# aantoine890/navierstokes

Hardware: AMD Instinct MI355X
Metric: fp64 CSR SpMV GFLOP/s & % HBM roofline @ nnz; 1/2/4/8 GPU (higher is better)
Workload: dtype f64

## Files before the change

include/mi355_spmv.h:

```cpp
#ifndef MI355_SPMV_H
#define MI355_SPMV_H

#ifdef __cplusplus
extern "C" {
#endif

#define MI355_SPMV_VERSION 501

enum {
    MI_OK = 0,
    MI_ERR_ARG = 1,
    MI_ERR_NODEVICE = 2,
    MI_ERR_HIP = 3,
    MI_ERR_ALLOC = 4,
    MI_ERR_UNSUPPORTED = 5,
    MI_ERR_STATE = 6
};

#define MI_MAX_POWERS 16

typedef struct mi_csr_s* mi_csr_t;
typedef struct mi_bcsr4_s* mi_bcsr4_t;
typedef struct mi_part_s* mi_part_t;
typedef void* mi_stream_t;

enum {
    MI_KERNEL_AUTO = 0,
    MI_KERNEL_STREAM = 1,
    MI_KERNEL_RING = 2,
    MI_KERNEL_ROWPAR = 3,
    MI_KERNEL_BCSR4 = 4,
    MI_KERNEL_MRING = 6,
    MI_KERNEL_SSTREAM = 7,
    MI_KERNEL_TILE = 5
};

int mi_version(void);
const char* mi_strerror(int status);
const char* mi_last_error(void);
int mi_device_count(int* count);
int mi_set_device(int device);
int mi_device_synchronize(void);
int mi_flush_cache(void);
int mi_flush_cache_async(mi_stream_t s);

int mi_csr_create(int n, int ncols, const int* ptrow, const int* indcol, const double* coef, mi_csr_t* out);
int mi_csr_create_mapped(int n, int ncols, const int* ptrow, const int* indcol, const double* coef,
                         const int* rowmap, mi_csr_t* out);
int mi_csr_destroy(mi_csr_t A);
int mi_csr_update_values(mi_csr_t A, const double* coef);
int mi_csr_update_values_dev(mi_csr_t A, const double* d_coef, mi_stream_t s);
int mi_csr_dims(mi_csr_t A, int* n, int* ncols, long long* nnz);
int mi_csr_reorder_info(mi_csr_t A, int* reordered, int* block, double* spread_before, double* spread_after,
                        double* us_natural, double* us_reordered);
int mi_csr_perm(mi_csr_t A, int* reordered, int* perm );
int mi_vec_to_internal_dev(mi_csr_t A, const double* d_x, double* d_x_int, mi_stream_t s);
int mi_vec_from_internal_dev(mi_csr_t A, const double* d_x_int, double* d_x, mi_stream_t s);
int mi_spmv_internal_dev(mi_csr_t A, const double* d_x_int, double* d_y_int, mi_stream_t s);
int mi_spmk_internal_dev(mi_csr_t A, int k, const double* d_x_int, double* const* d_y_int_out, mi_stream_t s);
int mi_reorder_probe(int n, const int* ptrow, const int* indcol, int* block, int* perm, double* spread_before,
                     double* spread_after);
int mi_csr_set_kernel(mi_csr_t A, int kernel_id);
int mi_csr_ring_info(mi_csr_t A, int* config_id, int* runs, int* runs_not_ringable, double* nnz_fraction_ringable);
int mi_csr_ring_shape_info(mi_csr_t A, int* blocks, int* lean, int* depth, double* us_aligned, double* us_unaligned);
int mi_csr_tune_info(mi_csr_t A, double* us_ring, double* us_stream);
int mi_csr_tune_detail(mi_csr_t A, double us[5], int* ring_nt, int* stream_nt);
int mi_ring_plan_probe(int n, const int* ptrow, const int* indcol, int config_id, int* nblk, int* runs,
                       int* runs_not_ringable, double* nnz_fraction_ringable, int* max_slot);
int mi_csr_tile_info(mi_csr_t A, int* built, int* nblk, double* unique_per_nnz, double us[2], int* nt);
int mi_tile_plan_probe(int n, const int* ptrow, const int* indcol, int threads, int* nblk, long long* distinct_total,
                       int* max_distinct, long long* nnz_listed);
int mi_csr_placement_info(mi_csr_t A, int* n_values, int* n_total, double* us, int cap);
int mi_vec_alloc_placed(mi_csr_t A, int nvec, int draws, double** d_vecs, double* us, int cap, int* n_us);
int mi_vec_free_placed(double* d_vec);
int mi_csr_sstream_info(mi_csr_t A, int* built, int* rounds, long long* steps, double* padding, double us[4], int* form);
int mi_sstream_plan_probe(int n, int ncols, const int* ptrow, const int* indcol, int* eligible, int* rounds, long long* steps, double* padding);
int mi_sstream_plan_probe_ex(int n, int ncols, const int* ptrow, const int* indcol, int shift, int ghost_lo, int ghost_hi, int* eligible, int* rounds,
                             long long* steps, double* padding, int* ghost_workgroups, int* rounds_min_max);
int mi_sstream_mw_plan_probe(int n, int ncols, const int* ptrow, const int* indcol, int shift, int* eligible, int* rounds, long long* steps, double* padding);
int mi_csr_mring_info(mi_csr_t A, int* built, int* runs, int* runs_not_served, double* nnz_fraction_served, double us[2], int* nt);
int mi_mring_plan_probe(int n, const int* ptrow, const int* indcol, int* nblk, int* runs, int* runs_not_served,
                        double* nnz_fraction_served, long long* window_restarts);
int mi_mring_plan_deal_probe(int n, const int* ptrow, const int* indcol, int* table_len, int* run_blocks, int cap);
int mi_ring_plan_lean(int n, const int* ptrow, const int* indcol, int config_id, int* lean);
int mi_csr_block4_structure(int n, const int* ptrow, const int* indcol, int* is_blocked, long long* nblocks);
int mi_csr_set_nontemporal(mi_csr_t A, int ring_nt, int stream_nt);
int mi_stream_read_probe(long long bytes, int launches, double* us_per_launch);
int mi_csr_get_kernel(mi_csr_t A, int* kernel_id);
const char* mi_csr_kernel_name(mi_csr_t A);

int mi_spmv(mi_csr_t A, const double* x, double* y);
int mi_spmv_dev(mi_csr_t A, const double* d_x, double* d_y, mi_stream_t s);

int mi_spmk(mi_csr_t A, int k, const double* x, double* const* y_out);
int mi_spmk_dev(mi_csr_t A, int k, const double* d_x, double* const* d_y_out, mi_stream_t s);

int mi_csr_spmk_info(mi_csr_t A, int k, int* eligible, int* one_launch, double* us_k_launches, double* us_one_launch);

int mi_spmk_plan_probe(int n, const int* ptrow, const int* indcol, int* eligible, int* runs, int* max_deps);

int mi_dot(int n, const double* x, const double* y, double* out);
int mi_dot_dev(int n, const double* d_x, const double* d_y, double* d_out, mi_stream_t s);
int mi_axpy(int n, double a, const double* x, double* y);
int mi_axpy_dev(int n, double a, const double* d_x, double* d_y, mi_stream_t s);
int mi_orthogonalize(int n, const double* b, const double* x1, double* x3, double alpha, double* beta_out);
int mi_orthogonalize_dev(int n, const double* d_b, const double* d_x1, double* d_x3, double alpha,
                         double* d_beta_out, mi_stream_t s);
int mi_spmv_dot_dev(mi_csr_t A, const double* d_x, double* d_y, const double* d_b, double* d_beta_out, mi_stream_t s);
int mi_csr_dot_epilogue_info(mi_csr_t A, int* in_epilogue);
int mi_csr_dot_epilogue_layout(mi_csr_t A, int* threads, int* wgs, int* nblk, int* run_first_block, int* block_row0,
                               int* block_rows, int cap_runs, int cap_blocks);
int mi_spmv_orthogonalize_dev(mi_csr_t A, const double* d_x, double* d_x1, const double* d_b, double* d_x3, double alpha,
                              double* d_beta_out, mi_stream_t s);
int mi_orthonormalize_against_basis(int n, int m, const double* const* basis, double* y, double* dots_out );
int mi_orthonormalize_against_basis_dev(int n, int m, const double* const* d_basis, double* d_y, double* d_dots ,
                                        mi_stream_t s);
int mi_mdot(int n, int m, const double* const* basis, const double* y, double* dots );
int mi_mdot_dev(int n, int m, const double* const* d_basis , const double* d_y,
                double* d_dots , mi_stream_t s);
int mi_maxpy(int n, int m, const double* coef , int negate, const double* const* basis, double* y);
int mi_maxpy_dev(int n, int m, const double* d_coef , int negate, const double* const* d_basis, double* d_y,
                 double* d_norm_out, mi_stream_t s);
int mi_cgs_dev(int n, int m, const double* const* d_basis, double* d_y, int passes, double* d_h ,
               double* d_norm , mi_stream_t s);
int mi_norm2(int n, const double* x, double* out);
int mi_norm2_dev(int n, const double* d_x, double* d_out, mi_stream_t s);
int mi_rel_error(int n, const double* ref, const double* test, double* out);
int mi_rel_error_dev(int n, const double* d_ref, const double* d_test, double* d_out, mi_stream_t s);
int mi_gather_dev(int m, const int* d_idx, const double* d_src, double* d_dst, mi_stream_t s);

int mi_bcsr4_create(int nbrows, int nbcols, const int* ptrow, const int* indcol, const double* coef,
                    mi_bcsr4_t* out);
int mi_bcsr4_destroy(mi_bcsr4_t A);
enum { MI_BLOCK_ROWMAJOR = 0, MI_BLOCK_COLMAJOR = 1 };
int mi_bcsr4_create_layout(int nbrows, int nbcols, const int* ptrow, const int* indcol, const double* coef, int layout, mi_bcsr4_t* out);
int mi_bcsr4_update_values_layout(mi_bcsr4_t A, const double* coef, int layout);
int mi_bcsr4_update_values_layout_dev(mi_bcsr4_t A, const double* d_coef, int layout, mi_stream_t s);
int mi_bcsr4_tile_info(mi_bcsr4_t A, int* built, int* in_use, double* us_plain, double* us_tile);
int mi_bcsr4_sell_info(mi_bcsr4_t A, int* built, int* form_in_use, long long* steps, double* padding, double us[4]);
int mi_bcsr4_sell_plan_probe(int nbrows, const int* ptrow, const int* indcol, int nwaves_max, int* nslices, long long* nsteps, int* nwaves,
                             int* sptr, int* wrng, unsigned* col);
int mi_bcsr4_update_values(mi_bcsr4_t A, const double* coef);
int mi_bcsr4_update_values_dev(mi_bcsr4_t A, const double* d_coef, mi_stream_t s);
int mi_bcsr4_spmv(mi_bcsr4_t A, const double* x, double* y);
int mi_bcsr4_spmv_dev(mi_bcsr4_t A, const double* d_x, double* d_y, mi_stream_t s);
int mi_bcsr4_spmk(mi_bcsr4_t A, int k, const double* x, double* const* y_out);
int mi_bcsr4_spmk_dev(mi_bcsr4_t A, int k, const double* d_x, double* const* d_y_out, mi_stream_t s);

enum { MI_ARITH_CHAIN = 0, MI_ARITH_BLOCKACC = 1 };
int mi_bcsr4_spmm(mi_bcsr4_t A, int s, const double* X, long long ldx, double* Y, long long ldy, int arith);
int mi_bcsr4_spmm_dev(mi_bcsr4_t A, int s, const double* d_X, long long ldx, double* d_Y, long long ldy, int arith,
                      mi_stream_t st);
int mi_bcsr4_spmm_info(mi_bcsr4_t A, int s, int* tile_built, int* form_in_use, int* longest_list, double us[5]);
int mi_bcsr4_spmm_plan_probe(int nbrows, const int* ptrow, const int* indcol, int per, int ucap, int* refused, int* ntiles, int* umax,
                             double* mean_list, int* wg_ptr, long long wg_ptr_cap, unsigned* nodes, long long nodes_cap,
                             unsigned short* slots, long long slots_cap, int* rows, long long rows_cap);
int mi_spmm_dev(mi_csr_t A, int s, const double* d_X, long long ldx, double* d_Y, long long ldy, mi_stream_t st);
int mi_krylov_basis_dev(mi_csr_t A, int s, const double* d_v0, double* d_V, long long ldv, int orth, double* d_coef,
                        mi_stream_t st);
int mi_krylov_basis_cgs_dev(mi_csr_t A, int s, const double* d_v0, double* d_V, long long ldv, int passes, double* d_coef,
                            mi_stream_t st);

typedef struct mi_bilu4_s* mi_bilu4_t;
int mi_bilu4_create(int nbrows, const int* ptrow, const int* indcol, const double* coef, int layout , int fill,
                    mi_bilu4_t* out);
int mi_bilu4_create_host(int nbrows, const int* ptrow, const int* indcol, const double* coef, int layout, int fill, mi_bilu4_t* out);
int mi_bilu4_destroy(mi_bilu4_t F);
int mi_bilu4_refactor(mi_bilu4_t F, const double* coef, int layout);
int mi_bilu4_solve_dev(mi_bilu4_t F, const double* d_b, double* d_x, mi_stream_t s);
int mi_bilu4_solve(mi_bilu4_t F, const double* b, double* x);
int mi_bilu4_info(mi_bilu4_t F, int* nbrows, long long* nblocks, int* fwd_levels, int* bwd_levels, int* launches, int* form,
                  double us[2], double* factor_seconds, long long* factor_bytes);
int mi_bilu4_factor_host(mi_bilu4_t F, int* ptr, int* col, int* diag, double* val, long long cap_blocks);
int mi_bilu4_plan_probe(int nbrows, const int* ptrow, const int* indcol, int fill, long long* nblocks, int* fwd_levels,
                        int* bwd_levels, int* fwd_launches, int* bwd_launches, int* fwd_sizes, int* bwd_sizes, int cap_levels);

int mi_bilu4dev_plan_probe(int nbrows, const int* ptrow, const int* indcol, int fill, long long* update_pairs, int* launches,
                           long long* plan_bytes);
int mi_bilu4dev_prepare(mi_bilu4_t F);
int mi_bilu4dev_refactor(mi_bilu4_t F, const double* d_coef, int layout, mi_stream_t s);
int mi_bilu4dev_status(mi_bilu4_t F, int* bad_row);
int mi_bilu4dev_fetch(mi_bilu4_t F);
int mi_bilu4dev_info(mi_bilu4_t F, int* prepared, int* launches, long long* plan_bytes);

enum { MI_BILU_FORM_LEVELS = 0, MI_BILU_FORM_ONE = 1, MI_BILU_FORM_AUTO = -1 };
int mi_bilu4one_plan_probe(int nbrows, const int* ptrow, const int* indcol, int fill, int workgroups, int* eligible, int nchunks[2],
                           int max_deps[2], long long* plan_bytes, int* const chunk_pos[2], int* const chunk_lev[2],
                           int* const dep_ptr[2], int* const dep[2]);
int mi_bilu4one_prepare(mi_bilu4_t F);
int (mi_bilu4_set_solve_form)(mi_bilu4_t F, int form);
int mi_bilu4one_status(mi_bilu4_t F);
int mi_bilu4one_info(mi_bilu4_t F, int* prepared, int* eligible, int* workgroups, int nchunks[2], int max_deps[2], long long* plan_bytes);

int mi_bilu4sw_prepare(mi_bilu4_t F);
int mi_bilu4sw_solve_dev(mi_bilu4_t F, const double* d_b, double* d_x, int sweeps_fwd, int sweeps_bwd, mi_stream_t s);
int mi_bilu4sw_solve(mi_bilu4_t F, const double* b, double* x, int sweeps_fwd, int sweeps_bwd);
int mi_bilu4sw_info(mi_bilu4_t F, int* prepared, int* max_fwd, int* max_bwd, int* launches_last, long long* work_bytes);

int mi_bilu4sp_prepare(mi_bilu4_t F);
int mi_bilu4sp_solve_dev(mi_bilu4_t F, const double* d_b, double* d_x, int sweeps_fwd, int sweeps_bwd, mi_stream_t s);
int mi_bilu4sp_solve(mi_bilu4_t F, const double* b, double* x, int sweeps_fwd, int sweeps_bwd);
int mi_bilu4sp_status(mi_bilu4_t F, int* bad_block_row, long long* overflowed);
int mi_bilu4sp_fetch(mi_bilu4_t F, float* val, long long cap_blocks);
int mi_bilu4sp_info(mi_bilu4_t F, int* prepared, int* convert_launches, int* launches_last, long long* copy_bytes);

int mi_part_create(int nranks, int rank, const long long* row_starts, const int* ptrow,
                   const int* indcol_global, const double* coef, mi_part_t* out);
int mi_part_destroy(mi_part_t P);
int mi_part_sizes(mi_part_t P, int* n_local, int* n_halo, int* n_interior_rows, int* n_boundary_rows);
int mi_part_recv_counts(mi_part_t P, int* counts );
int mi_part_recv_ids(mi_part_t P, int peer, long long* ids );
int mi_part_set_send_ids(mi_part_t P, int peer, int count, const long long* ids );
int mi_part_send_counts(mi_part_t P, int* counts );
int mi_part_local_csr(mi_part_t P, int which, int* nrows, const int** ptrow, const int** indcol_local,
                      const double** coef, const int** rowmap);
int mi_part_combined_info(mi_part_t P, int* n_left);
int mi_part_sends_contiguous(mi_part_t P, int* contiguous);
int mi_part_send_index(mi_part_t P, int* total, const int** local_idx );
int mi_part_finalize(mi_part_t P);
int mi_part_set_kernel(mi_part_t P, int kernel_id);
int mi_part_update_values(mi_part_t P, const double* coef);
int mi_part_pack_dev(mi_part_t P, const double* d_x_ext, double* d_sendbuf, mi_stream_t s);
int mi_part_spmv_interior_dev(mi_part_t P, const double* d_x_ext, double* d_y_local, mi_stream_t s);
int mi_part_spmv_boundary_dev(mi_part_t P, const double* d_x_ext, double* d_y_local, mi_stream_t s);

#define MI_COMM_ID_BYTES 128
int mi_comm_available(void);
int mi_comm_unique_id(void* id128);
int mi_part_comm_init(mi_part_t P, const void* id128);
int mi_part_comm_info(mi_part_t P, int* comm_ranks, int* comm_rank);
int mi_part_spmv_dev(mi_part_t P, double* d_x_ext, double* d_y_local, mi_stream_t s);
int mi_part_status(mi_part_t P);
int mi_part_send_union(mi_part_t P, int* count, const int** local_idx );
int mi_part_allgather_setup(mi_part_t P, const int* counts , const long long* ids );
int mi_part_set_allgather(mi_part_t P, int on);
int mi_part_allgather_info(mi_part_t P, int* ready, int* in_use, int* slice );
#define MI_IPC_HANDLE_BYTES 64
int mi_part_push_export(mi_part_t P, void* handle64, long long* layout );
int mi_part_push_connect(mi_part_t P, const void* handles , const long long* layouts );
int mi_part_spmv_push_dev(mi_part_t P, double* d_x_ext, double* d_y_local, mi_stream_t s);
int mi_part_push_info(mi_part_t P, int* ready, int* fused, int* neighbours);
const char* mi_part_kernel_name(mi_part_t P, int which);
int mi_part_push_unfuse(mi_part_t P);
int mi_part_push_disable(mi_part_t P);
int mi_comm_selftest(int count, double* max_abs_err);

typedef struct mi_dist_s* mi_dist_t;
typedef struct mi_dist_vec_s* mi_dist_vec_t;
int mi_dist_create(int ndev, int n, const int* ptrow, const int* indcol, const double* coef, mi_dist_t* out);
int mi_dist_destroy(mi_dist_t D);
int mi_dist_info(mi_dist_t D, int* nranks, int* distinct_devices, int* exchange, int* fused, long long* halo_total, long long* halo_max);
const char* mi_dist_exchange_name(mi_dist_t D);
const char* mi_dist_exchange_note(mi_dist_t D);
int mi_dist_rank_info(mi_dist_t D, int rank, int* device, long long* row_start, int* n_local, int* n_halo, long long* nnz_local,
                      mi_stream_t* stream );
int mi_dist_update_values(mi_dist_t D, const double* coef);
int mi_dist_spmv(mi_dist_t D, const double* x, double* y);
int mi_dist_spmk(mi_dist_t D, int k, const double* x, double* const* y_out);
int mi_dist_dot(mi_dist_t D, const double* x, const double* y, double* out);
int mi_dist_orthogonalize(mi_dist_t D, const double* b, const double* x1, double* x3, double alpha, double* beta_out);
int mi_dist_vec_create(mi_dist_t D, mi_dist_vec_t* out);
int mi_dist_vec_destroy(mi_dist_vec_t v);
int mi_dist_vec_set(mi_dist_vec_t v, const double* host );
int mi_dist_vec_get(mi_dist_vec_t v, double* host );
int mi_dist_vec_ptr(mi_dist_vec_t v, int rank, double** d_ptr);
int mi_dist_spmv_dev(mi_dist_t D, mi_dist_vec_t x, mi_dist_vec_t y);
int mi_dist_spmk_dev(mi_dist_t D, int k, mi_dist_vec_t x, const mi_dist_vec_t* y_out );
int mi_dist_synchronize(mi_dist_t D);
int mi_dist_dot_dev(mi_dist_t D, mi_dist_vec_t a, mi_dist_vec_t b, double* out);
int mi_dist_orthogonalize_dev(mi_dist_t D, mi_dist_vec_t b, mi_dist_vec_t x1, mi_dist_vec_t x3, double alpha, double* beta_out);

#ifdef __cplusplus
}
#endif
#endif
```

navierstokes_amd/csrc/capi_csr.hip:

```cpp
#include "capi_internal.hpp"
#include "reorder.hpp"
#include "mring_plan.hpp"
#include "tile_plan.hpp"

int get_table(mi_csr_t A, int nnzb, BlockTable** out)
{
    auto it = A->tables.find(nnzb);
    if (it == A->tables.end()) {
        std::vector<int> rows, ptrs;
        int row_align = A->nnz < 20000000 ? 64 : 1;
        if (const char* e = getenv("MI355_STREAM_ROW_ALIGN")) row_align = std::max(1, atoi(e));
        build_row_blocks(A->n, A->h_ptrow.data(), nnzb, 4 * kWG, rows, ptrs, row_align, 7);
        BlockTable T;
        T.nnzb = nnzb;
        T.nblk = (int)rows.size() - 1;
        std::vector<int2> h(rows.size());
        for (size_t i = 0; i < rows.size(); i++) h[i] = make_int2(rows[i], ptrs[i]);
        HIP_TRY(T.d_blk.upload(h));
        it = A->tables.emplace(nnzb, std::move(T)).first;
    }
    *out = &it->second;
    return MI_OK;
}

static inline bool beyond_infinity_cache(double bytes_per_nnz, long long nnz, int n) { return bytes_per_nnz * (double)nnz + 16.0 * (double)n > 0.75 * 256e6; }

constexpr double kSsMaxPadding = 0.12;
static double ss_max_padding()
{
    if (const char* e = getenv("MI355_SSTREAM_MAX_PADDING")) return std::max(0.0, atof(e));
    return kSsMaxPadding;
}

static int build_sstream(mi_csr_t A, const int* ptrow, const int* indcol, int ghost_lo = 0, int ghost_hi = 0)
{
    if (A->ss.dev.val) return MI_OK;
    SsPlanHost P;
    SsMwPlanHost M;
    const int shift = (A->y_offset & 1) && !A->d_rowmap ? 1 : 0;
    build_sstream_plan(A->n, A->ncols, ptrow, indcol, ss_max_padding(), P, true, shift, ghost_lo, ghost_hi);
    SstreamCopy T;
    hipError_t e;
    if (!P.eligible) {
        if (ghost_lo < ghost_hi || env_is("MI355_SSTREAM_MW", "0")) return MI_OK;
        build_sstream_mw_plan(A->n, A->ncols, ptrow, indcol, ss_max_padding(), M, shift);
        if (!M.eligible) return MI_OK;
        e = ss_mw_upload(M, T.dev);
        T.mw = e == hipSuccess;
    } else e = ss_upload(P, T.dev, ghost_lo < ghost_hi);
    const SsPlanHost& Q = P.eligible ? P : M;
    if (e != hipSuccess) {
        if (e == hipErrorOutOfMemory) { (void)hipGetLastError(); return MI_OK; }
        return fail(MI_ERR_HIP, std::string("sliced copy: ") + hipGetErrorString(e));
    }
    T.nwg = Q.nwg;
    T.rounds = Q.rounds;
    T.shift = Q.shift;
    T.steps = Q.steps;
    T.padding = (double)Q.pad_places / (double)A->nnz;
    T.max_slice_nnz = Q.max_slice_nnz;
    if (ghost_lo < ghost_hi) {
        T.h_wg_halo = P.wg_halo;
        T.h_wg = P.wg;
        T.fusable = P.fusable;
    }
    sstream_fill_values(T.rounds, A->n, T.shift, A->d_ptrow, A->d_coef, nullptr, T.dev.slice_step, T.dev.slice_len, T.dev.val, T.max_slice_nnz, nullptr, T.mw ? 1 : 0);
    if ((e = hipGetLastError()) != hipSuccess) {
        T = {};
        return fail(MI_ERR_HIP, std::string("sliced copy fill: ") + hipGetErrorString(e));
    }
    T.nt = beyond_infinity_cache(10.0, A->nnz, A->n);
    T.deep = T.nt;
    if (const char* fe = getenv("MI355_SSTREAM_FORM")) {
        const int f = atoi(fe);
        T.nt = (f & 1) == 0;
        T.deep = f >= 2;
    }
    A->ss.copy() = std::move(T);
    return MI_OK;
}

int launch_sstream(mi_csr_t A, const double* d_x, double* d_y, const int* rowmap, hipStream_t s, const RingComm* comm)
{
    SstreamTable& T = A->ss;
    SsView S{T.dev.val, T.dev.slot, T.dev.wg, T.dev.win, T.nwg, A->n + T.shift, A->ncols, rowmap, T.shift};
    double* yy = rowmap ? d_y : d_y - T.shift;
    if (T.mw) {
        if (comm) return fail(MI_ERR_STATE, "the cut-ring sliced stream has no fused multi-GPU form");
        SsMwView V{S, T.dev.winK};
        if (T.deep) {
            if (T.nt) hipLaunchKernelGGL((spmv_sstream_mw<12, true>), dim3((unsigned)T.nwg), dim3(256), 0, s, V, d_x, yy);
            else hipLaunchKernelGGL((spmv_sstream_mw<12, false>), dim3((unsigned)T.nwg), dim3(256), 0, s, V, d_x, yy);
        } else {
            if (T.nt) hipLaunchKernelGGL((spmv_sstream_mw<8, true>), dim3((unsigned)T.nwg), dim3(256), 0, s, V, d_x, yy);
            else hipLaunchKernelGGL((spmv_sstream_mw<8, false>), dim3((unsigned)T.nwg), dim3(256), 0, s, V, d_x, yy);
        }
        HIP_TRY(hipGetLastError());
        return MI_OK;
    }
    if (comm) {
        const unsigned grid = (unsigned)(T.nwg + comm->push_wgs);
        if (T.deep) {
            if (T.nt) hipLaunchKernelGGL((spmv_sstream_fused<12, true>), dim3(grid), dim3(256), 0, s, S, d_x, yy, *comm);
            else hipLaunchKernelGGL((spmv_sstream_fused<12, false>), dim3(grid), dim3(256), 0, s, S, d_x, yy, *comm);
        } else {
            if (T.nt) hipLaunchKernelGGL((spmv_sstream_fused<8, true>), dim3(grid), dim3(256), 0, s, S, d_x, yy, *comm);
            else hipLaunchKernelGGL((spmv_sstream_fused<8, false>), dim3(grid), dim3(256), 0, s, S, d_x, yy, *comm);
        }
    } else if (T.deep) {
        if (T.nt) hipLaunchKernelGGL((spmv_sstream<12, true>), dim3((unsigned)T.nwg), dim3(256), 0, s, S, d_x, yy);
        else hipLaunchKernelGGL((spmv_sstream<12, false>), dim3((unsigned)T.nwg), dim3(256), 0, s, S, d_x, yy);
    } else {
        if (T.nt) hipLaunchKernelGGL((spmv_sstream<8, true>), dim3((unsigned)T.nwg), dim3(256), 0, s, S, d_x, yy);
        else hipLaunchKernelGGL((spmv_sstream<8, false>), dim3((unsigned)T.nwg), dim3(256), 0, s, S, d_x, yy);
    }
    HIP_TRY(hipGetLastError());
    return MI_OK;
}

static bool ring_wants_skew(int n, const int* ptrow)
{
    long long bad = 0;
    for (int i = 0; i < n; i++) {
        const int len = ptrow[i + 1] - ptrow[i];
        bad += len > 0 && (len % 16 == 0 || len == 8);
    }
    return 2 * bad > n;
}

constexpr long long kLargeNnz = 20000000;
static size_t placed_vector_len(int n, int ncols) { return (size_t)std::max(n, ncols) + 64; }
static int large_row_align(long long nnz) { return nnz >= kLargeNnz ? 1 : 0; }

static int build_mring(mi_csr_t A, const int* indcol, int row_align = 0)
{
    if (A->mring.d_plan || A->n == 0 || A->nnz == 0) return MI_OK;
    std::vector<int> back;
    if (!indcol) {
        if (!A->d_indcol) return fail(MI_ERR_STATE, "mring plan: the handle no longer holds its column indices");
        back.resize((size_t)A->nnz);
        HIP_TRY(hipMemcpy(back.data(), A->d_indcol, sizeof(int) * (size_t)A->nnz, hipMemcpyDeviceToHost));
        indcol = back.data();
    }
    MringPlanHost P;
    build_mring_plan(A->n, A->h_ptrow.data(), indcol, P, row_align);
    MringTable M;
    HIP_TRY(M.d_plan.alloc(P.plan.size()));
    HIP_TRY(M.d_first.upload(P.first));
    HIP_TRY(M.d_ok.alloc(P.run_ok.size()));
    HIP_TRY(M.d_rng.alloc(P.run_rng.size()));
    HIP_TRY(M.d_slots.alloc(P.slots.size()));
    HIP_TRY(M.d_plan.fill(P.plan));
    HIP_TRY(M.d_ok.fill(P.run_ok));
    HIP_TRY(M.d_rng.fill(P.run_rng));
    HIP_TRY(M.d_slots.fill(P.slots));
    M.nblk = P.nblk;
    M.wgs = P.wgs;
    M.nruns = P.nruns;
    M.bpw = P.bpw;
    M.bad_runs = P.bad_runs;
    M.restarts = P.restarts;
    M.ok_fraction = 1.0 - (double)P.bad_nnz / (double)A->nnz;
    M.depth = P.bpw >= 40 ? 4 : 2;
    M.skew = ring_wants_skew(A->n, A->h_ptrow.data());
    M.nt = beyond_infinity_cache(10.0, A->nnz, A->n);
    A->mring = std::move(M);
    return MI_OK;
}

static int build_tile(mi_csr_t A, const int* indcol)
{
    if (A->tile.d_desc || A->n == 0 || A->nnz == 0) return MI_OK;
    std::vector<int> back;
    if (!indcol) {
        if (!A->d_indcol) return fail(MI_ERR_STATE, "tile plan: the handle no longer holds its column indices");
        back.resize((size_t)A->nnz);
        HIP_TRY(hipMemcpy(back.data(), A->d_indcol, sizeof(int) * (size_t)A->nnz, hipMemcpyDeviceToHost));
        indcol = back.data();
    }
    TilePlanHost P;
    build_tile_plan(A->n, A->h_ptrow.data(), indcol, P, kTileNnzb, 0, A->nnz < 20000000 ? 64 : 1);
    TileTable T;
    HIP_TRY(T.d_desc.alloc(P.desc.size()));
    HIP_TRY(T.d_ulist.alloc(P.ulist.size()));
    HIP_TRY(T.d_slots.alloc(P.slots.size()));
    HIP_TRY(T.d_desc.fill(P.desc));
    HIP_TRY(T.d_ulist.fill(P.ulist));
    HIP_TRY(T.d_slots.fill(P.slots));
    T.nblk = P.nblk;
    T.unique_per_nnz = (double)(P.ulist.size() - kTileThreads) / (double)A->nnz;
    long long mult8 = 0;
    for (int i = 0; i < A->n; i++) {
        const int len = A->h_ptrow[i + 1] - A->h_ptrow[i];
        mult8 += len > 0 && len % 8 == 0;
    }
    T.skew = 10 * mult8 > A->n;
    T.nt = beyond_infinity_cache(10.0, A->nnz, A->n);
    A->tile = std::move(T);
    return MI_OK;
}

static int fill_ring_table(RingTable& R, const RingPlanHost& best, int n, const int* ptrow, const int* indcol, long long nnz, bool ghosts,
                           const int* row_min = nullptr, const int* row_max = nullptr, bool square = false)
{
    R.cfg = best.cfg;
    if (best.cfg.id == 4 && best.bpw >= 40) R.cfg.depth = 4;
    if (const char* e = getenv("MI355_RING_DEPTH")) {
        const int d = atoi(e);
        if (best.cfg.id == 4 && d >= 2 && d <= 4) R.cfg.depth = d;
    }
    R.nblk = best.nblk;
    R.wgs = best.wgs;
    R.bpw = best.bpw;
    R.bad_runs = best.bad_runs;
    R.ok_fraction = nnz ? 1.0 - (double)best.bad_nnz / (double)nnz : 0.0;
    R.lean = best.lean && best.cfg.id == 4 && !env_is("MI355_RING_LEAN", "0");
    if (best.nblk <= 0) return MI_OK;
    HIP_TRY(R.d_plan.upload(best.plan));
    HIP_TRY(R.d_ok.upload(best.run_ok));
    R.all_in_loop = true;
    for (int g = 0; g < best.wgs; g++) R.all_in_loop = R.all_in_loop && best.run_ok[g] == 1;
    R.h_dep_ptr.clear();
    R.h_dep_run.clear();
    if (square && row_min && R.all_in_loop && R.lean && best.cfg.id == 4 && !ghosts) build_run_deps(best, n, R.h_dep_ptr, R.h_dep_run);
    for (int g = 0; g < best.wgs; g++)
        R.uniform = R.uniform && best.run_rng[2 * g] == std::min(best.nblk, g * best.bpw) &&
                    best.run_rng[2 * g + 1] == std::min(best.nblk, (g + 1) * best.bpw);
    HIP_TRY(R.d_rng.upload(best.run_rng));
    if (ghosts) {
        R.h_run_halo = best.run_halo;
        HIP_TRY(R.d_run_halo.upload(best.run_halo));
    }
    {
        std::vector<unsigned short> slots;
        build_ring_slots(best, indcol, slots);
        HIP_TRY(R.d_slots.upload(slots));
    }
    R.skew = ring_wants_skew(n, ptrow);
    if (const char* e2 = getenv("MI355_RING_SKEW")) R.skew = atoi(e2) != 0;
    return MI_OK;
}

static int time_on(LaunchTimer& tm, mi_csr_t A, const double* x, double* y, int warm, int timed, double* us)
{
    return tm.time(warm, timed, [&] { return launch_spmv(A, x, y, nullptr); }, us);
}

static int placement_draws(mi_csr_t A, ScratchPair* given, bool keep_pair)
{
    const long long nnz = A->nnz;
    const char* pe = getenv("MI355_PLACEMENT_DRAWS");
    int draws = pe ? std::max(0, std::min(16, atoi(pe))) : 4;
    const bool early_stop = pe == nullptr;
    if (!pe) {
        size_t mem_free = 0, mem_total = 0;
        if (hipMemGetInfo(&mem_free, &mem_total) == hipSuccess && nnz > 0)
            draws = (int)std::min<size_t>((size_t)draws, mem_free / 8 / (sizeof(double) * (size_t)nnz));
        else (void)hipGetLastError();
    }
    const bool blocked_choice = A->auto_kernel == MI_KERNEL_BCSR4 && A->blocked && A->blocked->d_coef && !(A->blocked->sell_form >= 0 && A->blocked->sell.val);
    const bool streams_coef = A->auto_kernel == MI_KERNEL_RING || A->auto_kernel == MI_KERNEL_MRING || A->auto_kernel == MI_KERNEL_STREAM || A->auto_kernel == MI_KERNEL_TILE || blocked_choice;
    if (!(draws > 0 && streams_coef && nnz >= kLargeNnz)) return MI_OK;
    LaunchTimer tm;
    ScratchPair own;
    ScratchPair& pair = given ? *given : own;
    if (!given) {
        const size_t len = std::max(placed_vector_len(A->n, A->ncols), (size_t)(A->n_out > 0 ? A->n_out : 1));
        if (int rc = own.alloc(len, len)) return rc;
    }
    double *const tx = pair.x, *const ty = pair.y;
    if (int rc = tm.init()) return rc;
    auto time_now = [&](double* us) { return time_on(tm, A, tx, ty, 3, 8, us); };
    auto redraw = [&](auto& slot, size_t len, size_t pad, int ndraws) {
        using Arr = std::remove_reference_t<decltype(slot)>;
        double best = 0.0;
        if (!slot || len == 0 || time_now(&best) != MI_OK) return;
        const double first = best;
        A->place_us.push_back(best);
        std::vector<Arr> losers;
        for (int d = 0; d < ndraws; d++) {
            Arr fresh;
            if (fresh.alloc(len + pad) != hipSuccess) { (void)hipGetLastError(); break; }
            if ((pad && hipMemset(fresh + len, 0, sizeof(*fresh.get()) * pad) != hipSuccess) ||
                hipMemcpy(fresh, slot, sizeof(*fresh.get()) * len, hipMemcpyDeviceToDevice) != hipSuccess) { (void)hipGetLastError(); break; }
            std::swap(slot, fresh);
            double t = 0.0;
            const int rct = time_now(&t);
            A->place_us.push_back(rct == MI_OK ? t : -1.0);
            if (rct == MI_OK && t < 0.96 * best) best = t;
            else std::swap(slot, fresh);
            losers.push_back(std::move(fresh));
            if (early_stop && d == 0 && rct == MI_OK && std::fabs(t - first) <= 0.02 * first) break;
        }
        for (Arr& l : losers) l = {};
    };
    if (blocked_choice) redraw(A->blocked->d_coef, 16 * (size_t)A->blocked->nblocks, 16, draws);
    else redraw(A->d_coef, (size_t)nnz, (size_t)kRingPadNnz, draws);
    A->place_draws_coef = (int)A->place_us.size();
    if (A->auto_kernel == MI_KERNEL_RING) redraw(A->ring.d_slots, (size_t)A->ring.nblk * A->ring.cfg.nnzb, 0, (draws + 1) / 2);
    else if (A->auto_kernel == MI_KERNEL_MRING) redraw(A->mring.d_slots, (size_t)A->mring.nblk * kMringNnzb, 0, (draws + 1) / 2);
    if (keep_pair && !A->kept_x) A->kept_x = std::move(pair.x), A->kept_y = std::move(pair.y);
    return MI_OK;
}

constexpr long long kMeasureNnz = 200000;

struct CsrInput {
    int n, ncols;
    const int* ptrow;
    const int* indcol;
    const double* coef;
    const int* rowmap;
    int ghost_lo, ghost_hi;
    long long nnz = 0;
    bool offset_only = false;
    std::vector<int> row_min, row_max;
    bool ghosts() const { return ghost_lo < ghost_hi; }
};

static int check_input(CsrInput& in)
{
    const int n = in.n;
    const int* ptrow = in.ptrow;
    CHECK_ARG(n >= 0 && in.ncols >= 0, "negative dimension");
    CHECK_ARG(ptrow, "ptrow is null");
    CHECK_ARG(ptrow[0] == 0, "ptrow[0] must be 0");
    for (int i = 0; i < n; i++) CHECK_ARG(ptrow[i] <= ptrow[i + 1], "ptrow must be non-decreasing");
    in.nnz = ptrow[n];
    CHECK_ARG(in.nnz == 0 || (in.indcol && in.coef), "indcol/coef is null");
    CHECK_ARG(in.nnz <= 0x7fffffffLL - 2 * kRingPadNnz && n <= 0x7fffffff - 2 * kRingPadRows, "matrix too large for 32-bit offsets: partition it (mi_part_*)");
    in.row_min.resize((size_t)n);
    in.row_max.resize((size_t)n);
    for (int i = 0; i < n; i++) {
        int lo = 0x7fffffff, hi = -1;
        for (int k = ptrow[i]; k < ptrow[i + 1]; k++) {
            const int c = in.indcol[k];
            CHECK_ARG(c >= 0 && c < in.ncols, "column index outside [0, ncols)");
            lo = c < lo ? c : lo;
            hi = c > hi ? c : hi;
        }
        in.row_min[i] = lo;
        in.row_max[i] = hi;
    }
    in.offset_only = in.rowmap != nullptr && n > 0;
    for (int i = 1; in.offset_only && i < n; i++) in.offset_only = in.rowmap[i] == in.rowmap[0] + i;
    return MI_OK;
}

static int upload(mi_csr_t A, const CsrInput& in)
{
    const int n = in.n;
    const long long nnz = in.nnz;
    const size_t pad = 8, padv = kRingPadNnz, padr = kRingPadRows;
    HIP_TRY(hipGetDevice(&A->device));
    HIP_TRY(A->d_ptrow.alloc((size_t)n + 1 + padr));
    HIP_TRY(A->d_indcol.alloc((size_t)nnz + pad));
    HIP_TRY(A->d_coef.alloc((size_t)nnz + padv));
    HIP_TRY(hipMemset(A->d_ptrow + n + 1, 0, sizeof(int) * padr));
    HIP_TRY(hipMemset(A->d_indcol + nnz, 0, sizeof(int) * pad));
    HIP_TRY(hipMemset(A->d_coef + nnz, 0, sizeof(double) * padv));
    HIP_TRY(A->d_ptrow.fill(in.ptrow, (size_t)n + 1));
    HIP_TRY(A->d_indcol.fill(in.indcol, (size_t)nnz));
    HIP_TRY(A->d_coef.fill(in.coef, (size_t)nnz));
    A->mapped = in.rowmap != nullptr;
    if (in.offset_only) A->y_offset = in.rowmap[0];
    if (in.rowmap && n > 0 && !in.offset_only) {
        HIP_TRY(A->d_rowmap.alloc((size_t)n + padr));
        HIP_TRY(hipMemset(A->d_rowmap + n, 0, sizeof(int) * padr));
        HIP_TRY(A->d_rowmap.fill(in.rowmap, (size_t)n));
    }
    return MI_OK;
}

static int plan_ring(mi_csr_t A, const CsrInput& in)
{
    const int n = in.n;
    const long long nnz = in.nnz;
    if (n == 0 || nnz == 0) return MI_OK;
    int forced = 0;
    if (const char* e = getenv("MI355_RING_CONFIG")) forced = atoi(e);
    RingPlanHost best;
    bool have = false;
    for (int t = 0; t < kNumRingConfigs && !have; t++) {
        const int id = forced >= 1 && forced <= kNumRingConfigs ? forced : kRingConfigOrder[t];
        RingPlanHost P;
        build_ring_plan(kRingConfigs[id - 1], n, in.ptrow, in.row_min.data(), in.row_max.data(), P, in.ghost_lo, in.ghost_hi, large_row_align(nnz));
        const double okf = 1.0 - (double)P.bad_nnz / (double)nnz;
        if (forced || okf >= 0.90) {
            best = std::move(P);
            have = true;
        } else if (t == 0) {
            best = std::move(P);
        }
        if (forced) break;
    }
    RingTable R;
    if (int rc = fill_ring_table(R, best, n, in.ptrow, in.indcol, nnz, in.ghosts(), in.row_min.data(), in.row_max.data(), n == in.ncols)) return rc;
    A->ring = std::move(R);
    A->auto_kernel = (have && A->ring.ok_fraction >= 0.90) ? MI_KERNEL_RING : MI_KERNEL_STREAM;
    return MI_OK;
}

static bool plan_wanted(const char* sw, const char* name, bool by_size, bool* asked)
{
    *asked = env_is(sw, "1") || env_is("MI355_SPMV_KERNEL", name);
    return !env_is(sw, "0") && (*asked || by_size);
}

static int plan_optional(mi_csr_t A, const CsrInput& in)
{
    if (in.n == 0 || in.nnz == 0) return MI_OK;
    const bool measured = in.nnz >= kMeasureNnz;
    bool asked;
    int rc;
    if (plan_wanted("MI355_TILE", "tile", measured && A->auto_kernel != MI_KERNEL_RING, &asked)) {
        if ((rc = build_tile(A, in.indcol))) return rc;
        if (!asked && A->tile.unique_per_nnz > 0.6) A->tile = {};
    }
    if (plan_wanted("MI355_MRING", "mring", measured && A->auto_kernel != MI_KERNEL_RING, &asked)) {
        if ((rc = build_mring(A, in.indcol, large_row_align(in.nnz)))) return rc;
        if (!asked && A->mring.ok_fraction < 0.90) A->mring = {};
    }
    if (plan_wanted("MI355_SSTREAM", "sstream", measured, &asked)) {
        if ((rc = build_sstream(A, in.ptrow, in.indcol, in.ghost_lo, in.ghost_hi))) return rc;
        A->ss.asked = asked;
    }
    return MI_OK;
}

static int attach_blocked(mi_csr_t A, const CsrInput& in)
{
    const int n = in.n;
    const int* rowmap = in.rowmap;
    bool node_map = rowmap != nullptr && !in.offset_only && n % 4 == 0;
    for (int b = 0; node_map && b < n / 4; b++)
        node_map = rowmap[4 * b] % 4 == 0 && rowmap[4 * b + 1] == rowmap[4 * b] + 1 && rowmap[4 * b + 2] == rowmap[4 * b] + 2 &&
                   rowmap[4 * b + 3] == rowmap[4 * b] + 3;
    if (!(!rowmap || in.offset_only || node_map) || n < 4 || in.nnz < 16 || in.ncols % 4 != 0 || env_is("MI355_AUTO_BCSR", "0")) return MI_OK;
    std::vector<int> bptr, bcol;
    std::vector<double> bval;
    if (!csr_to_bcsr4_exact(n, in.ptrow, in.indcol, in.coef, bptr, bcol, bval)) return MI_OK;
    mi_bcsr4_t B = nullptr;
    if (int rc = mi_bcsr4_create(n / 4, in.ncols / 4, bptr.data(), bcol.data(), bval.data(), &B)) return rc;
    A->blocked.reset(B);
    if (node_map) {
        std::vector<int> bmap((size_t)n / 4);
        for (int b = 0; b < n / 4; b++) bmap[b] = rowmap[4 * b] / 4;
        HIP_TRY(B->d_browmap.upload(bmap));
    }
    return MI_OK;
}

static void load_defaults(mi_csr_t A, const CsrInput& in)
{
    A->ring.nt = A->ring.d_slots && beyond_infinity_cache(10.0, in.nnz, in.n);
    if (const char* e = getenv("MI355_RING_NT")) A->ring.nt = A->ring.d_slots && atoi(e) != 0;
    A->stream_nt = beyond_infinity_cache(12.0, in.nnz, in.n);
    if (const char* e = getenv("MI355_STREAM_NT")) A->stream_nt = atoi(e) != 0;
    if (const char* e = getenv("MI355_TILE_NT")) A->tile.nt = atoi(e) != 0;
    if (const char* e = getenv("MI355_MRING_NT")) A->mring.nt = atoi(e) != 0;
    if (A->blocked) A->auto_kernel = MI_KERNEL_BCSR4;
    A->n_out = in.n;
    if (in.rowmap)
        for (int i = 0; i < in.n; i++) A->n_out = in.rowmap[i] + 1 > A->n_out ? in.rowmap[i] + 1 : A->n_out;
}

static bool apply_forced_kernel(mi_csr_t A)
{
    const char* e = getenv("MI355_SPMV_KERNEL");
    if (!e) return false;
    if (!strcmp(e, "stream")) A->auto_kernel = MI_KERNEL_STREAM;
    else if (!strcmp(e, "ring") && A->ring.d_plan) A->auto_kernel = MI_KERNEL_RING;
    else if (!strcmp(e, "rowpar")) A->auto_kernel = MI_KERNEL_ROWPAR;
    else if (!strcmp(e, "bcsr4") && A->blocked) A->auto_kernel = MI_KERNEL_BCSR4;
    else if (!strcmp(e, "tile") && A->tile.d_desc) A->auto_kernel = MI_KERNEL_TILE;
    else if (!strcmp(e, "mring") && A->mring.d_plan) A->auto_kernel = MI_KERNEL_MRING;
    else if (!strcmp(e, "sstream") && A->ss.dev.val) A->auto_kernel = MI_KERNEL_SSTREAM;
    else return false;
    return true;
}

static bool& nt_flag(mi_csr_t A, int k)
{
    switch (k) {
    case MI_KERNEL_RING: return A->ring.nt;
    case MI_KERNEL_TILE: return A->tile.nt;
    case MI_KERNEL_MRING: return A->mring.nt;
    default: return A->stream_nt;
    }
}

static double tuned_us(mi_csr_t A, int k)
{
    if (k == MI_KERNEL_BCSR4 && A->tune_us[k][0] > 0) return A->tune_us[k][0];
    if (k != MI_KERNEL_RING && k != MI_KERNEL_TILE && k != MI_KERNEL_MRING) k = MI_KERNEL_STREAM;
    return A->tune_us[k][nt_flag(A, k)];
}

static const struct {
    int kernel;
    const char* nt_env;
} kTuneKernels[4] = {{MI_KERNEL_RING, "MI355_RING_NT"}, {MI_KERNEL_STREAM, "MI355_STREAM_NT"}, {MI_KERNEL_TILE, "MI355_TILE_NT"}, {MI_KERNEL_MRING, "MI355_MRING_NT"}};

static void tune(mi_csr_t A, LaunchTimer& tm, const ScratchPair& sp)
{
    const int timed = A->nnz < 40000000 ? 12 : 6;
    auto measure = [&](int warm, int count, double& slot, bool& failed) {
        double t = 0.0;
        if (time_on(tm, A, sp.x, sp.y, warm, count, &t) == MI_OK) slot = min_measured(slot, t);
        else failed = true;
    };
    const bool ring_ok = A->auto_kernel == MI_KERNEL_RING;
    auto in_race = [&](int k) {
        return k == MI_KERNEL_RING ? ring_ok : k == MI_KERNEL_TILE ? A->tile.d_desc != nullptr : k == MI_KERNEL_MRING ? A->mring.d_plan != nullptr : true;
    };
    bool nt0[4], failed[4][2] = {};
    for (int i = 0; i < 4; i++) nt0[i] = nt_flag(A, kTuneKernels[i].kernel);
    const double* ring_us = A->tune_us[MI_KERNEL_RING];
    for (int round = 0; round < 2; round++)
        for (int i = 0; i < 4; i++)
            for (int nt = 0; nt < 2; nt++) {
                const int k = kTuneKernels[i].kernel;
                double& us = A->tune_us[k][nt];
                if (!in_race(k) || failed[i][nt] || (getenv(kTuneKernels[i].nt_env) && nt != nt0[i])) continue;
                if (k == MI_KERNEL_RING && nt && !A->ring.d_slots) continue;
                if (k == MI_KERNEL_STREAM && round == 1 && ring_ok &&
                    us > 1.25 * std::min(ring_us[0] > 0 ? ring_us[0] : ring_us[1], ring_us[1] > 0 ? ring_us[1] : ring_us[0]))
                    continue;
                nt_flag(A, k) = nt;
                A->kernel = k;
                measure(3, timed, us, failed[i][nt]);
            }
    for (int i = 0; i < 4; i++) {
        const int k = kTuneKernels[i].kernel;
        for (int nt = 0; nt < 2; nt++)
            if (failed[i][nt]) A->tune_us[k][nt] = 0.0;
        nt_flag(A, k) = in_race(k) ? better(A->tune_us[k][1], A->tune_us[k][0]) : nt0[i];
    }
    for (int i = 0; i < 4; i++)
        if (better(tuned_us(A, kTuneKernels[i].kernel), tuned_us(A, A->auto_kernel))) A->auto_kernel = kTuneKernels[i].kernel;
    if (A->blocked) {
        const double holder = tuned_us(A, A->auto_kernel);
        bool bfailed = false;
        A->kernel = MI_KERNEL_BCSR4;
        measure(3, 6, A->tune_us[MI_KERNEL_BCSR4][0], bfailed);
        if (better(A->tune_us[MI_KERNEL_BCSR4][0], holder)) A->auto_kernel = MI_KERNEL_BCSR4;
    }
    if (A->ss.dev.val && !getenv("MI355_SSTREAM_FORM")) {
        const double holder = tuned_us(A, A->auto_kernel);
        double* us = A->ss.tune_us;
        bool sfailed[4] = {};
        A->kernel = MI_KERNEL_SSTREAM;
        for (int round = 0; round < 2; round++)
            for (int f = 0; f < 4; f++) {
                if (sfailed[f]) continue;
                A->ss.nt = (f & 1) == 0;
                A->ss.deep = f >= 2;
                measure(3, timed, us[f], sfailed[f]);
            }
        int bf = -1;
        for (int f = 0; f < 4; f++) {
            if (sfailed[f]) us[f] = 0.0;
            if (us[f] > 0 && (bf < 0 || us[f] < us[bf])) bf = f;
        }
        if (bf >= 0) {
            A->ss.nt = (bf & 1) == 0;
            A->ss.deep = bf >= 2;
            if (better(us[bf], holder)) A->auto_kernel = MI_KERNEL_SSTREAM;
        }
        if (A->auto_kernel != MI_KERNEL_SSTREAM && !A->ss.asked && !(A->ghost_lo < A->ghost_hi)) A->ss.copy() = {};
    }
    A->kernel = MI_KERNEL_AUTO;
}

static void compare_ring_shapes(mi_csr_t A, const CsrInput& in, LaunchTimer& tm, const ScratchPair& sp)
{
    const long long nnz = in.nnz;
    if (!env_is("MI355_RING_SHAPE_COMPARE", "1") || getenv("MI355_RING_ROW_ALIGN") || nnz < kLargeNnz) return;
    auto time_now = [&](double* us) { return time_on(tm, A, sp.x, sp.y, 3, 8, us); };
    double us64 = 0.0, us1 = 0.0;
    if (A->auto_kernel == MI_KERNEL_RING && A->ring.cfg.id == 4) {
        RingPlanHost alt;
        build_ring_plan(kRingConfigs[3], in.n, in.ptrow, in.row_min.data(), in.row_max.data(), alt, in.ghost_lo, in.ghost_hi, 64);
        RingTable aligned;
        if (1.0 - (double)alt.bad_nnz / (double)nnz >= 0.90 &&
            fill_ring_table(aligned, alt, in.n, in.ptrow, in.indcol, nnz, in.ghosts(), in.row_min.data(), in.row_max.data(), in.n == in.ncols) == MI_OK) {
            aligned.nt = A->ring.nt;
            A->kernel = MI_KERNEL_RING;
            int rct = time_now(&us1);
            RingTable unaligned = std::move(A->ring);
            A->ring = std::move(aligned);
            if (rct == MI_OK) rct = time_now(&us64);
            A->kernel = MI_KERNEL_AUTO;
            A->tune_us_ring_aligned = us64;
            A->tune_us_ring_unaligned = us1;
            if (rct != MI_OK || !(us64 < 0.98 * us1)) A->ring = std::move(unaligned);
            else unaligned = {};
        }
    } else if (A->auto_kernel == MI_KERNEL_MRING) {
        MringTable unaligned = std::move(A->mring);
        if (build_mring(A, in.indcol, 64) == MI_OK && A->mring.d_plan && A->mring.ok_fraction >= 0.90) {
            A->mring.nt = unaligned.nt;
            A->kernel = MI_KERNEL_MRING;
            int rct = time_now(&us64);
            MringTable aligned = std::move(A->mring);
            A->mring = std::move(unaligned);
            if (rct == MI_OK) rct = time_now(&us1);
            A->kernel = MI_KERNEL_AUTO;
            A->tune_us_ring_aligned = us64;
            A->tune_us_ring_unaligned = us1;
            if (rct == MI_OK && us64 < 0.98 * us1) A->mring = std::move(aligned);
            else aligned = {};
        } else {
            A->mring = std::move(unaligned);
        }
    }
}

static int measure_at_create(mi_csr_t A, const CsrInput& in, bool defer_placement)
{
    const size_t scratch_len = placed_vector_len(in.n, in.ncols);
    LaunchTimer tm;
    ScratchPair sp;
    int rc = sp.alloc(std::max(scratch_len, (size_t)(in.ncols > 0 ? in.ncols : 1)), std::max(scratch_len, (size_t)(A->n_out > 0 ? A->n_out : 1)));
    if (rc || (rc = tm.init())) return rc;
    tune(A, tm, sp);
    compare_ring_shapes(A, in, tm, sp);
    if (!defer_placement) (void)placement_draws(A, &sp, !in.rowmap && in.n == in.ncols && in.n == A->n_out && !in.ghosts());
    return MI_OK;
}

int csr_create_impl(int n, int ncols, const int* ptrow, const int* indcol, const double* coef,
                    const int* rowmap, mi_csr_t* out, int ghost_lo, int ghost_hi, bool defer_placement)
{
    CHECK_ARG(out, "out is null");
    *out = nullptr;
    CsrInput in{n, ncols, ptrow, indcol, coef, rowmap, ghost_lo, ghost_hi};
    int rc = check_input(in);
    if (rc || (rc = need_device())) return rc;
    std::unique_ptr<mi_csr_s> owner(new (std::nothrow) mi_csr_s());
    mi_csr_t A = owner.get();
    if (!A) return fail(MI_ERR_ALLOC, "host allocation failed");
    A->n = n;
    A->ncols = ncols;
    A->nnz = in.nnz;
    A->ghost_lo = ghost_lo;
    A->ghost_hi = ghost_hi;
    A->h_ptrow.assign(ptrow, ptrow + n + 1);
    if ((rc = upload(A, in)) || (rc = plan_ring(A, in)) || (rc = plan_optional(A, in)) || (rc = attach_blocked(A, in))) return rc;
    load_defaults(A, in);
    const bool forced_kernel = apply_forced_kernel(A);
    if (!forced_kernel && in.nnz < kMeasureNnz && A->auto_kernel == MI_KERNEL_RING && !in.ghosts()) A->auto_kernel = MI_KERNEL_STREAM;
    if (!forced_kernel && !env_is("MI355_SPMV_AUTOTUNE", "0") && in.nnz >= kMeasureNnz && (rc = measure_at_create(A, in, defer_placement))) return rc;
    HIP_TRY(hipStreamSynchronize(nullptr));
    *out = owner.release();
    return MI_OK;
}

static int time_handle(mi_csr_t A, int warm, int timed, double* us)
{
    LaunchTimer tm;
    ScratchPair sp;
    int rc = sp.alloc((size_t)(A->ncols > 0 ? A->ncols : 1), (size_t)(A->n_out > 0 ? A->n_out : 1));
    if (rc || (rc = tm.init())) return rc;
    return time_on(tm, A, sp.x, sp.y, warm, timed, us);
}

static int maybe_reorder(mi_csr_t A, const int* ptrow, const int* indcol, const double* coef)
{
    const bool force = env_is("MI355_REORDER", "1");
    if (env_is("MI355_REORDER", "0")) return MI_OK;
    const int n = A->n;
    if (A->mapped || n != A->ncols || n < 8 || A->nnz == 0) return MI_OK;
    if (!force && (n < 100000 || resolve_kernel(A) == MI_KERNEL_RING || resolve_kernel(A) == MI_KERNEL_SSTREAM)) return MI_OK;
    const int block = csr_has_block4_pattern(n, ptrow, indcol) ? 4 : 1;
    const double nn = (double)n / block;
    const double spread = mean_column_distance(n, ptrow, indcol, block);
    A->spread_before = spread;
    if (!force && spread < 2.0 * std::pow(nn, 2.0 / 3.0)) return MI_OK;
    Reorder R;
    rcm_reorder(n, ptrow, indcol, block, R);
    A->reorder_block = block;
    A->spread_after = R.spread_after;
    if (!force && R.spread_after > 0.5 * spread) return MI_OK;
    std::vector<int> p2, c2, src_start;
    std::vector<double> v2;
    permute_csr(n, ptrow, indcol, coef, R, p2, c2, v2, src_start);
    mi_csr_t inner = nullptr;
    int rc = csr_create_impl(n, n, p2.data(), c2.data(), v2.data(), R.iperm.data(), &inner);
    if (rc) return rc;
    A->inner.reset(inner);
    HIP_TRY(A->d_iperm.alloc((size_t)n));
    HIP_TRY(A->d_src_start.alloc((size_t)n));
    HIP_TRY(A->d_xp.alloc((size_t)n));
    HIP_TRY(A->d_iperm.fill(R.iperm));
    HIP_TRY(A->d_src_start.fill(src_start));
    bool keep = true;
    if (!force && !env_is("MI355_SPMV_AUTOTUNE", "0")) {
        const int timed = A->nnz < 40000000 ? 12 : 6;
        (void)A->inner.own.release();
        rc = time_handle(A, 3, timed, &A->us_natural);
        A->inner.reset(inner);
        if (rc) return rc;
        if ((rc = time_handle(A, 3, timed, &A->us_reordered))) return rc;
        keep = A->us_reordered < 0.97 * A->us_natural;
    }
    if (!keep) {
        A->inner.reset(), A->d_iperm = {}, A->d_src_start = {}, A->d_xp = {};
        return MI_OK;
    }
    A->h_iperm = R.iperm;
    A->xp_claimed = false;
    A->d_ptrow = {}, A->d_indcol = {}, A->d_coef = {};
    A->drop_tables();
    A->ring = {}, A->tile = {}, A->mring = {}, A->ss = {}, A->blocked.reset();
    return MI_OK;
}

extern "C" int mi_csr_create(int n, int ncols, const int* ptrow, const int* indcol, const double* coef, mi_csr_t* out)
{
    int rc = csr_create_impl(n, ncols, ptrow, indcol, coef, nullptr, out, 0, 0, true);
    if (rc) return rc;
    if ((rc = maybe_reorder(*out, ptrow, indcol, coef)) || (!(*out)->inner && (rc = placement_draws(*out, nullptr, n == ncols))) ||
        (hipStreamSynchronize(nullptr) != hipSuccess && (rc = fail(MI_ERR_HIP, "mi_csr_create: synchronize")))) {
        mi_csr_destroy(*out);
        *out = nullptr;
    }
    return rc;
}

extern "C" int mi_reorder_probe(int n, const int* ptrow, const int* indcol, int* block, int* perm, double* spread_before,
                                double* spread_after)
{
    CHECK_ARG(n >= 0 && ptrow && (ptrow[n] == 0 || indcol), "bad argument");
    for (int i = 0; i < n; i++) {
        CHECK_ARG(ptrow[i] <= ptrow[i + 1], "ptrow must be non-decreasing");
        for (int k = ptrow[i]; k < ptrow[i + 1]; k++) CHECK_ARG(indcol[k] >= 0 && indcol[k] < n, "column index outside [0, n)");
    }
    const int b = csr_has_block4_pattern(n, ptrow, indcol) ? 4 : 1;
    Reorder R;
    rcm_reorder(n, ptrow, indcol, b, R);
    if (block) *block = b;
    if (perm)
        for (int i = 0; i < n; i++) perm[i] = R.perm[i];
    if (spread_before) *spread_before = R.spread_before;
    if (spread_after) *spread_after = R.spread_after;
    return MI_OK;
}

extern "C" int mi_csr_reorder_info(mi_csr_t A, int* reordered, int* block, double* spread_before, double* spread_after,
                                   double* us_natural, double* us_reordered)
{
    CHECK_ARG(A, "null handle");
    if (reordered) *reordered = A->inner ? 1 : 0;
    if (block) *block = A->reorder_block;
    if (spread_before) *spread_before = A->spread_before;
    if (spread_after) *spread_after = A->spread_after;
    if (us_natural) *us_natural = A->us_natural;
    if (us_reordered) *us_reordered = A->us_reordered;
    return MI_OK;
}

extern "C" int mi_csr_perm(mi_csr_t A, int* reordered, int* perm)
{
    CHECK_ARG(A, "null handle");
    if (reordered) *reordered = A->inner ? 1 : 0;
    if (perm) {
        if (A->inner) {
            CHECK_ARG((int)A->h_iperm.size() == A->n, "permutation not kept on this handle");
            for (int r = 0; r < A->n; r++) perm[A->h_iperm[r]] = r;
        } else {
            for (int i = 0; i < A->n; i++) perm[i] = i;
        }
    }
    return MI_OK;
}

extern "C" int mi_vec_to_internal_dev(mi_csr_t A, const double* d_x, double* d_x_int, mi_stream_t s)
{
    CHECK_ARG(A, "null handle");
    if (A->n == 0) return MI_OK;
    CHECK_ARG(d_x && d_x_int && d_x != d_x_int, "null vector, or in place");
    if (A->inner) return gather_perm(A, d_x, d_x_int, (hipStream_t)s);
    HIP_TRY(hipMemcpyAsync(d_x_int, d_x, sizeof(double) * (size_t)A->n, hipMemcpyDeviceToDevice, (hipStream_t)s));
    return MI_OK;
}

extern "C" int mi_vec_from_internal_dev(mi_csr_t A, const double* d_x_int, double* d_x, mi_stream_t s)
{
    CHECK_ARG(A, "null handle");
    if (A->n == 0) return MI_OK;
    CHECK_ARG(d_x && d_x_int && d_x != d_x_int, "null vector, or in place");
    if (A->inner) return scatter_perm(A, d_x_int, d_x, (hipStream_t)s);
    HIP_TRY(hipMemcpyAsync(d_x, d_x_int, sizeof(double) * (size_t)A->n, hipMemcpyDeviceToDevice, (hipStream_t)s));
    return MI_OK;
}

extern "C" int mi_spmv_internal_dev(mi_csr_t A, const double* d_x_int, double* d_y_int, mi_stream_t s)
{
    CHECK_ARG(A, "null handle");
    CHECK_ARG(A->n == A->ncols && !A->mapped, "the internal numbering is defined for square, unmapped matrices");
    CHECK_ARG(A->n == 0 || (d_x_int && d_y_int), "null vector");
    if (A->inner) return launch_spmv(A->inner, d_x_int, d_y_int, (hipStream_t)s, false);
    return launch_spmv(A, d_x_int, d_y_int, (hipStream_t)s);
}

extern "C" int mi_spmk_internal_dev(mi_csr_t A, int k, const double* d_x_int, double* const* d_y_int_out, mi_stream_t s)
{
    CHECK_ARG(A, "null handle");
    if (k < 1 || k > MI_MAX_POWERS) return fail(MI_ERR_UNSUPPORTED, "k must be in 1..MI_MAX_POWERS");
    CHECK_ARG(d_y_int_out, "null output array");
    CHECK_ARG(A->n == A->ncols && !A->mapped, "the internal numbering is defined for square, unmapped matrices");
    if (A->n == 0) return MI_OK;
    CHECK_ARG(d_x_int, "null vector");
    for (int p = 0; p < k; p++) CHECK_ARG(d_y_int_out[p], "null output vector");
    return spmk_unmapped(A->inner ? A->inner : A, k, d_x_int, d_y_int_out, (hipStream_t)s);
}

extern "C" int mi_csr_create_mapped(int n, int ncols, const int* ptrow, const int* indcol, const double* coef,
                                    const int* rowmap, mi_csr_t* out)
{
    return csr_create_impl(n, ncols, ptrow, indcol, coef, rowmap, out);
}

extern "C" int mi_csr_destroy(mi_csr_t A)
{
    if (!A) return MI_OK;
    delete A;
    return MI_OK;
}

static int refresh_blocked_values(mi_csr_t A, hipStream_t s, bool sliced_done = false)
{
    if (A->ss.dev.val && !sliced_done) {
        SstreamTable& T = A->ss;
        sstream_fill_values(T.rounds, A->n, T.shift, A->d_ptrow, A->d_coef, nullptr, T.dev.slice_step, T.dev.slice_len, T.dev.val, T.max_slice_nnz, s, T.mw ? 1 : 0);
        HIP_TRY(hipGetLastError());
    }
    if (!A->blocked || A->blocked->nbrows == 0) return MI_OK;
    return bcsr4_refresh_from_csr(A->blocked, A->d_ptrow, A->d_coef, nullptr, s);
}

__global__ __launch_bounds__(256) void permute_values_kernel(int n, const int* __restrict__ new_ptrow, const int* __restrict__ src_start,
                                                             const double* __restrict__ src, double* __restrict__ dst)
{
    __shared__ int s_p[65], s_a[64];
    const int tid = threadIdx.x;
    for (int r0 = blockIdx.x * 64; r0 < n; r0 += gridDim.x * 64) {
        const int nr = min(64, n - r0);
        if (tid <= nr) s_p[tid] = new_ptrow[r0 + tid];
        if (tid < nr) s_a[tid] = src_start[r0 + tid];
        __syncthreads();
        const int b0 = s_p[0], seg = s_p[nr] - b0;
        for (int k = tid; k < seg; k += 256) {
            const int p = b0 + k;
            int lo = 0, hi = nr;
            while (hi - lo > 1) {
                const int mid = (lo + hi) >> 1;
                if (s_p[mid] <= p) lo = mid;
                else hi = mid;
            }
            dst[p] = src[s_a[lo] + (p - s_p[lo])];
        }
        __syncthreads();
    }
}

extern "C" int mi_csr_update_values_dev(mi_csr_t A, const double* d_coef, mi_stream_t s_)
{
    CHECK_ARG(A, "null handle");
    if (A->nnz == 0) return MI_OK;
    CHECK_ARG(d_coef, "null coef");
    hipStream_t s = (hipStream_t)s_;
    if (A->inner) {
        mi_csr_t I = A->inner;
        hipLaunchKernelGGL(permute_values_kernel, dim3((unsigned)std::max(1, std::min((A->n + 63) / 64, 4096))), dim3(256), 0, s, A->n, I->d_ptrow, A->d_src_start, d_coef, I->d_coef);
        HIP_TRY(hipGetLastError());
        return refresh_blocked_values(I, s);
    }
    if (A->ss.dev.val && d_coef != A->d_coef) {
        SstreamTable& T = A->ss;
        sstream_fill_values(T.rounds, A->n, T.shift, A->d_ptrow, d_coef, A->d_coef, T.dev.slice_step, T.dev.slice_len, T.dev.val, T.max_slice_nnz, s, T.mw ? 1 : 0);
        HIP_TRY(hipGetLastError());
        return refresh_blocked_values(A, s, true);
    }
    if (A->blocked && A->blocked->nbrows > 0 && d_coef != A->d_coef)
        return bcsr4_refresh_from_csr(A->blocked, A->d_ptrow, d_coef, A->d_coef, s);
    if (d_coef != A->d_coef) HIP_TRY(hipMemcpyAsync(A->d_coef, d_coef, sizeof(double) * (size_t)A->nnz, hipMemcpyDeviceToDevice, s));
    return refresh_blocked_values(A, s);
}

extern "C" int mi_csr_update_values(mi_csr_t A, const double* coef)
{
    CHECK_ARG(A, "null handle");
    if (A->nnz == 0) return MI_OK;
    CHECK_ARG(coef, "null coef");
    if (A->inner) {
        if (!A->d_vtmp) HIP_TRY(A->d_vtmp.alloc((size_t)A->nnz));
        HIP_TRY(hipMemcpy(A->d_vtmp, coef, sizeof(double) * (size_t)A->nnz, hipMemcpyHostToDevice));
        int rc = mi_csr_update_values_dev(A, A->d_vtmp, nullptr);
        if (rc) return rc;
        HIP_TRY(hipStreamSynchronize(nullptr));
        return MI_OK;
    }
    HIP_TRY(hipMemcpy(A->d_coef, coef, sizeof(double) * (size_t)A->nnz, hipMemcpyHostToDevice));
    int rc = refresh_blocked_values(A, nullptr);
    if (rc) return rc;
    HIP_TRY(hipStreamSynchronize(nullptr));
    return MI_OK;
}

extern "C" int mi_csr_dims(mi_csr_t A, int* n, int* ncols, long long* nnz)
{
    CHECK_ARG(A, "null handle");
    if (n) *n = A->n;
    if (ncols) *ncols = A->ncols;
    if (nnz) *nnz = A->nnz;
    return MI_OK;
}

int resolve_kernel(const mi_csr_s* A)
{
    int k = A->kernel != MI_KERNEL_AUTO ? A->kernel : A->auto_kernel;
    if (k == MI_KERNEL_RING && !A->ring.d_plan) k = MI_KERNEL_STREAM;
    if (k == MI_KERNEL_BCSR4 && !A->blocked) k = MI_KERNEL_STREAM;
    if (k == MI_KERNEL_TILE && !A->tile.d_desc) k = MI_KERNEL_STREAM;
    if (k == MI_KERNEL_MRING && !A->mring.d_plan) k = MI_KERNEL_STREAM;
    if (k == MI_KERNEL_SSTREAM && !A->ss.dev.val) k = A->ring.d_plan && A->ring.ok_fraction >= 0.90 ? MI_KERNEL_RING : MI_KERNEL_STREAM;
    return k;
}

extern "C" int mi_csr_tune_info(mi_csr_t A, double* us_ring, double* us_stream)
{
    CHECK_ARG(A, "null handle");
    if (A->inner) A = A->inner;
    if (us_ring) *us_ring = A->tune_us[MI_KERNEL_RING][A->ring.nt];
    if (us_stream) *us_stream = A->tune_us[MI_KERNEL_STREAM][A->stream_nt];
    return MI_OK;
}

extern "C" int mi_csr_tune_detail(mi_csr_t A, double us[5], int* ring_nt, int* stream_nt)
{
    CHECK_ARG(A, "null handle");
    if (A->inner) A = A->inner;
    if (us) {
        us[0] = A->tune_us[MI_KERNEL_RING][0];
        us[1] = A->tune_us[MI_KERNEL_RING][1];
        us[2] = A->tune_us[MI_KERNEL_STREAM][0];
        us[3] = A->tune_us[MI_KERNEL_STREAM][1];
        us[4] = A->tune_us[MI_KERNEL_BCSR4][0];
    }
    if (ring_nt) *ring_nt = A->ring.nt ? 1 : 0;
    if (stream_nt) *stream_nt = A->stream_nt ? 1 : 0;
    return MI_OK;
}
extern "C" int mi_ring_plan_probe(int n, const int* ptrow, const int* indcol, int config_id, int* nblk, int* runs,
                                  int* runs_not_ringable, double* nnz_fraction_ringable, int* max_slot)
{
    CHECK_ARG(n >= 0 && ptrow && config_id >= 1 && config_id <= kNumRingConfigs, "bad argument");
    const long long nnz = ptrow[n];
    CHECK_ARG(nnz == 0 || indcol, "indcol is null");
    std::vector<int> row_min((size_t)n), row_max((size_t)n);
    for (int i = 0; i < n; i++) {
        int lo = 0x7fffffff, hi = -1;
        for (int k = ptrow[i]; k < ptrow[i + 1]; k++) {
            lo = std::min(lo, indcol[k]);
            hi = std::max(hi, indcol[k]);
        }
        row_min[i] = lo;
        row_max[i] = hi;
    }
    RingPlanHost P;
    build_ring_plan(kRingConfigs[config_id - 1], n, ptrow, row_min.data(), row_max.data(), P);
    std::vector<unsigned short> slots;
    if (P.nblk > 0) build_ring_slots(P, indcol, slots);
    const RingConfig& c = P.cfg;
    const int T = c.threads, per = c.nnzb / T;
    int next_row = 0, mslot = -1;
    long long next_nz = 0;
    std::vector<int> content((size_t)c.ring, -1);
    int cur_run = -1;
    std::vector<int> run_of((size_t)P.nblk, -1);
    long long wmax = 0, wsum = 0;
    for (int g = 0; g < P.wgs; g++) {
        const int b0 = P.run_rng[2 * g], b1 = P.run_rng[2 * g + 1];
        if (b0 < 0 || b1 < b0 || b1 > P.nblk || b1 - b0 > kRingMaxB) return fail(MI_ERR_STATE, "run range out of bounds or longer than the kernel's plan");
        long long w = 0;
        for (int b = b0; b < b1; b++) {
            if (run_of[b] >= 0) return fail(MI_ERR_STATE, "a block belongs to two runs");
            run_of[b] = g;
            w += !P.run_ok[g] || P.plan[(size_t)8 * b + 7] == 2 ? kRingPlainWeight : 1;
        }
        wmax = std::max(wmax, w);
        wsum += w;
    }
    for (int b = 0; b < P.nblk; b++)
        if (run_of[b] < 0) return fail(MI_ERR_STATE, "a block belongs to no run");
    if (P.wgs > 0 && wmax > 2 * (wsum / P.wgs) + 4 * kRingPlainWeight) return fail(MI_ERR_STATE, "one run carries more than twice the mean weight");
    for (int b = 0; b < P.nblk; b++) {
        const int* Q = &P.plan[(size_t)8 * b];
        if (Q[0] != next_row || Q[1] != next_nz) return fail(MI_ERR_STATE, "plan does not cover rows / nonzeros in order");
        const int brows = Q[7] == 2 ? Q[4] : Q[2];
        next_row += brows;
        next_nz += Q[3];
        if (Q[3] != ptrow[Q[0] + brows] - ptrow[Q[0]]) return fail(MI_ERR_STATE, "block nonzero count disagrees with ptrow");
        const int run = run_of[b];
        if (P.lean && P.run_ok[run] && brows > T) return fail(MI_ERR_STATE, "a LEAN plan holds a block of more than T rows");
        if (!P.run_ok[run] || Q[3] == 0) {
            if (Q[7] == 2 || (Q[7] && Q[3] == 0)) return fail(MI_ERR_STATE, "flags of a block outside the ring loop");
            continue;
        }
        if (Q[7] == 2) {
            if (Q[2] != 0 || Q[5] != 0) return fail(MI_ERR_STATE, "a PLAIN block is visible to the ring loop");
            if (P.run_ok[run] != 3) return fail(MI_ERR_STATE, "a run with a PLAIN block does not tell the kernel to look behind its loop");
            continue;
        }
        if (Q[7] != 1 || Q[3] > c.nnzb || Q[2] > 2 * T) return fail(MI_ERR_STATE, "a served run holds a block the kernel cannot take");
        int cmin = 0x7fffffff, cmax = -1;
        for (long long k = Q[1]; k < (long long)Q[1] + Q[3]; k++) {
            cmin = std::min(cmin, indcol[k]);
            cmax = std::max(cmax, indcol[k]);
        }
        if (cmax - cmin + 1 > c.ring) return fail(MI_ERR_STATE, "block window wider than the ring");
        if (cmin - Q[6] < 0 || cmax - Q[6] >= 2 * c.ring) return fail(MI_ERR_STATE, "ring base out of range for the block's columns");
        if (Q[4] + Q[5] < cmax + 1) return fail(MI_ERR_STATE, "window does not reach the block's last column");
        if (P.lean && Q[5] > T && b != P.run_rng[2 * run]) return fail(MI_ERR_STATE, "a LEAN plan brings more than T new columns into a block inside a run");
        if (run != cur_run) {
            std::fill(content.begin(), content.end(), -1);
            cur_run = run;
        }
        for (int col = Q[4]; col < Q[4] + Q[5]; col++) {
            int sl = col - Q[6];
            if (sl >= c.ring) sl -= c.ring;
            if (sl < 0 || sl >= c.ring) return fail(MI_ERR_STATE, "a new column falls outside the ring");
            content[sl] = col;
        }
        for (int k = 0; k < Q[3]; k++)
            if (content[(indcol[Q[1] + k] - Q[6]) >= c.ring ? indcol[Q[1] + k] - Q[6] - c.ring : indcol[Q[1] + k] - Q[6]] != indcol[Q[1] + k])
                return fail(MI_ERR_STATE, "a nonzero's column is not in the window when its block runs");
        for (int k = 0; k < Q[3]; k++) {
            const int slot = slots[(size_t)b * c.nnzb + (size_t)ring_slot_pos(T, per, k)];
            int want = indcol[Q[1] + k] - Q[6];
            if (want >= c.ring) want -= c.ring;
            if (slot != want || slot < 0 || slot >= c.ring) return fail(MI_ERR_STATE, "16-bit slot disagrees with the column");
            mslot = std::max(mslot, slot);
        }
    }
    if (next_row != n || next_nz != nnz) return fail(MI_ERR_STATE, "plan does not cover the matrix");
    if (nblk) *nblk = P.nblk;
    if (runs) *runs = P.wgs;
    if (runs_not_ringable) *runs_not_ringable = P.bad_runs;
    if (nnz_fraction_ringable) *nnz_fraction_ringable = nnz ? 1.0 - (double)P.bad_nnz / (double)nnz : 0.0;
    if (max_slot) *max_slot = mslot;
    return MI_OK;
}

extern "C" int mi_spmk_plan_probe(int n, const int* ptrow, const int* indcol, int* eligible, int* runs, int* max_deps)
{
    CHECK_ARG(n >= 0 && ptrow && ptrow[0] == 0 && eligible, "bad argument");
    CHECK_ARG(ptrow[n] == 0 || indcol, "indcol is null");
    *eligible = 0;
    if (runs) *runs = 0;
    if (max_deps) *max_deps = 0;
    if (n == 0 || ptrow[n] == 0) return MI_OK;
    std::vector<int> row_min((size_t)n), row_max((size_t)n);
    for (int i = 0; i < n; i++) {
        int lo = 0x7fffffff, hi = -1;
        for (int k = ptrow[i]; k < ptrow[i + 1]; k++) {
            CHECK_ARG(indcol[k] >= 0 && indcol[k] < n, "column index outside [0, n)");
            lo = std::min(lo, indcol[k]);
            hi = std::max(hi, indcol[k]);
        }
        row_min[i] = lo;
        row_max[i] = hi;
    }
    RingPlanHost P;
    build_ring_plan(kRingConfigs[3], n, ptrow, row_min.data(), row_max.data(), P);
    bool all_in_loop = P.lean && P.nblk > 0;
    for (int g = 0; g < P.wgs; g++) all_in_loop = all_in_loop && P.run_ok[g] == 1;
    if (!all_in_loop) return MI_OK;
    std::vector<int> dp, dr;
    build_run_deps(P, n, dp, dr);
    const int W = P.wgs, T = P.cfg.threads;
    std::vector<int> owner((size_t)n, -1);
    for (int g = 0; g < W; g++)
        for (int b = P.run_rng[2 * g]; b < P.run_rng[2 * g + 1]; b++)
            for (int r = P.plan[(size_t)8 * b]; r < P.plan[(size_t)8 * b] + P.plan[(size_t)8 * b + 2]; r++) owner[r] = g;
    for (int i = 0; i < n; i++)
        if (owner[i] < 0) return fail(MI_ERR_STATE, "a row belongs to no run");
    int md = 0;
    std::vector<char> on_list((size_t)W);
    for (int g = 0; g < W; g++) {
        md = std::max(md, dp[g + 1] - dp[g]);
        std::fill(on_list.begin(), on_list.end(), 0);
        for (int j = dp[g]; j < dp[g + 1]; j++) on_list[dr[j]] = 1;
        const int b0 = P.run_rng[2 * g], b1 = P.run_rng[2 * g + 1];
        if (b0 >= b1) continue;
        for (int b = b0; b < b1; b++) {
            const int* Q = &P.plan[(size_t)8 * b];
            for (int k = Q[1]; k < Q[1] + Q[3]; k++)
                if (!on_list[owner[indcol[k]]]) return fail(MI_ERR_STATE, "a run names a column of a run that is not on its list");
            const int load_hi = std::min(n - 1, Q[4] + std::max(Q[5], T) - 1);
            for (int col = Q[4]; col <= load_hi; col++)
                if (!on_list[owner[col]]) return fail(MI_ERR_STATE, "a run loads a column of a run that is not on its list");
        }
    }
    *eligible = md <= 64 ? 1 : 0;
    if (runs) *runs = W;
    if (max_deps) *max_deps = md;
    return MI_OK;
}

extern "C" int mi_csr_sstream_info(mi_csr_t A, int* built, int* rounds, long long* steps, double* padding, double us[4], int* form)
{
    CHECK_ARG(A, "null handle");
    if (A->inner) A = A->inner;
    if (built) *built = A->ss.dev.val != nullptr;
    if (rounds) *rounds = A->ss.rounds;
    if (steps) *steps = A->ss.steps;
    if (padding) *padding = A->ss.padding;
    if (us)
        for (int f = 0; f < 4; f++) us[f] = A->ss.tune_us[f];
    if (form) *form = A->ss.dev.val ? (A->ss.deep ? 2 : 0) + (A->ss.nt ? 0 : 1) : -1;
    return MI_OK;
}

extern "C" int mi_sstream_plan_probe(int n, int ncols, const int* ptrow, const int* indcol, int* eligible, int* rounds, long long* steps, double* padding)
{
    return mi_sstream_plan_probe_ex(n, ncols, ptrow, indcol, 0, 0, 0, eligible, rounds, steps, padding, nullptr, nullptr);
}

extern "C" int mi_sstream_plan_probe_ex(int n, int ncols, const int* ptrow, const int* indcol, int shift, int ghost_lo, int ghost_hi, int* eligible, int* rounds,
                                        long long* steps, double* padding, int* ghost_workgroups, int* rounds_min_max)
{
    CHECK_ARG(n >= 0 && ncols >= 0 && ptrow && ptrow[0] == 0 && eligible, "bad argument");
    CHECK_ARG(shift == 0 || shift == 1, "shift must be 0 or 1");
    CHECK_ARG(ghost_lo >= 0 && ghost_hi <= ncols, "ghost range outside the columns");
    CHECK_ARG(ptrow[n] == 0 || indcol, "indcol is null");
    for (int i = 0; i < n; i++) CHECK_ARG(ptrow[i] <= ptrow[i + 1], "ptrow must be non-decreasing");
    for (int k = 0; k < ptrow[n]; k++) CHECK_ARG(indcol[k] >= 0 && indcol[k] < ncols, "column index outside [0, ncols)");
    SsPlanHost P;
    build_sstream_plan(n, ncols, ptrow, indcol, ss_max_padding(), P, true, shift, ghost_lo, ghost_hi);
    *eligible = P.eligible ? 1 : 0;
    if (rounds) *rounds = P.rounds;
    if (steps) *steps = P.steps;
    if (padding) *padding = ptrow[n] > 0 ? (double)P.pad_places / (double)ptrow[n] : 0.0;
    if (ghost_workgroups) *ghost_workgroups = 0;
    if (rounds_min_max) rounds_min_max[0] = rounds_min_max[1] = 0;
    if (!P.eligible) {
        g_err = std::string("not eligible: ") + P.why;
        return MI_OK;
    }
    if (const char* bad = check_sstream_plan(P, n, ptrow, indcol, ghost_lo, ghost_hi)) return fail(MI_ERR_STATE, std::string("sliced-stream plan: ") + bad);
    int gw = 0, rmin = 0x7fffffff, rmax = 0, rmax_ghost = 0, pmin = 0x7fffffff, pmax = 0;
    for (int g = 0; g < P.nwg; g++) {
        const int c = P.rptr[g + 1] - P.rptr[g];
        gw += P.wg_halo[g];
        rmin = std::min(rmin, c);
        rmax = std::max(rmax, c);
        if (P.wg_halo[g]) rmax_ghost = std::max(rmax_ghost, c);
        else { pmin = std::min(pmin, c); pmax = std::max(pmax, c); }
    }
    if (pmax > 0 && pmax - pmin > 1) return fail(MI_ERR_STATE, "sliced-stream plan: the workgroups' shares differ by more than a round");
    if (gw && gw < P.nwg && rmax > 1 && rmax_ghost >= rmax && P.rounds >= 2 * P.nwg) return fail(MI_ERR_STATE, "sliced-stream plan: a ghost-reading workgroup carries the longest share");
    if (ghost_lo < ghost_hi && !P.fusable) g_err = "eligible, but a ghost-reading workgroup's columns do not fit its first fill: the fused step keeps the ring kernel";
    if (ghost_workgroups) *ghost_workgroups = gw;
    if (rounds_min_max) { rounds_min_max[0] = rmin; rounds_min_max[1] = rmax; }
    return MI_OK;
}

extern "C" int mi_sstream_mw_plan_probe(int n, int ncols, const int* ptrow, const int* indcol, int shift, int* eligible, int* rounds, long long* steps, double* padding)
{
    CHECK_ARG(n >= 0 && ncols >= 0 && ptrow && ptrow[0] == 0 && eligible, "bad argument");
    CHECK_ARG(shift == 0 || shift == 1, "shift must be 0 or 1");
    CHECK_ARG(ptrow[n] == 0 || indcol, "indcol is null");
    for (int i = 0; i < n; i++) CHECK_ARG(ptrow[i] <= ptrow[i + 1], "ptrow must be non-decreasing");
    for (int k = 0; k < ptrow[n]; k++) CHECK_ARG(indcol[k] >= 0 && indcol[k] < ncols, "column index outside [0, ncols)");
    SsMwPlanHost P;
    build_sstream_mw_plan(n, ncols, ptrow, indcol, ss_max_padding(), P, shift);
    *eligible = P.eligible ? 1 : 0;
    if (rounds) *rounds = P.rounds;
    if (steps) *steps = P.steps;
    if (padding) *padding = ptrow[n] > 0 ? (double)P.pad_places / (double)ptrow[n] : 0.0;
    if (!P.eligible) {
        g_err = std::string("not eligible: ") + P.why;
        return MI_OK;
    }
    if (const char* bad = check_sstream_mw_plan(P, n, ptrow, indcol)) return fail(MI_ERR_STATE, std::string("cut-ring sliced-stream plan: ") + bad);
    return MI_OK;
}

extern "C" int mi_csr_block4_structure(int n, const int* ptrow, const int* indcol, int* is_blocked, long long* nblocks)
{
    CHECK_ARG(n >= 0 && ptrow && is_blocked, "bad argument");
    CHECK_ARG(ptrow[n] == 0 || indcol, "indcol is null");
    std::vector<double> dummy((size_t)ptrow[n], 0.0);
    std::vector<int> bptr, bcol;
    std::vector<double> bval;
    const bool ok = csr_to_bcsr4_exact(n, ptrow, indcol, dummy.data(), bptr, bcol, bval);
    *is_blocked = ok ? 1 : 0;
    if (nblocks) *nblocks = ok ? (long long)bcol.size() : 0;
    return MI_OK;
}

extern "C" int mi_csr_set_nontemporal(mi_csr_t A, int ring_nt, int stream_nt)
{
    CHECK_ARG(A, "null handle");
    if (A->inner) A = A->inner;
    if (ring_nt >= 0) A->ring.nt = ring_nt != 0 && A->ring.d_slots;
    if (stream_nt >= 0) A->stream_nt = stream_nt != 0;
    return MI_OK;
}

extern "C" int mi_csr_ring_info(mi_csr_t A, int* config_id, int* runs, int* runs_not_ringable, double* nnz_fraction_ringable)
{
    CHECK_ARG(A, "null handle");
    if (A->inner) A = A->inner;
    if (config_id) *config_id = A->ring.cfg.id;
    if (runs) *runs = A->ring.wgs;
    if (runs_not_ringable) *runs_not_ringable = A->ring.bad_runs;
    if (nnz_fraction_ringable) *nnz_fraction_ringable = A->ring.ok_fraction;
    return MI_OK;
}

extern "C" int mi_csr_tile_info(mi_csr_t A, int* built, int* nblk, double* unique_per_nnz, double us[2], int* nt)
{
    CHECK_ARG(A, "null handle");
    if (A->inner) A = A->inner;
    if (built) *built = A->tile.d_desc != nullptr;
    if (nblk) *nblk = A->tile.nblk;
    if (unique_per_nnz) *unique_per_nnz = A->tile.unique_per_nnz;
    if (us) {
        us[0] = A->tune_us[MI_KERNEL_TILE][0];
        us[1] = A->tune_us[MI_KERNEL_TILE][1];
    }
    if (nt) *nt = A->tile.nt;
    return MI_OK;
}

extern "C" int mi_csr_placement_info(mi_csr_t A, int* n_values, int* n_total, double* us, int cap)
{
    CHECK_ARG(A && cap >= 0 && (cap == 0 || us), "bad argument");
    if (A->inner) A = A->inner;
    if (n_values) *n_values = A->place_draws_coef;
    if (n_total) *n_total = (int)A->place_us.size();
    for (int i = 0; i < cap && i < (int)A->place_us.size(); i++) us[i] = A->place_us[i];
    return MI_OK;
}

extern "C" int mi_vec_alloc_placed(mi_csr_t A, int nvec, int draws, double** d_vecs, double* us, int cap, int* n_us)
{
    CHECK_ARG(A && nvec >= 1 && d_vecs && cap >= 0 && (cap == 0 || us), "bad argument");
    int rc = need_device();
    if (rc) return rc;
    if (n_us) *n_us = 0;
    const size_t bytes = sizeof(double) * placed_vector_len(A->n, A->ncols);
    const int npairs = (nvec + 1) / 2;
    if (draws > 64) draws = 64;
    const bool timed = draws > npairs && A->nnz >= kLargeNnz && A->n == A->ncols;
    const int cand = timed ? draws : npairs;
    std::vector<double*> xs((size_t)cand, nullptr), ys((size_t)cand, nullptr);
    auto release = [&]() {
        for (double* q : xs) if (q) (void)hipFree(q);
        for (double* q : ys) if (q) (void)hipFree(q);
    };
    for (int c = 0; c < cand; c++) {
        hipError_t e = hipSuccess;
        if (c == 0 && A->kept_x && A->kept_y) {
            xs[0] = A->kept_x.own.release();
            ys[0] = A->kept_y.own.release();
        } else {
            e = hipMalloc(&xs[c], bytes);
            if (e == hipSuccess) e = hipMalloc(&ys[c], bytes);
        }
        if (e == hipSuccess) e = hipMemset(xs[c], 0, bytes);
        if (e == hipSuccess) e = hipMemset(ys[c], 0, bytes);
        if (e != hipSuccess) {
            release();
            return fail(e == hipErrorOutOfMemory ? MI_ERR_ALLOC : MI_ERR_HIP, std::string("mi_vec_alloc_placed: ") + hipGetErrorString(e));
        }
    }
    std::vector<int> order((size_t)cand);
    for (int c = 0; c < cand; c++) order[c] = c;
    if (timed) {
        std::vector<double> t((size_t)cand, 0.0);
        int rct;
        {
            LaunchTimer tm;
            rct = tm.init();
            for (int c = 0; c < cand && !rct; c++) rct = tm.time(4, 10, [&] { return mi_spmv_dev(A, xs[c], ys[c], nullptr); }, &t[c]);
        }
        if (rct) {
            release();
            return fail(MI_ERR_HIP, "mi_vec_alloc_placed: timing a candidate pair failed");
        }
        std::stable_sort(order.begin(), order.end(), [&](int a, int b) { return t[a] < t[b]; });
        for (int c = 0; c < cand && c < cap; c++) us[c] = t[c];
        if (n_us) *n_us = std::min(cand, cap);
        for (int c = 0; c < cand; c++) (void)hipMemset(ys[c], 0, bytes);
        (void)hipDeviceSynchronize();
    }
    for (int v = 0; v < nvec; v++) {
        double*& slot = (v & 1) ? ys[order[v >> 1]] : xs[order[v >> 1]];
        d_vecs[v] = slot;
        slot = nullptr;
    }
    release();
    return MI_OK;
}

extern "C" int mi_vec_free_placed(double* d_vec)
{
    if (d_vec) HIP_TRY(hipFree(d_vec));
    return MI_OK;
}

extern "C" int mi_csr_mring_info(mi_csr_t A, int* built, int* runs, int* runs_not_served, double* nnz_fraction_served, double us[2], int* nt)
{
    CHECK_ARG(A, "null handle");
    if (A->inner) A = A->inner;
    if (built) *built = A->mring.d_plan != nullptr;
    if (runs) *runs = A->mring.nruns;
    if (runs_not_served) *runs_not_served = A->mring.bad_runs;
    if (nnz_fraction_served) *nnz_fraction_served = A->mring.ok_fraction;
    if (us) {
        us[0] = A->tune_us[MI_KERNEL_MRING][0];
        us[1] = A->tune_us[MI_KERNEL_MRING][1];
    }
    if (nt) *nt = A->mring.nt;
    return MI_OK;
}

extern "C" int mi_mring_plan_probe(int n, const int* ptrow, const int* indcol, int* nblk, int* runs, int* runs_not_served,
                                   double* nnz_fraction_served, long long* window_restarts)
{
    CHECK_ARG(n >= 0 && ptrow && ptrow[0] == 0, "bad matrix");
    CHECK_ARG(ptrow[n] == 0 || indcol, "indcol is null");
    MringPlanHost P;
    build_mring_plan(n, ptrow, indcol, P);
    if (const char* bad = check_mring_plan(P, n, ptrow, indcol)) return fail(MI_ERR_STATE, std::string("mring plan: ") + bad);
    if (nblk) *nblk = P.nblk;
    if (runs) *runs = P.nruns;
    if (runs_not_served) *runs_not_served = P.bad_runs;
    if (nnz_fraction_served) *nnz_fraction_served = ptrow[n] ? 1.0 - (double)P.bad_nnz / (double)ptrow[n] : 0.0;
    if (window_restarts) *window_restarts = P.restarts;
    return MI_OK;
}

extern "C" int mi_mring_plan_deal_probe(int n, const int* ptrow, const int* indcol, int* table_len, int* run_blocks, int cap)
{
    CHECK_ARG(n >= 0 && ptrow && ptrow[0] == 0 && table_len && cap >= 0 && (cap == 0 || run_blocks), "bad argument");
    CHECK_ARG(ptrow[n] == 0 || indcol, "indcol is null");
    MringPlanHost P;
    build_mring_plan(n, ptrow, indcol, P);
    *table_len = P.wgs;
    for (int g = 0; g < P.wgs && g < cap; g++) run_blocks[g] = P.run_rng[2 * g + 1] - P.run_rng[2 * g];
    return MI_OK;
}

extern "C" int mi_tile_plan_probe(int n, const int* ptrow, const int* indcol, int threads, int* nblk, long long* distinct_total,
                                  int* max_distinct, long long* nnz_listed)
{
    CHECK_ARG(n >= 0 && ptrow && ptrow[0] == 0, "bad matrix");
    CHECK_ARG(ptrow[n] == 0 || indcol, "indcol is null");
    TilePlanHost P;
    build_tile_plan(n, ptrow, indcol, P, kTileNnzb, threads);
    if (const char* bad = check_tile_plan(P, n, ptrow, indcol)) return fail(MI_ERR_STATE, std::string("tile plan: ") + bad);
    if (nblk) *nblk = P.nblk;
    if (distinct_total) *distinct_total = P.nblk > 0 ? (long long)P.ulist.size() - kTileThreads : 0;
    if (max_distinct) *max_distinct = P.max_unique;
    if (nnz_listed) *nnz_listed = P.listed;
    return MI_OK;
}

extern "C" int mi_ring_plan_lean(int n, const int* ptrow, const int* indcol, int config_id, int* lean)
{
    CHECK_ARG(n >= 0 && ptrow && lean && config_id >= 1 && config_id <= kNumRingConfigs, "bad argument");
    std::vector<int> row_min((size_t)n), row_max((size_t)n);
    for (int i = 0; i < n; i++) {
        int lo = 0x7fffffff, hi = -1;
        for (int k = ptrow[i]; k < ptrow[i + 1]; k++) {
            lo = std::min(lo, indcol[k]);
            hi = std::max(hi, indcol[k]);
        }
        row_min[i] = lo;
        row_max[i] = hi;
    }
    RingPlanHost P;
    build_ring_plan(kRingConfigs[config_id - 1], n, ptrow, row_min.data(), row_max.data(), P);
    *lean = P.lean && P.cfg.id == 4 && P.bad_runs == 0;
    return MI_OK;
}

extern "C" int mi_csr_ring_shape_info(mi_csr_t A, int* blocks, int* lean, int* depth, double* us_aligned, double* us_unaligned)
{
    CHECK_ARG(A, "null handle");
    if (A->inner) A = A->inner;
    if (blocks) *blocks = A->ring.nblk;
    if (lean) *lean = A->ring.lean;
    if (depth) *depth = A->ring.cfg.depth;
    if (us_aligned) *us_aligned = A->tune_us_ring_aligned;
    if (us_unaligned) *us_unaligned = A->tune_us_ring_unaligned;
    return MI_OK;
}

extern "C" int mi_csr_set_kernel(mi_csr_t A, int kernel_id)
{
    CHECK_ARG(A, "null handle");
    if (A->inner) A = A->inner;
    CHECK_ARG(kernel_id >= MI_KERNEL_AUTO && kernel_id <= MI_KERNEL_SSTREAM, "unknown kernel id");
    if (kernel_id == MI_KERNEL_SSTREAM && !A->ss.dev.val && A->nnz > 0 && A->d_indcol && !env_is("MI355_SSTREAM", "0")) {
        int rc = need_device();
        if (rc) return rc;
        std::vector<int> back((size_t)A->nnz);
        HIP_TRY(hipMemcpy(back.data(), A->d_indcol, sizeof(int) * (size_t)A->nnz, hipMemcpyDeviceToHost));
        if ((rc = build_sstream(A, A->h_ptrow.data(), back.data(), A->ghost_lo, A->ghost_hi))) return rc;
        A->ss.asked = true;
    }
    if (kernel_id == MI_KERNEL_SSTREAM && !A->ss.dev.val)
        return fail(MI_ERR_UNSUPPORTED, "MI_KERNEL_SSTREAM: the handle holds no sliced copy (the matrix pads too much or its rows do "
                                        "not fit the sliding LDS window: mi_sstream_plan_probe says which)");
    if (kernel_id == MI_KERNEL_BCSR4 && !A->blocked)
        return fail(MI_ERR_UNSUPPORTED, "MI_KERNEL_BCSR4: this matrix has no exact 4x4 block structure (or is row-mapped)");
    if (kernel_id == MI_KERNEL_TILE) {
        int rc = need_device();
        if (rc) return rc;
        if ((rc = build_tile(A, nullptr))) return rc;
    }
    if (kernel_id == MI_KERNEL_MRING) {
        int rc = need_device();
        if (rc) return rc;
        if ((rc = build_mring(A, nullptr, large_row_align(A->nnz)))) return rc;
    }
    A->kernel = kernel_id;
    HIP_TRY(hipStreamSynchronize(nullptr));
    return MI_OK;
}

extern "C" int mi_csr_get_kernel(mi_csr_t A, int* kernel_id)
{
    CHECK_ARG(A && kernel_id, "null argument");
    if (A->inner) A = A->inner;
    *kernel_id = resolve_kernel(A);
    return MI_OK;
}

extern "C" const char* mi_csr_kernel_name(mi_csr_t A)
{
    if (!A) return "";
    if (A->inner) A = A->inner;
    switch (resolve_kernel(A)) {
    case MI_KERNEL_STREAM: return A->stream_nt ? "spmv_csr_stream<1024, true>" : "spmv_csr_stream<1024, false>";
    case MI_KERNEL_RING: {
        static thread_local char nm[128];
        const RingConfig& c = A->ring.cfg;
        snprintf(nm, sizeof nm, "spmv_csr_ring<%d, %d, %d, %d, %d, %s, %s, %s, false, %s, false>", c.threads, c.nnzb, c.ring, c.depth, kRingMaxB,
                 A->d_rowmap ? "true" : "false", A->ring.nt ? "true" : "false", A->ring.skew ? "true" : "false",
                 A->ring.lean && c.threads == 256 && c.depth != 3 ? "true" : "false");
        return nm;
    }
    case MI_KERNEL_ROWPAR: return "spmv_csr_rowpar";
    case MI_KERNEL_BCSR4: {
        const mi_bcsr4_s* B = A->blocked;
        static const char* const sell_names[4] = {"spmv_bcsr4_sell<8, true, 0, 2, 4>", "spmv_bcsr4_sell<8, false, 0, 2, 4>", "spmv_bcsr4_sell<4, true, 0, 2, 8>", "spmv_bcsr4_sell<12, true, 0, 2, 4>"};
        if (B && B->sell_form >= 0 && B->sell.val) return sell_names[B->sell_form & 3];
        return B && B->use_tile && B->tl.ptr ? "spmv_bcsr4_tile<2>" : "spmv_bcsr4<2>";
    }
    case MI_KERNEL_MRING: {
        static thread_local char nm[96];
        snprintf(nm, sizeof nm, "spmv_csr_mring<%d, %d, %d, %d, %s, %s, %s>", kMringThreads, kMringNnzb, A->mring.depth, kMringMaxB,
                 A->d_rowmap ? "true" : "false", A->mring.nt ? "true" : "false", A->mring.skew ? "true" : "false");
        return nm;
    }
    case MI_KERNEL_SSTREAM: {
        static thread_local char nm[64];
        if (A->ss.mw) snprintf(nm, sizeof nm, "spmv_sstream_mw<%d, %s>", A->ss.deep ? 12 : 8, A->ss.nt ? "true" : "false");
        else snprintf(nm, sizeof nm, "spmv_sstream<%d, %s, 0>", A->ss.deep ? 12 : 8, A->ss.nt ? "true" : "false");
        return nm;
    }
    case MI_KERNEL_TILE: {
        static thread_local char nm[64];
        snprintf(nm, sizeof nm, "spmv_csr_tile<%d, %s, %s>", kTileNnzb, A->tile.nt ? "true" : "false", A->tile.skew ? "true" : "false");
        return nm;
    }
    default: return "";
    }
}
extern "C" int mi_spmv_dev(mi_csr_t A, const double* d_x, double* d_y, mi_stream_t s)
{
    CHECK_ARG(A, "null handle");
    CHECK_ARG(A->n == 0 || (d_x && d_y), "null vector");
    return launch_spmv(A, d_x, d_y, (hipStream_t)s);
}

extern "C" int mi_spmv(mi_csr_t A, const double* x, double* y)
{
    CHECK_ARG(A, "null handle");
    CHECK_ARG(A->n == 0 || (x && y), "null vector");
    if (A->mapped) return fail(MI_ERR_UNSUPPORTED, "mapped matrices are device-only (use mi_spmv_dev)");
    if (A->n == 0) return MI_OK;
    if (!A->d_x) HIP_TRY(A->d_x.alloc((size_t)(A->ncols > 0 ? A->ncols : 1)));
    if (!A->d_y) HIP_TRY(A->d_y.alloc((size_t)A->n));
    HIP_TRY(hipMemcpy(A->d_x, x, sizeof(double) * (size_t)A->ncols, hipMemcpyHostToDevice));
    int rc = launch_spmv(A, A->d_x, A->d_y, nullptr);
    if (rc) return rc;
    HIP_TRY(hipMemcpy(y, A->d_y, sizeof(double) * (size_t)A->n, hipMemcpyDeviceToHost));
    return MI_OK;
}

extern "C" int mi_spmk_dev(mi_csr_t A, int k, const double* d_x, double* const* d_y_out, mi_stream_t s)
{
    CHECK_ARG(A, "null handle");
    if (k < 1 || k > MI_MAX_POWERS) return fail(MI_ERR_UNSUPPORTED, "k must be in 1..MI_MAX_POWERS");
    CHECK_ARG(A->n == A->ncols, "matrix powers need a square matrix");
    CHECK_ARG(!A->mapped, "matrix powers need an unmapped matrix");
    CHECK_ARG(d_y_out, "null output array");
    if (A->n == 0) return MI_OK;
    for (int p = 0; p < k; p++) CHECK_ARG(d_y_out[p], "null output vector");
    if (A->inner) {
        int rc = A->d_pp.grow(k, (size_t)A->n);
        if (rc) return rc;
        double* xp = nullptr;
        if ((rc = reorder_scratch(A, (hipStream_t)s, &xp))) return rc;
        if ((rc = gather_perm(A, d_x, xp, (hipStream_t)s))) return rc;
        if ((rc = spmk_unmapped(A->inner, k, xp, A->d_pp.ptr.data(), (hipStream_t)s))) return rc;
        for (int p = 0; p < k; p++)
            if ((rc = scatter_perm(A, A->d_pp.ptr[p], d_y_out[p], (hipStream_t)s))) return rc;
        return MI_OK;
    }
    return spmk_unmapped(A, k, d_x, d_y_out, (hipStream_t)s);
}

extern "C" int mi_spmk(mi_csr_t A, int k, const double* x, double* const* y_out)
{
    CHECK_ARG(A, "null handle");
    if (k < 1 || k > MI_MAX_POWERS) return fail(MI_ERR_UNSUPPORTED, "k must be in 1..MI_MAX_POWERS");
    CHECK_ARG(A->n == A->ncols, "matrix powers need a square matrix");
    CHECK_ARG(A->n == 0 || (x && y_out), "null vector");
    if (A->n == 0) return MI_OK;
    if (!A->d_x) HIP_TRY(A->d_x.alloc((size_t)A->ncols));
    if (int rc = A->d_pow.grow(k, (size_t)A->n)) return rc;
    HIP_TRY(hipMemcpy(A->d_x, x, sizeof(double) * (size_t)A->ncols, hipMemcpyHostToDevice));
    int rc = mi_spmk_dev(A, k, A->d_x, A->d_pow.ptr.data(), nullptr);
    if (rc) return rc;
    for (int p = 0; p < k; p++) {
        CHECK_ARG(y_out[p], "null output vector");
        HIP_TRY(hipMemcpy(y_out[p], A->d_pow.ptr[p], sizeof(double) * (size_t)A->n, hipMemcpyDeviceToHost));
    }
    return MI_OK;
}
```

navierstokes_amd/csrc/capi_internal.hpp:

```cpp
#pragma once
#include "mi355_spmv.h"

#include <hip/hip_runtime.h>

#include <cstdio>
#include <cstdlib>
#include <cmath>
#include <chrono>
#include <cstring>
#include <map>
#include <memory>
#include <mutex>
#include <new>
#include <string>
#include <vector>

#include "dev_array.hpp"
#include "partition.hpp"
#include "push_exchange.hpp"
#include "ring_plan.hpp"
#include "spmv_kernels.hpp"
#include "spmv_ring.hpp"
#include "spmv_sstream_mw.hpp"

using namespace mi355;

extern thread_local std::string g_err;

static inline int fail(int code, const std::string& msg)
{
    g_err = msg;
    return code;
}

static inline int hip_fail(hipError_t e, const char* what)
{
    const int code = (e == hipErrorNoDevice || e == hipErrorInvalidDevice || e == hipErrorInsufficientDriver) ? MI_ERR_NODEVICE
                                                                                                               : (e == hipErrorOutOfMemory ? MI_ERR_ALLOC : MI_ERR_HIP);
    return fail(code, std::string(what) + ": " + hipGetErrorString(e));
}

#define HIP_TRY_AS(what, expr)                            \
    do {                                                  \
        hipError_t e_ = (expr);                           \
        if (e_ != hipSuccess) return hip_fail(e_, what);  \
    } while (0)
#define HIP_TRY(expr) HIP_TRY_AS(#expr, expr)

#define CHECK_ARG(cond, msg)                        \
    do {                                            \
        if (!(cond)) return fail(MI_ERR_ARG, msg);  \
    } while (0)


template <class T> static inline int dev_alloc(DevArray<T>& a, size_t n, size_t at_least = 0) { HIP_TRY_AS("hipMalloc", a.alloc(std::max(n, at_least))); return MI_OK; }
template <class T> static inline int dev_zeros(DevArray<T>& a, size_t n, size_t at_least = 0) { HIP_TRY_AS("hipMalloc + hipMemset", a.zeros(std::max(n, at_least))); return MI_OK; }
template <class T> static inline int dev_upload(DevArray<T>& a, const std::vector<T>& h, size_t at_least = 0) { HIP_TRY_AS("hipMalloc + hipMemcpy", a.upload(h, at_least)); return MI_OK; }
static inline int dev_alloc(MappedWord& w) { HIP_TRY_AS("hipHostMalloc (mapped)", w.alloc()); return MI_OK; }
static inline int dev_create(OwnedStream& s, unsigned flags = hipStreamDefault) { HIP_TRY_AS("hipStreamCreate", s.create(flags)); return MI_OK; }
static inline int dev_create(OwnedEvent& e, unsigned flags = hipEventDefault) { HIP_TRY_AS("hipEventCreate", e.create(flags)); return MI_OK; }

int need_device();

static inline bool env_is(const char* name, const char* value)
{
    const char* e = getenv(name);
    return e && !strcmp(e, value);
}

struct LaunchTimer {
    hipStream_t s;
    OwnedEvent e1, e0;
    explicit LaunchTimer(hipStream_t st = nullptr) : s(st) {}
    int init()
    {
        int rc;
        (rc = dev_create(e0)) || (rc = dev_create(e1));
        return rc;
    }
    template <class F>
    int time(int warm, int timed, F&& launch, double* us)
    {
        int rc;
        for (int w = 0; w < warm; w++)
            if ((rc = launch())) return rc;
        HIP_TRY(hipEventRecord(e0, s));
        for (int w = 0; w < timed; w++)
            if ((rc = launch())) return rc;
        HIP_TRY(hipEventRecord(e1, s));
        HIP_TRY(hipEventSynchronize(e1));
        float ms = 0.f;
        HIP_TRY(hipEventElapsedTime(&ms, e0, e1));
        *us = ms * 1e3 / timed;
        return MI_OK;
    }
};

struct ScratchPair {
    DevArray<double> x, y;
    ~ScratchPair() { x = {}, y = {}; }
    int alloc(size_t nx, size_t ny)
    {
        HIP_TRY(x.alloc(nx));
        HIP_TRY(y.alloc(ny));
        HIP_TRY(hipMemset(x, 0, sizeof(double) * nx));
        return MI_OK;
    }
};

static inline double min_measured(double a, double b) { return a > 0 ? std::min(a, b) : b; }
static inline bool better(double a, double b) { return a > 0 && (b <= 0 || a < b); }

static inline bool stream_is_capturing(hipStream_t s)
{
    hipStreamCaptureStatus st = hipStreamCaptureStatusNone;
    if (hipStreamIsCapturing(s, &st) != hipSuccess) {
        (void)hipGetLastError();
        return false;
    }
    return st != hipStreamCaptureStatusNone;
}

struct BlockTable {
    int nnzb = 0;
    int nblk = 0;
    DevArray<int2> d_blk;
};

struct RingTable {
    RingConfig cfg{};
    int nblk = 0, wgs = 0, bpw = 0, bad_runs = 0;
    double ok_fraction = 0.0;
    DevArray<int> d_plan;
    DevArray<int> d_ok;
    DevArray<int> d_rng;
    DevArray<int> d_run_halo;
    std::vector<int> h_run_halo;
    bool uniform = true;
    bool lean = false;
    bool all_in_loop = false;
    std::vector<int> h_dep_ptr, h_dep_run;
    DevArray<unsigned short> d_slots;
    bool nt = false;
    bool skew = false;
};

struct MringTable {
    int nblk = 0, wgs = 0, nruns = 0, bpw = 0, bad_runs = 0, depth = 2;
    double ok_fraction = 0.0;
    long long restarts = 0;
    DevArray<int> d_plan;
    DevArray<int> d_first;
    DevArray<int> d_ok;
    DevArray<int> d_rng;
    DevArray<unsigned short> d_slots;
    bool nt = false, skew = false;
};

struct TileTable {
    int nblk = 0;
    DevArray<int> d_desc;
    DevArray<unsigned> d_ulist;
    DevArray<unsigned short> d_slots;
    double unique_per_nnz = 0.0;
    bool nt = false;
    bool skew = false;
};

struct SstreamCopy {
    bool mw = false;
    SsDevice dev;
    int nwg = 0, rounds = 0;
    int shift = 0;
    long long steps = 0;
    double padding = 0.0;
    int max_slice_nnz = 0;
    bool nt = true;
    bool deep = true;
    bool fusable = false;
    bool asked = false;
    std::vector<int> h_wg_halo;
    std::vector<SsWg> h_wg;
};
struct SstreamTable : SstreamCopy {
    double tune_us[4] = {0, 0, 0, 0};
    SstreamCopy& copy() { return *this; }
};

template <class H, class Destroy = std::default_delete<H>>
struct OwnedHandle {
    std::unique_ptr<H, Destroy> own;
    operator H*() const { return own.get(); }
    H* operator->() const { return own.get(); }
    void reset(H* p = nullptr) { own.reset(p); }
};

struct DevPowers {
    std::vector<DevArray<double>> own;
    std::vector<double*> ptr;
    int grow(int k, size_t n)
    {
        while ((int)own.size() < k) {
            DevArray<double> a;
            HIP_TRY(a.alloc(n));
            ptr.push_back(a);
            own.push_back(std::move(a));
        }
        return MI_OK;
    }
    void release()
    {
        for (auto& a : own) a = {};
        own.clear(), ptr.clear();
    }
};

struct SpmkTables {
    DevArray<unsigned> flags;
    DevArray<int> dep_ptr, dep_run;
    MappedWord giveups;
};

struct SpmmTilePlan {
    int rows = 0, umax = 0, ntiles = 0;
    double mean_list = 0.0;
    DevArray<int> d_ptr;
    DevArray<unsigned> d_nodes;
    DevArray<unsigned short> d_slots;
    DevArray<int> d_rows;
};

struct Bcsr4TileLists {
    DevArray<int> ptr;
    DevArray<unsigned> nodes;
    DevArray<unsigned short> slots;
};

struct Bcsr4Sliced {
    DevArray<double> val;
    DevArray<unsigned> col;
    DevArray<int> sptr;
    DevArray<int> wrng;
    DevArray<int> wrng2;
};

struct mi_bcsr4_s {
    int device = 0;
    int nbrows = 0, nbcols = 0;
    long long nblocks = 0;
    DevArray<int> d_ptrow, d_indcol;
    DevArray<double> d_coef;
    DevArray<int> d_browmap;
    Bcsr4TileLists tl;
    bool use_tile = false;
    double tune_us_plain = 0.0, tune_us_tile = 0.0;
    Bcsr4Sliced sell;
    int sell_nslices = 0, sell_nwaves = 0, sell_nwaves2 = 0;
    long long sell_nsteps = 0;
    int max_slice_vals = 0;
    int sell_form = -1;
    double tune_us_sell[4] = {0, 0, 0, 0};
    SpmmTilePlan st, st64;
    int st_state = 0;
    int spmm_choice[9] = {0, 0, 0, 0, 0, 0, 0, 0, 0};
    double spmm_us[9][5] = {};
    DevArray<double> d_x, d_y;
    DevPowers d_pow;
    ~mi_bcsr4_s() { d_ptrow = {}, d_indcol = {}, d_coef = {}, d_browmap = {}, tl = {}, sell = {}, st = {}, st64 = {}, d_x = {}, d_y = {}, d_pow.release(); }
};


struct mi_csr_s {
    int device = 0;
    int n = 0, ncols = 0;
    long long nnz = 0;
    DevArray<int> d_ptrow, d_indcol;
    DevArray<double> d_coef;
    DevArray<int> d_rowmap;
    bool mapped = false;
    int y_offset = 0;
    int ghost_lo = 0, ghost_hi = 0;
    std::vector<int> h_ptrow;
    std::map<int, BlockTable> tables;
    RingTable ring;
    TileTable tile;
    SstreamTable ss;
    MringTable mring;
    int kernel = MI_KERNEL_AUTO;
    int auto_kernel = MI_KERNEL_STREAM;
    std::vector<double> place_us;
    int place_draws_coef = 0;
    DevArray<double> kept_x, kept_y;
    double tune_us[MI_KERNEL_SSTREAM + 1][2] = {};
    double tune_us_ring_aligned = 0.0, tune_us_ring_unaligned = 0.0;
    bool stream_nt = false;
    OwnedHandle<mi_bcsr4_s> blocked;
    int n_out = 0;
    OwnedHandle<mi_csr_s> inner;
    DevArray<int> d_iperm;
    std::vector<int> h_iperm;
    DevArray<int> d_src_start;
    DevArray<double> d_xp;
    hipStream_t xp_stream = nullptr;
    bool xp_claimed = false;
    std::map<hipStream_t, DevArray<double>> xp_more;
    DevPowers d_pp;
    DevArray<double> d_vtmp;
    double spread_before = 0.0, spread_after = 0.0, us_natural = 0.0, us_reordered = 0.0;
    int reorder_block = 0;
    DevArray<double> d_x, d_y;
    DevPowers d_pow;
    SpmkTables kstep;
    unsigned kstep_epoch = 0;
    int kstep_setup = 0;
    int kstep_choice[9] = {0, 0, 0, 0, 0, 0, 0, 0, 0};
    double kstep_us[9][2] = {};
    void drop_tables()
    {
        for (auto& kv : tables) kv.second = {};
        tables.clear();
    }
    ~mi_csr_s()
    {
        d_ptrow = {}, d_indcol = {}, d_coef = {}, d_rowmap = {}, d_x = {}, d_y = {}, kept_x = {}, kept_y = {}, d_pow.release();
        drop_tables();
        ring = {}, tile = {}, mring = {}, ss = {}, blocked.reset(), inner.reset(), d_iperm = {}, d_src_start = {}, d_xp = {};
        for (auto& kv : xp_more) kv.second = {};
        d_vtmp = {}, d_pp.release(), kstep = {};
    }
};

struct RcclCommDestroy { void operator()(void* comm) const; };
struct IpcMappingClose { void operator()(void* base) const; };
struct WinRegistryErase { void operator()(std::string* key) const; };
using RcclComm = std::unique_ptr<void, RcclCommDestroy>;
using IpcMappings = std::vector<std::unique_ptr<void, IpcMappingClose>>;
using WinRegistryEntry = std::unique_ptr<std::string, WinRegistryErase>;

struct PartRccl {
    RcclComm comm;
    OwnedStream comm_stream;
    OwnedEvent ev_pack, ev_comm;
    DevArray<double> d_sendbuf;
    unsigned step_no = 0;
    bool flag_handoff = false;
};

struct PartAllGather {
    DevArray<int> d_ag_idx;
    DevArray<int> d_ag_src;
    DevArray<double> d_ag_send;
    DevArray<double> d_ag_recv;
    int ag_slice = 0;
    bool ready() const { return d_ag_idx != nullptr; }
};

struct PushWindow {
    IpcMappings ipc_opened;
    WinRegistryEntry win_entry;
    DevArray<char> win;
    unsigned* win_flags = nullptr;
    double* win_data = nullptr;
    bool peer_on_my_device = false;
};
struct PushTables {
    DevArray<PushLink> d_links;
    DevArray<int2> d_push_work;
    DevArray<int> d_link_chunks;
    DevArray<unsigned> d_tickets;
    DevArray<int> d_nb;
    int n_links = 0, n_push_work = 0, n_nb = 0;
};
struct PartPush : PushWindow, PushTables {
    unsigned push_step = 0;
    bool push_ready = false;
    PushTables& tables() { return *this; }
};

struct PartOneLaunch {
    DevArray<int> d_run_link;
    DevArray<double> d_stage;
    DevArray<unsigned> d_ready;
    DevArray<int2> d_ext_units;
    DevArray<unsigned> d_ext_order;
    OwnedHandle<mi_csr_s> piece_all;
    const int* d_run_halo = nullptr;
    int npush_runs = 0;
    bool fused = false;
    bool ghost_readers = true;
    bool fused_ext = false;
    bool ext_csr = false;
    int ext_wgs = 0;
    int n_ext_units = 0;
    int n_ext_plain = 0;
    bool ext_split = false;
    int ext_debug = 0;
};

struct mi_part_s {
    PartPlan plan;
    OwnedHandle<mi_csr_s> piece[2];
    DevArray<int> d_send_idx;
    bool finalized = false;
    int kernel = MI_KERNEL_AUTO;
    PartRccl rccl;
    std::vector<int> ag_union;
    PartAllGather ag;
    bool ag_use = false;
    DevArray<unsigned> d_flags;
    MappedWord timeouts;
    PartPush push;
    PartOneLaunch one;
    ~mi_part_s() { piece[0].reset(), piece[1].reset(), d_send_idx = {}, rccl = {}, ag = {}, d_flags = {}, timeouts = {}, push = {}, one = {}; }
};

static inline size_t win_data_offset(int nranks) { return ((size_t)nranks * kWinFlagStride * sizeof(unsigned) + 255) / 256 * 256; }

extern std::mutex g_mu;
int get_ws(hipStream_t s, double** out);

struct Scratch {
    std::vector<DevArray<double>> bufs;
    ~Scratch()
    {
        for (auto& a : bufs) a = {};
    }
    int up(const double* h, size_t n, double** d)
    {
        *d = nullptr;
        DevArray<double> a;
        int rc = dev_alloc(a, n, 1);
        if (rc) return rc;
        *d = a;
        bufs.push_back(std::move(a));
        if (h && n) HIP_TRY(hipMemcpy(*d, h, sizeof(double) * n, hipMemcpyHostToDevice));
        return MI_OK;
    }
};

int csr_create_impl(int n, int ncols, const int* ptrow, const int* indcol, const double* coef, const int* rowmap, mi_csr_t* out,
                    int ghost_lo = 0, int ghost_hi = 0, bool defer_placement = false);
int resolve_kernel(const mi_csr_s* A);
int get_table(mi_csr_t A, int nnzb, BlockTable** out);
int launch_spmv(mi_csr_t A, const double* d_x, double* d_y, hipStream_t s, bool use_map = true, const RingComm* comm = nullptr,
                const RingDot* dot = nullptr);
bool ring_dot_eligible(const mi_csr_s* A);
int reorder_scratch(mi_csr_t A, hipStream_t s, double** buf);
void launch_ring_cfg(const mi_csr_s* A, const CsrView& V, const double* d_x, double* d_y, hipStream_t s, const RingComm* comm, const RingDot* dot);
int spmk_unmapped(mi_csr_t H, int k, const double* d_x, double* const* d_y, hipStream_t s);
int gather_perm(mi_csr_t A, const double* d_x, double* d_xp, hipStream_t s);
int ortho_update_from_parts(int n, int nparts, const double* parts, double alpha, const double* d_b, const double* d_x1, double* d_x3, double* d_beta_out,
                            hipStream_t s);
int scatter_perm(mi_csr_t A, const double* d_src, double* d_dst, hipStream_t s);
constexpr size_t kLdsBytesPerCU = 160 * 1024;
static inline size_t spmm_tile_lds(const SpmmTilePlan* T, int s) { return T ? (size_t)T->umax * (4 * s + 2) * sizeof(double) : (size_t)-1; }
hipError_t spmm_tile_launch(const mi_bcsr4_s* A, const SpmmTilePlan* Pl, const Bcsr4View& V, int s, int arith, const double* X, long long ldx,
                            double* Y, long long ldy, hipStream_t st);
hipError_t spmm_otile_launch(const mi_bcsr4_s* A, const SpmmTilePlan* Pl, const Bcsr4View& V, int s, int arith, bool nt, const double* X, long long ldx,
                             double* Y, long long ldy, hipStream_t st);
int part_push_window(mi_part_s* P);
void part_push_layout(const mi_part_s* P, long long* layout );
int part_push_connect_bases(mi_part_s* P, void* const* bases , const long long* layouts,
                            IpcMappings opened = {}, bool peer_on_my_device = false);
int part_ext_launch(mi_part_s* P, const double* d_x_ext, double* d_y_local, unsigned step, unsigned spin_max, hipStream_t s, unsigned long long* trace, int* grid_out);
int launch_sstream(mi_csr_t A, const double* d_x, double* d_y, const int* rowmap, hipStream_t s, const RingComm* comm = nullptr);
static inline bool sstream_y_ok(const mi_csr_s* A, const double* yy, const int* map) { return map || A->ss.mw || (((uintptr_t)(yy - A->ss.shift)) & 15) == 0; }
int bcsr4_values_changed(mi_bcsr4_s* A, hipStream_t s);
void bcsr4_drop_sliced(mi_bcsr4_s* A);
int bcsr4_refresh_from_csr(mi_bcsr4_s* A, const int* d_csr_ptrow, const double* d_src, double* d_csr_out, hipStream_t s);
int launch_bcsr4(mi_bcsr4_t A, const double* d_x, double* d_y, mi_stream_t s, bool use_map);
```

navierstokes_amd/csrc/spmv_sstream.hpp:

```cpp
#pragma once
#include <hip/hip_runtime.h>

#include <algorithm>
#include <thread>
#include <vector>

#include "dev_array.hpp"
#include "spmv_ring.hpp"

namespace mi355 {

typedef double ss_v2d __attribute__((ext_vector_type(2)));
constexpr int kSsRing = 8192;
constexpr int kSsSliceRows = 128;
constexpr int kSsRound = 512;
constexpr int kSsNewMax = 1024;
constexpr int kSsPark = 20;
#ifndef MI355_SS_TAIL
#define MI355_SS_TAIL 2
#endif
constexpr int kSsTail = MI355_SS_TAIL;
constexpr unsigned kSsPad = 0x8000u;
constexpr unsigned kSsFirst = 0x4000u;
constexpr int kSsPadSteps = 64;
constexpr int kSsMaxWgs = 256;
constexpr int kSsFill = 24;
constexpr int kSsGhostSlack = 3;

struct SsWg {
    int r_begin, r_end;
    int w0_lo, w0_n;
    int w1_lo, w1_n;
    int t[5];
    int halo;
    int link;
    int pad[3];
};
static_assert(sizeof(SsWg) == 64, "one record = one 64-byte scalar load");

struct SsView {
    const ss_v2d* val;
    const unsigned* slot;
    const SsWg* wg;
    const int2* win;
    int nwg, n, ncols;
    const int* rowmap;
    int shift;
    unsigned long long* trace = nullptr;
};

struct SsPlanHost {
    bool eligible = false;
    const char* why = "";
    int nwg = 0, rounds = 0, shift = 0;
    long long steps = 0, pad_places = 0;
    int max_slice_nnz = 0;
    std::vector<int> wptr, rptr, slice_step, slice_len;
    std::vector<int2> win;
    std::vector<SsWg> wg;
    std::vector<int> wg_halo;
    bool fusable = false;
    std::vector<unsigned> slot;
};

inline void build_sstream_plan(int n, int ncols, const int* ptrow, const int* indcol, double max_padding, SsPlanHost& P, bool want_slots = true, int shift = 0,
                               int ghost_lo = 0, int ghost_hi = 0)
{
    P = SsPlanHost();
    const long long nnz = n > 0 ? ptrow[n] : 0;
    if (n <= 0 || nnz <= 0) { P.why = "empty matrix"; return; }
    if (shift != 0 && shift != 1) { P.why = "bad shift"; return; }
    P.shift = shift;
    const int nv = n + shift;
    auto PT = [&](int v) { const int i = v - shift; return ptrow[i < 0 ? 0 : (i > n ? n : i)]; };
    const int rounds = (nv + kSsRound - 1) / kSsRound;
    int nwg = std::min(kSsMaxWgs, rounds);
    if (nwg >= 8) nwg = nwg / 8 * 8;
    P.nwg = nwg;
    P.rounds = rounds;
    const bool ghosts = ghost_lo < ghost_hi;
    std::vector<int> cmin((size_t)rounds, 0x7fffffff), cmax((size_t)rounds, -1);
    for (int r = 0; r < rounds; r++) {
        int lo = 0x7fffffff, hi = -1;
        for (int k = PT(r * kSsRound); k < PT(std::min(nv, (r + 1) * kSsRound)); k++) {
            lo = std::min(lo, indcol[k]);
            hi = std::max(hi, indcol[k]);
        }
        cmin[r] = lo;
        cmax[r] = hi;
    }
    auto deal = [&](const std::vector<int>& less) {
        std::vector<int> cnt((size_t)nwg, rounds / nwg);
        const int extra = rounds % nwg;
        const int per = nwg % 8 == 0 ? nwg / 8 : nwg, chunks = nwg / per;
        for (int xcd = 0; xcd < chunks; xcd++) {
            const int e = (int)((long long)extra * (xcd + 1) / chunks - (long long)extra * xcd / chunks);
            for (int j = 0; j < e; j++) cnt[(size_t)xcd * per + j]++;
        }
        int pool = 0;
        for (int g = 0; g < nwg; g++) {
            const int take = std::min(less[g], cnt[g] - 1);
            if (take > 0) { cnt[g] -= take; pool += take; }
        }
        while (pool > 0) {
            int best = -1;
            for (int g = 0; g < nwg; g++)
                if (!less[g] && (best < 0 || cnt[g] < cnt[best] || (cnt[g] == cnt[best] && g % per < best % per))) best = g;
            if (best < 0) {
                for (int g = 0; g < nwg && pool > 0; g++) { cnt[g]++; pool--; }
                break;
            }
            cnt[best]++;
            pool--;
        }
        P.rptr.assign((size_t)nwg + 1, 0);
        for (int g = 0; g < nwg; g++) P.rptr[g + 1] = P.rptr[g] + cnt[g];
    };
    std::vector<char> too_wide((size_t)nwg, 0);
    auto windows = [&]() -> bool {
        P.win.assign((size_t)rounds, make_int2(0, 0));
        P.wg_halo.assign((size_t)nwg, 0);
        std::fill(too_wide.begin(), too_wide.end(), 0);
        for (int g = 0; g < nwg; g++) {
            int allmin = 0x7fffffff;
            for (int r = P.rptr[g]; r < P.rptr[g + 1]; r++) allmin = std::min(allmin, cmin[r]);
            int whi = 0, wlo = 0;
            for (int r = P.rptr[g]; r < P.rptr[g + 1]; r++) {
                const int nhi = std::max(whi, cmax[r] + 1);
                if (r == P.rptr[g]) {
                    const int lo = std::max(std::max(0, nhi - kSsRing), std::min(allmin, nhi));
                    P.win[r] = make_int2(lo, nhi - lo);
                    wlo = lo;
                } else {
                    P.win[r] = make_int2(whi, nhi - whi);
                    if (nhi - whi > kSsNewMax) { P.why = "a round brings more new columns than the window takes in at once"; return false; }
                }
                whi = nhi;
                if (cmin[r] != 0x7fffffff && cmin[r] < whi - kSsRing) { P.why = "a round's rows reach further apart than the LDS ring holds"; return false; }
            }
            if (ghosts && whi > wlo && (wlo < ghost_lo || whi > ghost_hi)) {
                P.wg_halo[g] = 1;
                if (whi - wlo > kSsRing) too_wide[g] = 1;
                else {
                    P.win[P.rptr[g]] = make_int2(wlo, whi - wlo);
                    for (int r = P.rptr[g] + 1; r < P.rptr[g + 1]; r++) P.win[r] = make_int2(whi, 0);
                }
            }
        }
        return true;
    };
    std::vector<int> less((size_t)nwg, 0);
    deal(less);
    if (!windows()) return;
    if (ghosts)
        for (int it = 0; it < 64; it++) {
            std::vector<int> want = less;
            bool changed = false;
            for (int g = 0; g < nwg; g++) {
                if (!P.wg_halo[g]) continue;
                const int need = too_wide[g] ? std::max(less[g] + 1, kSsGhostSlack) : std::max(less[g], kSsGhostSlack);
                if (need != less[g]) { want[g] = need; changed = true; }
            }
            if (!changed) break;
            less = want;
            deal(less);
            if (!windows()) return;
        }
    P.fusable = ghosts;
    for (int g = 0; g < nwg; g++)
        if (P.wg_halo[g] && too_wide[g]) P.fusable = false;
    P.wptr.assign((size_t)nwg * 4 + 1, 0);
    P.slice_step.assign((size_t)rounds * 4, 0);
    P.slice_len.assign((size_t)rounds * 4, 0);
    long long t = 0, places = 0;
    for (int g = 0; g < nwg; g++)
        for (int wv = 0; wv < 4; wv++) {
            P.wptr[(size_t)g * 4 + wv] = (int)t;
            for (int r = P.rptr[g]; r < P.rptr[g + 1]; r++) {
                const int row0 = r * kSsRound + wv * kSsSliceRows;
                int L = 1;
                for (int v = row0; v < std::min(nv, row0 + kSsSliceRows); v++) L = std::max(L, PT(v + 1) - PT(v));
                if (row0 < nv) P.max_slice_nnz = std::max(P.max_slice_nnz, PT(std::min(nv, row0 + kSsSliceRows)) - PT(row0));
                P.slice_step[(size_t)r * 4 + wv] = (int)t;
                P.slice_len[(size_t)r * 4 + wv] = L;
                t += L;
                places += (long long)L * kSsSliceRows;
            }
        }
    P.wptr[(size_t)nwg * 4] = (int)t;
    P.steps = t;
    P.pad_places = places - nnz;
    if (t + kSsPadSteps >= 0x7fffffffLL / 64) { P.why = "too many steps for 32-bit offsets"; return; }
    if ((double)P.pad_places > max_padding * (double)nnz) { P.why = "row lengths vary too much inside the 128-row slices (padding)"; return; }
    P.wg.assign((size_t)nwg, SsWg());
    for (int g = 0; g < nwg; g++) {
        SsWg& W = P.wg[g];
        W.r_begin = P.rptr[g];
        W.r_end = P.rptr[g + 1];
        if (W.r_begin < W.r_end) {
            const int2 w0 = P.win[W.r_begin], w1 = P.win[std::min(W.r_begin + 1, W.r_end - 1)];
            W.w0_lo = w0.x;
            W.w0_n = w0.y;
            W.w1_lo = w1.x;
            W.w1_n = w1.y;
        }
        for (int k = 0; k < 5; k++) W.t[k] = P.wptr[(size_t)g * 4 + k];
        W.halo = P.wg_halo[g];
        W.link = -1;
    }
    P.eligible = true;
    if (!want_slots) return;
    P.slot.assign((size_t)(t + kSsPadSteps) * 64, kSsPad | (kSsPad << 16) | kSsFirst);
    auto fill = [&](int r0, int r1) {
        for (int r = r0; r < r1; r++)
            for (int wv = 0; wv < 4; wv++) {
                const int row0 = r * kSsRound + wv * kSsSliceRows;
                const size_t base = (size_t)P.slice_step[(size_t)r * 4 + wv] * 64;
                const int L = P.slice_len[(size_t)r * 4 + wv];
                for (int j = 0; j < L; j++)
                    for (int l = 0; l < 64; l++) {
                        unsigned s = 0;
                        for (int h = 0; h < 2; h++) {
                            const int v = row0 + 2 * l + h;
                            unsigned sh = kSsPad;
                            if (v < nv && j < PT(v + 1) - PT(v)) sh = (unsigned)(indcol[PT(v) + j] & (kSsRing - 1));
                            s |= sh << (16 * h);
                        }
                        if (j == 0) s |= kSsFirst;
                        P.slot[base + (size_t)j * 64 + l] = s;
                    }
            }
    };
    unsigned nt = std::thread::hardware_concurrency();
    nt = nt > 16 ? 16 : (nt < 1 ? 1 : nt);
    if (rounds < 64 || nt == 1) fill(0, rounds);
    else {
        std::vector<std::thread> th;
        for (unsigned k = 0; k < nt; k++) th.emplace_back(fill, (int)((long long)rounds * k / nt), (int)((long long)rounds * (k + 1) / nt));
        for (std::thread& x : th) x.join();
    }
}

inline const char* check_sstream_plan(const SsPlanHost& P, int n, const int* ptrow, const int* indcol, int ghost_lo = 0, int ghost_hi = 0)
{
    if (!P.eligible) return nullptr;
    const int shift = P.shift, nv = n + shift;
    auto PT = [&](int v) { const int i = v - shift; return ptrow[i < 0 ? 0 : (i > n ? n : i)]; };
    if (P.rptr[0] != 0 || P.rptr[P.nwg] != P.rounds) return "the workgroups' rounds do not cover the matrix";
    for (int g = 0; g < P.nwg; g++) {
        int wlo = 0, whi = 0;
        const SsWg& W = P.wg[g];
        if (W.r_begin != P.rptr[g] || W.r_end != P.rptr[g + 1] || W.r_end < W.r_begin) return "a workgroup record disagrees with the round table";
        for (int k = 0; k < 5; k++)
            if (W.t[k] != P.wptr[(size_t)g * 4 + k]) return "a workgroup record disagrees with the stream table";
        if (W.r_begin < W.r_end) {
            const int2 w0 = P.win[W.r_begin], w1 = P.win[std::min(W.r_begin + 1, W.r_end - 1)];
            if (W.w0_lo != w0.x || W.w0_n != w0.y || W.w1_lo != w1.x || W.w1_n != w1.y) return "a workgroup record disagrees with the window table";
        }
        bool names_ghost = false;
        for (int r = P.rptr[g]; r < P.rptr[g + 1]; r++) {
            const int2 w = P.win[r];
            if (r == P.rptr[g]) { wlo = w.x; whi = w.x + w.y; }
            else {
                if (w.x != whi) return "a round's new columns do not continue the window";
                whi += w.y;
                if (w.y > kSsNewMax) return "too many new columns";
            }
            wlo = std::max(wlo, whi - kSsRing);
            for (int wv = 0; wv < 4; wv++) {
                const int row0 = r * kSsRound + wv * kSsSliceRows;
                const size_t base = (size_t)P.slice_step[(size_t)r * 4 + wv] * 64;
                int L = 1;
                for (int v = row0; v < std::min(nv, row0 + kSsSliceRows); v++) L = std::max(L, PT(v + 1) - PT(v));
                if (L != P.slice_len[(size_t)r * 4 + wv]) return "slice length disagrees with the rows";
                for (int j = 0; j < L; j++)
                    for (int l = 0; l < 64; l++) {
                        const unsigned s = P.slot[base + (size_t)j * 64 + l];
                        if (l == 0 && ((s & kSsFirst) != 0) != (j == 0)) return "slice-begin flag misplaced";
                        for (int h = 0; h < 2; h++) {
                            const int v = row0 + 2 * l + h;
                            const unsigned sh = (s >> (16 * h)) & 0xffffu;
                            const bool real = v < nv && j < PT(v + 1) - PT(v);
                            if (!real) {
                                if (!(sh & kSsPad)) return "a padding place is not flagged";
                                continue;
                            }
                            const int c = indcol[PT(v) + j];
                            if (sh & kSsPad) return "a nonzero is flagged as padding";
                            if ((sh & (kSsRing - 1)) != (unsigned)(c & (kSsRing - 1))) return "slot is not the column's ring slot";
                            if (c < wlo || c >= whi) return "a column lies outside the window when its round runs";
                            names_ghost = names_ghost || (ghost_lo < ghost_hi && (c < ghost_lo || c >= ghost_hi));
                        }
                    }
            }
        }
        if (names_ghost && !P.wg_halo[g]) return "a workgroup names a ghost column and is not marked";
        if (P.fusable && P.wg_halo[g])
            for (int r = P.rptr[g] + 1; r < P.rptr[g + 1]; r++)
                if (P.win[r].y != 0) return "a ghost-reading workgroup takes columns in after its first fill";
        if (W.halo != P.wg_halo[g]) return "a workgroup record's ghost mark disagrees with the plan's";
    }
    return nullptr;
}

template <int CAP>
__global__ __launch_bounds__(256) void sstream_fill_kernel(int nslices, int n, int shift, const int* __restrict__ ptrow, const double* __restrict__ src,
                                                           double* __restrict__ csr_out, const int* __restrict__ slice_step, const int* __restrict__ slice_len,
                                                           ss_v2d* __restrict__ val, int pair64)
{
    __shared__ double buf[CAP > 0 ? CAP : 1];
    __shared__ int rp[kSsSliceRows + 1];
    const int tid = threadIdx.x;
    for (int sidx = blockIdx.x; sidx < nslices; sidx += gridDim.x) {
        const int row0 = kSsSliceRows * sidx - shift;
        if (tid <= kSsSliceRows) rp[tid] = ptrow[max(0, min(row0 + tid, n))];
        __syncthreads();
        const int base = rp[0], seg = rp[kSsSliceRows] - base;
        const bool staged = CAP > 0 && seg <= CAP;
        if (staged) {
            for (int k = tid; k < seg; k += 256) {
                const double v = src[base + k];
                buf[k] = v;
                if (csr_out) csr_out[base + k] = v;
            }
            __syncthreads();
        } else if (csr_out) {
            for (int k = tid; k < seg; k += 256) csr_out[base + k] = src[base + k];
        }
        const int t0 = slice_step[sidx], L = slice_len[sidx];
        for (int q = tid; q < L * 64; q += 256) {
            const int j = q >> 6, lane = q & 63;
            const int ra = pair64 ? lane : 2 * lane, rb = pair64 ? lane + 64 : 2 * lane + 1;
            const int a0 = rp[ra], a1 = rp[ra + 1], b0 = rp[rb], b1 = rp[rb + 1];
            ss_v2d v = {0.0, 0.0};
            if (j < a1 - a0) v.x = staged ? buf[a0 - base + j] : src[a0 + j];
            if (j < b1 - b0) v.y = staged ? buf[b0 - base + j] : src[b0 + j];
            val[(size_t)(t0 + j) * 64 + lane] = v;
        }
        __syncthreads();
    }
}

inline void sstream_fill_values(int rounds, int n, int shift, const int* d_ptrow, const double* d_src, double* d_csr_out, const int* d_slice_step,
                                const int* d_slice_len, ss_v2d* d_val, int max_slice_nnz, hipStream_t s, int pair64 = 0)
{
    const int nslices = 4 * rounds;
    if (nslices <= 0) return;
    if (max_slice_nnz <= 2048)
        hipLaunchKernelGGL((sstream_fill_kernel<2048>), dim3((unsigned)std::min(nslices, 2048)), dim3(256), 0, s, nslices, n, shift, d_ptrow, d_src, d_csr_out, d_slice_step, d_slice_len, d_val, pair64);
    else if (max_slice_nnz <= 8192)
        hipLaunchKernelGGL((sstream_fill_kernel<8192>), dim3((unsigned)std::min(nslices, 1024)), dim3(256), 0, s, nslices, n, shift, d_ptrow, d_src, d_csr_out, d_slice_step, d_slice_len, d_val, pair64);
    else
        hipLaunchKernelGGL((sstream_fill_kernel<0>), dim3((unsigned)std::min(nslices, 2048)), dim3(256), 0, s, nslices, n, shift, d_ptrow, d_src, d_csr_out, d_slice_step, d_slice_len, d_val, pair64);
}

struct SsDevice {
    DevArray<int2> winK;
    DevArray<ss_v2d> val;
    DevArray<unsigned> slot;
    DevArray<SsWg> wg;
    DevArray<int2> win;
    DevArray<int> slice_step, slice_len;
    DevArray<int> wg_halo;
};
inline hipError_t ss_upload(const SsPlanHost& P, SsDevice& Dv, bool ghosts)
{
    hipError_t e;
    const size_t vsteps = (size_t)(P.steps + kSsPadSteps) * 64;
    if ((e = Dv.val.alloc(vsteps)) != hipSuccess || (e = Dv.slot.alloc(P.slot.size())) != hipSuccess || (e = Dv.wg.alloc(P.wg.size())) != hipSuccess ||
        (e = Dv.win.alloc(P.win.size())) != hipSuccess || (e = Dv.slice_step.alloc(P.slice_step.size())) != hipSuccess ||
        (e = Dv.slice_len.alloc(P.slice_len.size())) != hipSuccess || (ghosts && (e = Dv.wg_halo.alloc(P.wg_halo.size())) != hipSuccess) ||
        (e = hipMemset(Dv.val + (size_t)P.steps * 64, 0, sizeof(ss_v2d) * (size_t)kSsPadSteps * 64)) != hipSuccess ||
        (e = Dv.slot.fill(P.slot)) != hipSuccess || (e = Dv.wg.fill(P.wg)) != hipSuccess || (e = Dv.win.fill(P.win)) != hipSuccess ||
        (e = Dv.slice_step.fill(P.slice_step)) != hipSuccess || (e = Dv.slice_len.fill(P.slice_len)) != hipSuccess ||
        (ghosts && (e = Dv.wg_halo.fill(P.wg_halo)) != hipSuccess))
        Dv = {};
    return e;
}

template <int D, bool NT, int ABL, int MODE>
__device__ __forceinline__ void ss_body(const SsView& S, const SsWg& W, int g, const double* __restrict__ x_in, double* __restrict__ y, const RingComm& C,
                                        double* ring , ss_v2d* s_park )
{
    constexpr bool GHOSTS = MODE == 2;
    const int tid = threadIdx.x, lane = tid & 63;
    const int wv = __builtin_amdgcn_readfirstlane(tid >> 6);
    const double* __restrict__ x = MODE != 0 ? x_in - C.n_left : x_in;
    const int r_begin = W.r_begin, r_end = W.r_end;
    if ((ABL & 8) && tid == 0) S.trace[4 * g] = __builtin_amdgcn_s_memrealtime();
    if (GHOSTS && W.link >= 0 && C.npush_runs > 0)
        for (int l = W.link; l < C.n_links; l += C.npush_runs) ring_push_link<256>(C, x_in, l);
    ss_v2d* park = s_park + wv * kSsPark * 64 + lane;
    int parked = 0, park_first = 0;
    const int t0 = wv == 0 ? W.t[0] : (wv == 1 ? W.t[1] : (wv == 2 ? W.t[2] : W.t[3]));
    const int t_end = wv == 0 ? W.t[1] : (wv == 1 ? W.t[2] : (wv == 2 ? W.t[3] : W.t[4]));
    const int clast = S.ncols - 1;
    const int cfirst = MODE != 0 ? C.n_left : 0;
    const int cowned = MODE != 0 ? C.n_left + C.n_local - 1 : clast;
    const ss_v2d* vb = S.val + lane;
    const unsigned* sb = S.slot + lane;
    ss_v2d a[D];
    unsigned sl[D];
    auto first_steps = [&]() {
#pragma unroll
        for (int d = 0; d < D; d++) {
            a[d] = NT ? __builtin_nontemporal_load(vb + (size_t)(t0 + d) * 64) : vb[(size_t)(t0 + d) * 64];
            sl[d] = sb[(size_t)(t0 + d) * 64];
        }
    };
    if (GHOSTS) {
        first_steps();
        push_wait_flags(C.flags, C.nb, C.n_nb, C.step, 0u, C.timeouts, C.spin_max, tid, 256);
        __syncthreads();
        __builtin_amdgcn_fence(__ATOMIC_ACQUIRE, "");
    }
    int r = r_begin;
    double nx[kSsNewMax / 256];
    int2 wn = make_int2(W.w1_lo, W.w1_n);
    {
        double fx[kSsFill];
#pragma unroll
        for (int u = 0; u < kSsFill; u++) fx[u] = GHOSTS ? ring_ldx<true>(x_in, C, min(W.w0_lo + tid + 256 * u, clast)) : x[min(W.w0_lo + tid + 256 * u, cowned)];
#pragma unroll
        for (int u = 0; u < kSsNewMax / 256; u++) nx[u] = (ABL & 4) ? 0.0 : x[min(max(wn.x + tid + 256 * u, cfirst), cowned)];
        if (!GHOSTS) first_steps();
#pragma unroll
        for (int u = 0; u < kSsFill; u++) {
            const int c = W.w0_lo + tid + 256 * u;
            if (c < W.w0_lo + W.w0_n) ring[c & (kSsRing - 1)] = fx[u];
        }
        for (int c0 = W.w0_lo + 256 * kSsFill + tid; c0 < W.w0_lo + W.w0_n; c0 += 256 * 8) {
            double f8[8];
#pragma unroll
            for (int u = 0; u < 8; u++) f8[u] = GHOSTS ? ring_ldx<true>(x_in, C, min(c0 + 256 * u, clast)) : x[min(c0 + 256 * u, cowned)];
#pragma unroll
            for (int u = 0; u < 8; u++)
                if (c0 + 256 * u < W.w0_lo + W.w0_n) ring[(c0 + 256 * u) & (kSsRing - 1)] = f8[u];
        }
    }
    __syncthreads();
    if ((ABL & 8) && tid == 0) S.trace[4 * g + 1] = __builtin_amdgcn_s_memrealtime();
    double acc0 = 0.0, acc1 = 0.0;
    auto store = [&](int round, ss_v2d v) {
        const int v0 = round * kSsRound + wv * kSsSliceRows + 2 * lane;
        if ((ABL & 2) && v.x != 123.456) return;
        if (S.rowmap) {
            const int i = v0 - S.shift;
            if (i >= 0 && v0 < S.n) y[S.rowmap[i]] = v.x;
            if (v0 + 1 < S.n) y[S.rowmap[i + 1]] = v.y;
        } else if (v0 >= S.shift && v0 + 1 < S.n) *reinterpret_cast<ss_v2d*>(y + v0) = v;
        else {
            if (v0 >= S.shift && v0 < S.n) y[v0] = v.x;
            if (v0 + 1 < S.n) y[v0 + 1] = v.y;
        }
    };
    auto flush = [&]() {
        for (int j = 0; j < parked; j++) store(park_first + j, park[j * 64]);
        parked = 0;
    };
    auto emit = [&]() {
        if (parked == 0) park_first = r;
        park[parked * 64] = ss_v2d{acc0, acc1};
        if (++parked == kSsPark || r == r_end - 1 - kSsTail) flush();
    };
    for (int t = t0; t < t_end; t += D) {
#pragma unroll
        for (int d = 0; d < D; d++) {
            const int i = t + d;
            if (i < t_end) {
                const unsigned s = sl[d];
                if ((__builtin_amdgcn_readfirstlane(s) & kSsFirst) && i != t0) {
                    emit();
                    acc0 = acc1 = 0.0;
                    r++;
                    __syncthreads();
                    if (!(ABL & 4)) {
#pragma unroll
                        for (int u = 0; u < kSsNewMax / 256; u++) {
                            const int c = wn.x + tid + 256 * u;
                            if (c < wn.x + wn.y) ring[c & (kSsRing - 1)] = nx[u];
                        }
                    }
                    __syncthreads();
                    if (!(ABL & 4)) {
                        wn = S.win[min(r + 1, r_end - 1)];
#pragma unroll
                        for (int u = 0; u < kSsNewMax / 256; u++) nx[u] = x[min(max(wn.x + tid + 256 * u, cfirst), cowned)];
                    }
                }
                const double x0 = (ABL & 1) ? 1.0 + lane : ring[s & (kSsRing - 1)], x1 = (ABL & 1) ? 0.5 : ring[(s >> 16) & (kSsRing - 1)];
                const double n0 = fma(a[d].x, x0, acc0), n1 = fma(a[d].y, x1, acc1);
                acc0 = (s & kSsPad) ? acc0 : n0;
                acc1 = (s & (kSsPad << 16)) ? acc1 : n1;
            }
            a[d] = NT ? __builtin_nontemporal_load(vb + (size_t)(i + D) * 64) : vb[(size_t)(i + D) * 64];
            sl[d] = sb[(size_t)(i + D) * 64];
        }
    }
    if ((ABL & 8) && tid == 0) S.trace[4 * g + 2] = __builtin_amdgcn_s_memrealtime();
    emit();
    flush();
    if (ABL & 8) {
        asm volatile("s_waitcnt vmcnt(0)" ::: "memory");
        __syncthreads();
        if (tid == 0) S.trace[4 * g + 3] = __builtin_amdgcn_s_memrealtime();
    }
}

__device__ __forceinline__ int ss_logical_wg(const SsView& S, int bid)
{
    const int per = S.nwg >> 3;
    return per > 0 && (S.nwg & 7) == 0 ? (bid & 7) * per + (bid >> 3) : bid;
}

template <int D, bool NT, int ABL = 0>
__global__ __launch_bounds__(256) void spmv_sstream(SsView S, const double* __restrict__ x, double* __restrict__ y)
{
    const int g = ss_logical_wg(S, (int)blockIdx.x);
    const SsWg W = S.wg[g];
    if (W.r_begin >= W.r_end) return;
    __shared__ double ring[kSsRing];
    __shared__ ss_v2d s_park[4 * kSsPark * 64];
    ss_body<D, NT, ABL, 0>(S, W, g, x, y, RingComm{}, ring, s_park);
}

template <int D, bool NT, int ABL = 0>
__global__ __launch_bounds__(256) void spmv_sstream_fused(SsView S, const double* __restrict__ x, double* __restrict__ y, RingComm C)
{
    if ((int)blockIdx.x < C.push_wgs) {
        if ((int)blockIdx.x < C.n_links) ring_push_gate<256>(C);
        for (int l = blockIdx.x; l < C.n_links; l += C.push_wgs) ring_push_link<256>(C, x, l);
        return;
    }
    const int g = ss_logical_wg(S, (int)blockIdx.x - C.push_wgs);
    const SsWg W = S.wg[g];
    if (W.r_begin >= W.r_end) return;
    __shared__ double ring[kSsRing];
    __shared__ ss_v2d s_park[4 * kSsPark * 64];
    if (W.halo) ss_body<D, NT, ABL, 2>(S, W, g, x, y, C, ring, s_park);
    else ss_body<D, NT, ABL, 1>(S, W, g, x, y, C, ring, s_park);
}

}
```

navierstokes_amd/mpk.py:

```python
from __future__ import annotations

import ctypes
import os

import numpy as np

_HERE = os.path.dirname(os.path.abspath(__file__))
LIB_PATH = os.environ.get("MI355_SPMV_LIBRARY") or os.path.join(_HERE, "csrc", "libmi355spmv.so")

MI_OK = 0
KERNEL_AUTO, KERNEL_STREAM, KERNEL_RING, KERNEL_ROWPAR = 0, 1, 2, 3
KERNELS = {"auto": 0, "stream": 1, "ring": 2, "rowpar": 3, "bcsr4": 4, "tile": 5, "mring": 6, "sstream": 7}

_c = ctypes
_vp = ctypes.c_void_p
_LIB = None


class MiError(RuntimeError):
    def __init__(self, status, detail):
        super().__init__(f"libmi355spmv status {status}: {detail}")
        self.status = status


def lib():
    global _LIB
    if _LIB is not None:
        return _LIB
    if not os.path.exists(LIB_PATH):
        raise RuntimeError(
            f"{LIB_PATH} is missing — the HIP extension was not built. Run "
            "`python -c 'import __graft_entry__ as g; g.build()'` (needs hipcc). "
            "There is no CPU fallback for this path."
        )
    try:
        import torch
    except Exception:
        pass
    L = ctypes.CDLL(LIB_PATH)
    L.mi_strerror.restype = _c.c_char_p
    L.mi_last_error.restype = _c.c_char_p
    L.mi_csr_kernel_name.restype = _c.c_char_p
    L.mi_csr_kernel_name.argtypes = [_vp]
    i, ll, d = _c.c_int, _c.c_longlong, _c.c_double
    P = _c.POINTER
    sigs = {
        "mi_version": [],
        "mi_device_count": [P(i)],
        "mi_set_device": [i],
        "mi_device_synchronize": [],
        "mi_flush_cache": [],
        "mi_flush_cache_async": [_vp],
        "mi_csr_create": [i, i, _vp, _vp, _vp, P(_vp)],
        "mi_csr_create_mapped": [i, i, _vp, _vp, _vp, _vp, P(_vp)],
        "mi_csr_destroy": [_vp],
        "mi_csr_update_values": [_vp, _vp],
        "mi_csr_update_values_dev": [_vp, _vp, _vp],
        "mi_bcsr4_update_values": [_vp, _vp],
        "mi_bcsr4_update_values_dev": [_vp, _vp, _vp],
        "mi_orthonormalize_against_basis": [i, i, _vp, _vp, _vp],
        "mi_orthonormalize_against_basis_dev": [i, i, _vp, _vp, _vp, _vp],
        "mi_mdot": [i, i, _vp, _vp, _vp],
        "mi_mdot_dev": [i, i, _vp, _vp, _vp, _vp],
        "mi_maxpy": [i, i, _vp, i, _vp, _vp],
        "mi_maxpy_dev": [i, i, _vp, i, _vp, _vp, _vp, _vp],
        "mi_cgs_dev": [i, i, _vp, _vp, i, _vp, _vp, _vp],
        "mi_part_status": [_vp],
        "mi_part_push_export": [_vp, _vp, _vp],
        "mi_part_push_connect": [_vp, _vp, _vp],
        "mi_part_spmv_push_dev": [_vp, _vp, _vp, _vp],
        "mi_part_push_info": [_vp, P(i), P(i), P(i)],
        "mi_part_sends_contiguous": [_vp, P(i)],
        "mi_part_combined_info": [_vp, P(i)],
        "mi_part_push_disable": [_vp],
        "mi_part_push_unfuse": [_vp],
        "mi_bcsr4_spmm": [_vp, i, _vp, ll, _vp, ll, i],
        "mi_bcsr4_spmm_info": [_vp, i, P(i), P(i), P(i), P(d)],
        "mi_bcsr4_spmm_dev": [_vp, i, _vp, ll, _vp, ll, i, _vp],
        "mi_spmm_dev": [_vp, i, _vp, ll, _vp, ll, _vp],
        "mi_krylov_basis_dev": [_vp, i, _vp, _vp, ll, i, _vp, _vp],
        "mi_krylov_basis_cgs_dev": [_vp, i, _vp, _vp, ll, i, _vp, _vp],
        "mi_csr_reorder_info": [_vp, P(i), P(i), P(d), P(d), P(d), P(d)],
        "mi_reorder_probe": [i, _vp, _vp, P(i), _vp, P(d), P(d)],
        "mi_csr_perm": [_vp, P(i), _vp],
        "mi_vec_to_internal_dev": [_vp, _vp, _vp, _vp],
        "mi_vec_from_internal_dev": [_vp, _vp, _vp, _vp],
        "mi_spmv_internal_dev": [_vp, _vp, _vp, _vp],
        "mi_spmk_internal_dev": [_vp, i, _vp, _vp, _vp],
        "mi_csr_dims": [_vp, P(i), P(i), P(ll)],
        "mi_csr_set_kernel": [_vp, i],
        "mi_csr_get_kernel": [_vp, P(i)],
        "mi_csr_ring_info": [_vp, P(i), P(i), P(i), P(d)],
        "mi_csr_ring_shape_info": [_vp, P(i), P(i), P(i), P(d), P(d)],
        "mi_csr_tune_info": [_vp, P(d), P(d)],
        "mi_csr_tune_detail": [_vp, P(d), P(_c.c_int), P(_c.c_int)],
        "mi_csr_set_nontemporal": [_vp, i, i],
        "mi_csr_block4_structure": [i, _vp, _vp, P(i), P(_c.c_longlong)],
        "mi_ring_plan_probe": [i, _vp, _vp, i, P(i), P(i), P(i), P(d), P(i)],
        "mi_ring_plan_lean": [i, _vp, _vp, i, P(i)],
        "mi_csr_tile_info": [_vp, P(i), P(i), P(d), P(d), P(i)],
        "mi_bcsr4_tile_info": [_vp, P(i), P(i), P(d), P(d)],
        "mi_bcsr4_sell_info": [_vp, P(i), P(i), P(ll), P(d), P(d)],
        "mi_bcsr4_sell_plan_probe": [i, _vp, _vp, i, P(i), P(ll), P(i), _vp, _vp, _vp],
        "mi_bcsr4_spmm_plan_probe": [i, _vp, _vp, i, i, P(i), P(i), P(i), P(d), _vp, ll, _vp, ll, _vp, ll, _vp, ll],
        "mi_csr_mring_info": [_vp, P(i), P(i), P(i), P(d), P(d), P(i)],
        "mi_csr_sstream_info": [_vp, P(i), P(i), P(ll), P(d), P(d), P(i)],
        "mi_sstream_plan_probe": [i, i, _vp, _vp, P(i), P(i), P(ll), P(d)],
        "mi_sstream_plan_probe_ex": [i, i, _vp, _vp, i, i, i, P(i), P(i), P(ll), P(d), P(i), P(i)],
        "mi_sstream_mw_plan_probe": [i, i, _vp, _vp, i, P(i), P(i), P(ll), P(d)],
        "mi_csr_placement_info": [_vp, P(i), P(i), P(d), i],
        "mi_vec_alloc_placed": [_vp, i, i, P(_vp), P(d), i, P(i)],
        "mi_vec_free_placed": [_vp],
        "mi_mring_plan_deal_probe": [i, _vp, _vp, P(i), _vp, i],
        "mi_mring_plan_probe": [i, _vp, _vp, P(i), P(i), P(i), P(d), P(ll)],
        "mi_tile_plan_probe": [i, _vp, _vp, i, P(i), P(ll), P(i), P(ll)],
        "mi_stream_read_probe": [ll, i, P(d)],
        "mi_spmv": [_vp, _vp, _vp],
        "mi_spmv_dev": [_vp, _vp, _vp, _vp],
        "mi_spmk": [_vp, i, _vp, _vp],
        "mi_spmk_dev": [_vp, i, _vp, _vp, _vp],
        "mi_csr_spmk_info": [_vp, i, P(i), P(i), P(d), P(d)],
        "mi_spmk_plan_probe": [i, _vp, _vp, P(i), P(i), P(i)],
        "mi_dot": [i, _vp, _vp, P(d)],
        "mi_dot_dev": [i, _vp, _vp, _vp, _vp],
        "mi_axpy": [i, d, _vp, _vp],
        "mi_axpy_dev": [i, d, _vp, _vp, _vp],
        "mi_orthogonalize": [i, _vp, _vp, _vp, d, P(d)],
        "mi_orthogonalize_dev": [i, _vp, _vp, _vp, d, _vp, _vp],
        "mi_spmv_dot_dev": [_vp, _vp, _vp, _vp, _vp, _vp],
        "mi_csr_dot_epilogue_info": [_vp, P(i)],
        "mi_csr_dot_epilogue_layout": [_vp, P(i), P(i), P(i), _vp, _vp, _vp, i, i],
        "mi_spmv_orthogonalize_dev": [_vp, _vp, _vp, _vp, _vp, d, _vp, _vp],
        "mi_norm2": [i, _vp, P(d)],
        "mi_norm2_dev": [i, _vp, _vp, _vp],
        "mi_rel_error": [i, _vp, _vp, P(d)],
        "mi_rel_error_dev": [i, _vp, _vp, _vp, _vp],
        "mi_gather_dev": [i, _vp, _vp, _vp, _vp],
        "mi_bcsr4_create": [i, i, _vp, _vp, _vp, P(_vp)],
        "mi_bcsr4_destroy": [_vp],
        "mi_bcsr4_create_layout": [i, i, _vp, _vp, _vp, i, P(_vp)],
        "mi_bcsr4_update_values_layout": [_vp, _vp, i],
        "mi_bcsr4_update_values_layout_dev": [_vp, _vp, i, _vp],
        "mi_bcsr4_spmv": [_vp, _vp, _vp],
        "mi_bcsr4_spmv_dev": [_vp, _vp, _vp, _vp],
        "mi_bcsr4_spmk": [_vp, i, _vp, _vp],
        "mi_bcsr4_spmk_dev": [_vp, i, _vp, _vp, _vp],
        "mi_bilu4_create": [i, _vp, _vp, _vp, i, i, P(_vp)],
        "mi_bilu4_create_host": [i, _vp, _vp, _vp, i, i, P(_vp)],
        "mi_bilu4_destroy": [_vp],
        "mi_bilu4_refactor": [_vp, _vp, i],
        "mi_bilu4_solve_dev": [_vp, _vp, _vp, _vp],
        "mi_bilu4_solve": [_vp, _vp, _vp],
        "mi_bilu4_info": [_vp, P(i), P(ll), P(i), P(i), P(i), P(i), P(d), P(d), P(ll)],
        "mi_bilu4_factor_host": [_vp, _vp, _vp, _vp, _vp, ll],
        "mi_bilu4_plan_probe": [i, _vp, _vp, i, P(ll), P(i), P(i), P(i), P(i), _vp, _vp, i],
        "mi_bilu4dev_plan_probe": [i, _vp, _vp, i, P(ll), P(i), P(ll)],
        "mi_bilu4dev_prepare": [_vp],
        "mi_bilu4dev_refactor": [_vp, _vp, i, _vp],
        "mi_bilu4dev_status": [_vp, P(i)],
        "mi_bilu4dev_fetch": [_vp],
        "mi_bilu4dev_info": [_vp, P(i), P(i), P(ll)],
        "mi_bilu4one_plan_probe": [i, _vp, _vp, i, i, P(i), _vp, _vp, P(ll), _vp, _vp, _vp, _vp],
        "mi_bilu4one_prepare": [_vp],
        "mi_bilu4_set_solve_form": [_vp, i],
        "mi_bilu4one_status": [_vp],
        "mi_bilu4one_info": [_vp, P(i), P(i), P(i), _vp, _vp, P(ll)],
        "mi_bilu4sw_prepare": [_vp],
        "mi_bilu4sw_solve_dev": [_vp, _vp, _vp, i, i, _vp],
        "mi_bilu4sw_solve": [_vp, _vp, _vp, i, i],
        "mi_bilu4sw_info": [_vp, P(i), P(i), P(i), P(i), P(ll)],
        "mi_bilu4sp_prepare": [_vp],
        "mi_bilu4sp_solve_dev": [_vp, _vp, _vp, i, i, _vp],
        "mi_bilu4sp_solve": [_vp, _vp, _vp, i, i],
        "mi_bilu4sp_status": [_vp, P(i), P(ll)],
        "mi_bilu4sp_fetch": [_vp, _vp, ll],
        "mi_bilu4sp_info": [_vp, P(i), P(i), P(i), P(ll)],
        "mi_part_create": [i, i, _vp, _vp, _vp, _vp, P(_vp)],
        "mi_part_destroy": [_vp],
        "mi_part_sizes": [_vp, P(i), P(i), P(i), P(i)],
        "mi_part_recv_counts": [_vp, _vp],
        "mi_part_recv_ids": [_vp, i, _vp],
        "mi_part_set_send_ids": [_vp, i, i, _vp],
        "mi_part_send_counts": [_vp, _vp],
        "mi_part_local_csr": [_vp, i, P(i), P(_vp), P(_vp), P(_vp), P(_vp)],
        "mi_part_send_index": [_vp, P(i), P(_vp)],
        "mi_part_finalize": [_vp],
        "mi_part_set_kernel": [_vp, i],
        "mi_part_update_values": [_vp, _vp],
        "mi_part_pack_dev": [_vp, _vp, _vp, _vp],
        "mi_part_spmv_interior_dev": [_vp, _vp, _vp, _vp],
        "mi_part_spmv_boundary_dev": [_vp, _vp, _vp, _vp],
        "mi_comm_available": [],
        "mi_comm_unique_id": [_vp],
        "mi_part_comm_init": [_vp, _vp],
        "mi_part_comm_info": [_vp, P(i), P(i)],
        "mi_part_spmv_dev": [_vp, _vp, _vp, _vp],
        "mi_comm_selftest": [i, P(d)],
        "mi_part_send_union": [_vp, P(i), P(_vp)],
        "mi_part_allgather_setup": [_vp, _vp, _vp],
        "mi_part_set_allgather": [_vp, i],
        "mi_part_allgather_info": [_vp, P(i), P(i), P(i)],
        "mi_dist_create": [i, i, _vp, _vp, _vp, P(_vp)],
        "mi_dist_destroy": [_vp],
        "mi_dist_info": [_vp, P(i), P(i), P(i), P(i), P(ll), P(ll)],
        "mi_dist_rank_info": [_vp, i, P(i), P(ll), P(i), P(i), P(ll), P(_vp)],
        "mi_dist_update_values": [_vp, _vp],
        "mi_dist_spmv": [_vp, _vp, _vp],
        "mi_dist_spmk": [_vp, i, _vp, _vp],
        "mi_dist_dot": [_vp, _vp, _vp, P(d)],
        "mi_dist_orthogonalize": [_vp, _vp, _vp, _vp, d, P(d)],
        "mi_dist_vec_create": [_vp, P(_vp)],
        "mi_dist_vec_destroy": [_vp],
        "mi_dist_vec_set": [_vp, _vp],
        "mi_dist_vec_get": [_vp, _vp],
        "mi_dist_vec_ptr": [_vp, i, P(_vp)],
        "mi_dist_spmv_dev": [_vp, _vp, _vp],
        "mi_dist_spmk_dev": [_vp, i, _vp, _vp],
        "mi_dist_synchronize": [_vp],
        "mi_dist_dot_dev": [_vp, _vp, _vp, P(d)],
        "mi_dist_orthogonalize_dev": [_vp, _vp, _vp, _vp, d, P(d)],
    }
    for name, argt in sigs.items():
        fn = getattr(L, name)
        fn.argtypes = argt
        fn.restype = _c.c_int
    for name in ("mi_dist_exchange_name", "mi_dist_exchange_note"):
        getattr(L, name).argtypes = [_vp]
        getattr(L, name).restype = _c.c_char_p
    L.mi_part_kernel_name.argtypes = [_vp, i]
    L.mi_part_kernel_name.restype = _c.c_char_p
    for name, argt in {"mi_debug_xcc_map": [i, _vp], "mi_debug_touch_pages": [_vp, i, _vp, ll, _vp, ll],
                       "mi_part_push_debug_preset": [_vp, _c.c_uint], "mi_debug_part_push_trace": [_vp, _vp, _vp, i, _vp, P(i), _vp],
                       "mi_debug_part_ext_mode": [_vp, i], "mi_debug_part_ext_trace": [_vp, _vp, _vp, i, _vp, P(i), _vp]}.items():
        if hasattr(L, name):
            fn = getattr(L, name)
            fn.argtypes = argt
            fn.restype = _c.c_int
    _LIB = L
    return L


def check(status):
    if status != MI_OK:
        raise MiError(status, lib().mi_last_error().decode(errors="replace"))



def _is_torch(t):
    return type(t).__module__.startswith("torch")


def _stream_ptr():
    import torch

    return _vp(torch.cuda.current_stream().cuda_stream)


def _dev_ptr(t, n=None, what="vector"):
    import torch

    if not (t.is_cuda and t.dtype == torch.float64 and t.is_contiguous()):
        raise TypeError(f"{what}: expected a contiguous float64 CUDA tensor, got {t.dtype} on {t.device}")
    if n is not None and t.numel() < n:
        raise ValueError(f"{what}: needs {n} entries, has {t.numel()}")
    return _vp(t.data_ptr())


def _host_f64(a, n=None, what="vector", writable=False):
    if not isinstance(a, np.ndarray) or a.dtype != np.float64 or not a.flags.c_contiguous:
        if writable:
            raise TypeError(f"{what}: output must be a C-contiguous float64 numpy array")
        a = np.ascontiguousarray(a, dtype=np.float64)
    if n is not None and a.size < n:
        raise ValueError(f"{what}: needs {n} entries, has {a.size}")
    return a



class csrmatrix:

    def __init__(self, n, ptrow, indcol, coef, ncols=None, rowmap=None):
        self.n = int(n)
        self.ptrow = np.ascontiguousarray(ptrow, dtype=np.int32)
        self.indcol = np.ascontiguousarray(indcol, dtype=np.int32)
        self.coef = np.ascontiguousarray(coef, dtype=np.float64)
        if len(self.ptrow) != self.n + 1:
            raise ValueError("ptrow must have n+1 entries")
        self.nnz = int(self.ptrow[-1]) if self.n > 0 else 0
        self.ncols = self.n if ncols is None else int(ncols)
        self.rowmap = None if rowmap is None else np.ascontiguousarray(rowmap, dtype=np.int32)
        self._h = None
        self._kernel = KERNEL_AUTO

    @property
    def handle(self):
        if self._h is None:
            h = _vp()
            if self.rowmap is None:
                check(lib().mi_csr_create(self.n, self.ncols, self.ptrow.ctypes.data, self.indcol.ctypes.data,
                                          self.coef.ctypes.data, _c.byref(h)))
            else:
                check(lib().mi_csr_create_mapped(self.n, self.ncols, self.ptrow.ctypes.data, self.indcol.ctypes.data,
                                                 self.coef.ctypes.data, self.rowmap.ctypes.data, _c.byref(h)))
            self._h = h
            if self._kernel != KERNEL_AUTO:
                check(lib().mi_csr_set_kernel(h, self._kernel))
        return self._h

    def set_kernel(self, kernel):
        kid = KERNELS[kernel] if isinstance(kernel, str) else int(kernel)
        self._kernel = kid
        if self._h is not None:
            check(lib().mi_csr_set_kernel(self._h, kid))
        return self

    def kernel_name(self):
        return lib().mi_csr_kernel_name(self.handle).decode()

    def ring_info(self):
        cfg, runs, bad = _c.c_int(), _c.c_int(), _c.c_int()
        frac = _c.c_double()
        check(lib().mi_csr_ring_info(self.handle, _c.byref(cfg), _c.byref(runs), _c.byref(bad), _c.byref(frac)))
        return cfg.value, runs.value, bad.value, frac.value

    def ring_shape_info(self):
        b, l, dd = _c.c_int(), _c.c_int(), _c.c_int()
        ua, uu = _c.c_double(), _c.c_double()
        check(lib().mi_csr_ring_shape_info(self.handle, _c.byref(b), _c.byref(l), _c.byref(dd), _c.byref(ua), _c.byref(uu)))
        return dict(blocks=b.value, lean=bool(l.value), depth=dd.value, us_aligned=ua.value, us_unaligned=uu.value)

    def tune_info(self):
        a, b = _c.c_double(), _c.c_double()
        check(lib().mi_csr_tune_info(self.handle, _c.byref(a), _c.byref(b)))
        return a.value, b.value

    def tune_detail(self):
        us = (_c.c_double * 5)()
        rnt, snt = _c.c_int(), _c.c_int()
        check(lib().mi_csr_tune_detail(self.handle, us, _c.byref(rnt), _c.byref(snt)))
        nt = rnt.value if "ring" in self.kernel_name() else snt.value
        out = dict(ring=us[0], ring_nt=us[1], stream=us[2], stream_nt=us[3], bcsr4=us[4])
        m = self.mring_info()
        if m["built"]:
            out.update(mring=m["us"], mring_nt=m["us_nt"])
            if "mring" in self.kernel_name():
                nt = m["nt"]
        t = self.tile_info()
        if t["built"]:
            out.update(tile=t["us"], tile_nt=t["us_nt"])
            if "tile" in self.kernel_name():
                nt = t["nt"]
        return out, bool(nt)

    def placement_info(self):
        nv, nt = _c.c_int(), _c.c_int()
        us = (_c.c_double * 32)()
        check(lib().mi_csr_placement_info(self.handle, _c.byref(nv), _c.byref(nt), us, 32))
        return dict(values=[round(us[k], 2) for k in range(nv.value)], column_stream=[round(us[k], 2) for k in range(nv.value, nt.value)])

    def alloc_vectors(self, nvec=2, draws=8):
        import torch
        ptrs = (_vp * nvec)()
        us = (_c.c_double * 64)()
        nus = _c.c_int()
        check(lib().mi_vec_alloc_placed(self.handle, nvec, draws, ptrs, us, 64, _c.byref(nus)))
        out = []
        for k in range(nvec):
            buf = _PlacedBuffer(int(ptrs[k]), max(self.n, self.ncols))
            t = torch.as_tensor(buf, device="cuda")[: self.n]
            t._placed = buf
            out.append(t)
        return out, [round(us[k], 2) for k in range(nus.value)]

    def mring_info(self):
        b, r, bad, nt = _c.c_int(), _c.c_int(), _c.c_int(), _c.c_int()
        f = _c.c_double()
        us = (_c.c_double * 2)()
        check(lib().mi_csr_mring_info(self.handle, _c.byref(b), _c.byref(r), _c.byref(bad), _c.byref(f), us, _c.byref(nt)))
        return dict(built=bool(b.value), runs=r.value, runs_not_served=bad.value, nnz_fraction=f.value, us=us[0], us_nt=us[1],
                    nt=bool(nt.value))

    def sstream_info(self):
        b, r, fm = _c.c_int(), _c.c_int(), _c.c_int()
        st = _c.c_longlong()
        pad = _c.c_double()
        us = (_c.c_double * 4)()
        check(lib().mi_csr_sstream_info(self.handle, _c.byref(b), _c.byref(r), _c.byref(st), _c.byref(pad), us, _c.byref(fm)))
        return dict(built=bool(b.value), rounds=r.value, steps=st.value, padding=pad.value, us_d8_nt=us[0], us_d8_temporal=us[1], us_d12_nt=us[2],
                    us_d12_temporal=us[3], form=fm.value)

    def tile_info(self):
        b, nb, nt = _c.c_int(), _c.c_int(), _c.c_int()
        u = _c.c_double()
        us = (_c.c_double * 2)()
        check(lib().mi_csr_tile_info(self.handle, _c.byref(b), _c.byref(nb), _c.byref(u), us, _c.byref(nt)))
        return dict(built=bool(b.value), nblk=nb.value, unique_per_nnz=u.value, us=us[0], us_nt=us[1], nt=bool(nt.value))

    def reorder_info(self):
        r, b = _c.c_int(), _c.c_int()
        v = [_c.c_double() for _ in range(4)]
        check(lib().mi_csr_reorder_info(self.handle, _c.byref(r), _c.byref(b), *[_c.byref(t) for t in v]))
        return dict(reordered=bool(r.value), block=b.value, spread_before=v[0].value, spread_after=v[1].value,
                    us_natural=v[2].value, us_reordered=v[3].value)

    def spmk_info(self, k):
        e, o = _c.c_int(), _c.c_int()
        a, b = _c.c_double(), _c.c_double()
        check(lib().mi_csr_spmk_info(self.handle, int(k), _c.byref(e), _c.byref(o), _c.byref(a), _c.byref(b)))
        return dict(eligible=bool(e.value), one_launch=bool(o.value), us_k_launches=a.value, us_one_launch=b.value)

    def dot_in_epilogue(self):
        r = _c.c_int()
        check(lib().mi_csr_dot_epilogue_info(self.handle, _c.byref(r)))
        return bool(r.value)

    def dot_epilogue_layout(self):
        t, w, nb = _c.c_int(), _c.c_int(), _c.c_int()
        check(lib().mi_csr_dot_epilogue_layout(self.handle, _c.byref(t), _c.byref(w), _c.byref(nb), None, None, None, 0, 0))
        first = np.zeros(w.value + 1, np.int32)
        row0 = np.zeros(max(nb.value, 1), np.int32)
        rows = np.zeros(max(nb.value, 1), np.int32)
        check(lib().mi_csr_dot_epilogue_layout(self.handle, _c.byref(t), _c.byref(w), _c.byref(nb), first.ctypes.data,
                                               row0.ctypes.data, rows.ctypes.data, first.size, row0.size))
        return dict(threads=t.value, run_first_block=first, block_row0=row0[: nb.value], block_rows=rows[: nb.value])

    def perm(self):
        r = _c.c_int()
        p = np.empty(self.n, np.int32)
        check(lib().mi_csr_perm(self.handle, _c.byref(r), p.ctypes.data))
        return bool(r.value), p

    def to_internal(self, x, out=None):
        import torch
        out = torch.empty_like(x) if out is None else out
        check(lib().mi_vec_to_internal_dev(self.handle, _dev_ptr(x, self.n, "x"), _dev_ptr(out, self.n, "x_int"), _stream_ptr()))
        return out

    def from_internal(self, x_int, out=None):
        import torch
        out = torch.empty_like(x_int) if out is None else out
        check(lib().mi_vec_from_internal_dev(self.handle, _dev_ptr(x_int, self.n, "x_int"), _dev_ptr(out, self.n, "x"), _stream_ptr()))
        return out

    def update_values(self, coef):
        if _is_torch(coef):
            check(lib().mi_csr_update_values_dev(self.handle, _dev_ptr(coef, self.nnz, "coef"), _stream_ptr()))
        else:
            self.coef = _host_f64(coef, self.nnz, "coef")
            check(lib().mi_csr_update_values(self.handle, self.coef.ctypes.data))
        return self

    def drop_host_arrays(self):
        _ = self.handle
        self.indcol = self.indcol[:0]
        self.coef = self.coef[:0]

    def close(self):
        if self._h is not None:
            lib().mi_csr_destroy(self._h)
            self._h = None

    def __del__(self):
        try:
            self.close()
        except Exception:
            pass


class bcsr4x4_matrix:

    def __init__(self, nrows, ptrow, indcol, coef, nbcols=None, layout="row"):
        self.layout = {"row": 0, "col": 1}[layout]
        self.nrows = int(nrows)
        self.ptrow = np.ascontiguousarray(ptrow, dtype=np.int32)
        self.indcol = np.ascontiguousarray(indcol, dtype=np.int32)
        self.coef = np.ascontiguousarray(coef, dtype=np.float64)
        self.nblocks = len(self.indcol)
        self.nbcols = (int(self.indcol.max()) + 1 if self.nblocks else 0) if nbcols is None else int(nbcols)
        self.nbcols = max(self.nbcols, self.nrows)
        self._h = None

    @property
    def handle(self):
        if self._h is None:
            h = _vp()
            check(lib().mi_bcsr4_create_layout(self.nrows, self.nbcols, self.ptrow.ctypes.data, self.indcol.ctypes.data,
                                               self.coef.ctypes.data, self.layout, _c.byref(h)))
            self._h = h
        return self._h

    def update_values(self, coef):
        if _is_torch(coef):
            check(lib().mi_bcsr4_update_values_layout_dev(self.handle, _dev_ptr(coef, 16 * self.nblocks, "coef"), self.layout, _stream_ptr()))
        else:
            self.coef = _host_f64(coef, 16 * self.nblocks, "coef")
            check(lib().mi_bcsr4_update_values_layout(self.handle, self.coef.ctypes.data, self.layout))
        return self

    def close(self):
        if self._h is not None:
            lib().mi_bcsr4_destroy(self._h)
            self._h = None

    def __del__(self):
        try:
            self.close()
        except Exception:
            pass


class bilu4:

    def __init__(self, A, ptrow=None, indcol=None, coef=None, fill=0, layout="row", host_only=False):
        if isinstance(A, bcsr4x4_matrix):
            nbrows, ptrow, indcol, coef, lay = A.nrows, A.ptrow, A.indcol, A.coef, A.layout
        else:
            nbrows, lay = int(A), {"row": 0, "col": 1}[layout]
        self.nbrows = int(nbrows)
        self.layout = lay
        self.fill = int(fill)
        ptrow = np.ascontiguousarray(ptrow, dtype=np.int32)
        indcol = np.ascontiguousarray(indcol, dtype=np.int32)
        coef = _host_f64(coef, None, "coef")
        if len(ptrow) != self.nbrows + 1:
            raise ValueError("ptrow must have nbrows+1 entries")
        if coef.size < 16 * len(indcol):
            raise ValueError("coef: 16 values per block")
        self._nblocks_in = len(indcol)
        self._h = None
        h = _vp()
        make = lib().mi_bilu4_create_host if host_only else lib().mi_bilu4_create
        check(make(self.nbrows, ptrow.ctypes.data, indcol.ctypes.data, coef.ctypes.data, lay, self.fill, _c.byref(h)))
        self._h = h

    @property
    def handle(self):
        if self._h is None:
            raise ValueError("bilu4: closed")
        return self._h

    def solve(self, x, b):
        n = 4 * self.nbrows
        if _is_torch(b):
            check(lib().mi_bilu4_solve_dev(self.handle, _dev_ptr(b, n, "b"), _dev_ptr(x, n, "x"), _stream_ptr()))
        else:
            xx = _host_f64(x, n, "x", writable=True)
            check(lib().mi_bilu4_solve(self.handle, _host_f64(b, n, "b").ctypes.data, xx.ctypes.data))
        return x

    def refactor(self, coef):
        coef = _host_f64(coef, 16 * self._nblocks_in, "coef")
        check(lib().mi_bilu4_refactor(self.handle, coef.ctypes.data, self.layout))
        return self

    def prepare_dev(self):
        check(lib().mi_bilu4dev_prepare(self.handle))
        return self

    def refactor_dev(self, coef):
        check(lib().mi_bilu4dev_refactor(self.handle, _dev_ptr(coef, 16 * self._nblocks_in, "coef"), self.layout, _stream_ptr()))
        return self

    def factor_status(self):
        bad = _c.c_int()
        check(lib().mi_bilu4dev_status(self.handle, _c.byref(bad)))
        return self

    def fetch_factor(self):
        check(lib().mi_bilu4dev_fetch(self.handle))
        return self

    def info_dev(self):
        pr, la, by = _c.c_int(), _c.c_int(), _c.c_longlong()
        check(lib().mi_bilu4dev_info(self.handle, _c.byref(pr), _c.byref(la), _c.byref(by)))
        return dict(prepared=bool(pr.value), launches=la.value, plan_bytes=by.value)

    def set_form(self, form):
        check(lib().mi_bilu4_set_solve_form(self.handle, int(form)))
        return self.info()["form"]

    def prepare_one(self):
        check(lib().mi_bilu4one_prepare(self.handle))
        return self

    def one_status(self):
        check(lib().mi_bilu4one_status(self.handle))
        return self

    def info_one(self):
        pr, el, wg, by = _c.c_int(), _c.c_int(), _c.c_int(), _c.c_longlong()
        nch, md = (_c.c_int * 2)(), (_c.c_int * 2)()
        check(lib().mi_bilu4one_info(self.handle, _c.byref(pr), _c.byref(el), _c.byref(wg), nch, md, _c.byref(by)))
        return dict(prepared=bool(pr.value), eligible=bool(el.value), workgroups=wg.value, nchunks=(nch[0], nch[1]), max_deps=(md[0], md[1]),
                    plan_bytes=by.value)

    def sweeps(self, fwd, bwd=None, precision="f64"):
        return bilu4_sweeps(self, fwd, fwd if bwd is None else bwd, precision)

    def prepare_sweeps(self, precision="f64"):
        check((lib().mi_bilu4sp_prepare if _sweep_precision(precision) else lib().mi_bilu4sw_prepare)(self.handle))
        return self

    def sweep_status_f32(self):
        bad, cnt = _c.c_int(), _c.c_longlong()
        status = lib().mi_bilu4sp_status(self.handle, _c.byref(bad), _c.byref(cnt))
        try:
            check(status)
        except MiError as e:
            e.bad_block_row, e.overflowed = bad.value, cnt.value
            raise
        return self

    def fetch_f32(self):
        nblk = self.info()["nblocks"]
        val = np.zeros((max(nblk, 1), 4, 4), np.float32)
        check(lib().mi_bilu4sp_fetch(self.handle, val.ctypes.data, max(nblk, 1)))
        return val[:nblk]

    def sweep_info_f32(self):
        pr, cv, la, by = _c.c_int(), _c.c_int(), _c.c_int(), _c.c_longlong()
        check(lib().mi_bilu4sp_info(self.handle, _c.byref(pr), _c.byref(cv), _c.byref(la), _c.byref(by)))
        return dict(prepared=bool(pr.value), convert_launches=cv.value, launches_last=la.value, copy_bytes=by.value)

    def sweep_info(self):
        pr, mf, mb, la, by = _c.c_int(), _c.c_int(), _c.c_int(), _c.c_int(), _c.c_longlong()
        check(lib().mi_bilu4sw_info(self.handle, _c.byref(pr), _c.byref(mf), _c.byref(mb), _c.byref(la), _c.byref(by)))
        return dict(prepared=bool(pr.value), max_fwd=mf.value, max_bwd=mb.value, launches_last=la.value, work_bytes=by.value)

    def info(self):
        nb, fl, bl, la, fo = (_c.c_int() for _ in range(5))
        nblk, by = _c.c_longlong(), _c.c_longlong()
        us = (_c.c_double * 2)()
        fs = _c.c_double()
        check(lib().mi_bilu4_info(self.handle, _c.byref(nb), _c.byref(nblk), _c.byref(fl), _c.byref(bl), _c.byref(la), _c.byref(fo), us,
                                  _c.byref(fs), _c.byref(by)))
        return dict(nbrows=nb.value, nblocks=nblk.value, fwd_levels=fl.value, bwd_levels=bl.value, launches=la.value, form=fo.value,
                    us_per_level_launches=us[0], us_one_launch=us[1], factor_seconds=fs.value, factor_bytes=by.value)

    def factor_host(self):
        nblk = self.info()["nblocks"]
        ptr = np.zeros(self.nbrows + 1, np.int32)
        col = np.zeros(max(nblk, 1), np.int32)
        diag = np.zeros(max(self.nbrows, 1), np.int32)
        val = np.zeros((max(nblk, 1), 4, 4), np.float64)
        check(lib().mi_bilu4_factor_host(self.handle, ptr.ctypes.data, col.ctypes.data, diag.ctypes.data, val.ctypes.data, max(nblk, 1)))
        return ptr, col[:nblk], diag[: self.nbrows], val[:nblk]

    def close(self):
        if self._h is not None:
            lib().mi_bilu4_destroy(self._h)
            self._h = None

    def __del__(self):
        try:
            self.close()
        except Exception:
            pass


def _sweep_precision(precision):
    if precision not in ("f64", "f32"):
        raise ValueError('bilu4: precision must be "f64" or "f32"')
    return precision == "f32"


class bilu4_sweeps:

    def __init__(self, F, fwd, bwd, precision="f64"):
        self.F, self.fwd, self.bwd, self.precision = F, int(fwd), int(bwd), precision
        self._f32 = _sweep_precision(precision)
        if self.fwd < 0 or self.bwd < 0:
            raise ValueError("bilu4.sweeps: negative sweep count")

    def solve(self, x, b):
        n = 4 * self.F.nbrows
        L = lib()
        if _is_torch(b):
            dev = L.mi_bilu4sp_solve_dev if self._f32 else L.mi_bilu4sw_solve_dev
            check(dev(self.F.handle, _dev_ptr(b, n, "b"), _dev_ptr(x, n, "x"), self.fwd, self.bwd, _stream_ptr()))
        else:
            xx = _host_f64(x, n, "x", writable=True)
            host = L.mi_bilu4sp_solve if self._f32 else L.mi_bilu4sw_solve
            check(host(self.F.handle, _host_f64(b, n, "b").ctypes.data, xx.ctypes.data, self.fwd, self.bwd))
        return x


def bilu4_plan_probe(nbrows, ptrow, indcol, fill=0):
    ptrow = np.ascontiguousarray(ptrow, dtype=np.int32)
    indcol = np.ascontiguousarray(indcol, dtype=np.int32)
    nblk = _c.c_longlong()
    fl, bl, fa, ba = (_c.c_int() for _ in range(4))
    cap = max(int(nbrows), 1)
# ... 600 lines not shown
```

Before: 1252.

## Pack sliced-stream column indices as 12-bit row-relative offsets

Adds a packed column stream for the sliced SpMV kernel. Each nonzero's column is stored as a 12-bit offset from its row, three 32-bit words per four steps, instead of 16-bit ring slots in a 32-bit word per step. Row boundaries come from slice lengths rather than a flag bit in each slot. This cuts index bytes per nonzero in a bandwidth-bound kernel. In exchange it adds bit-unpacking work, applies only when every nonzero is within 2047 columns of its row and there are no ghost columns, and is chosen at create time by timing packed against unpacked.

New measurement: 1241. About the same (-0.9%).

```diff
diff --git a/include/mi355_spmv.h b/include/mi355_spmv.h
--- a/include/mi355_spmv.h
+++ b/include/mi355_spmv.h
@@ -74,6 +74,10 @@
 int mi_vec_alloc_placed(mi_csr_t A, int nvec, int draws, double** d_vecs, double* us, int cap, int* n_us);
 int mi_vec_free_placed(double* d_vec);
 int mi_csr_sstream_info(mi_csr_t A, int* built, int* rounds, long long* steps, double* padding, double us[4], int* form);
+int mi_csr_sstream_pack_info(mi_csr_t A, int* built, int* slots_built, int* in_use, int* eligible, const char** reason, long long* groups,
+                             double* us_packed, double* us_unpacked, double* stream_bytes_per_nnz);
+int mi_csr_sstream_set_packed(mi_csr_t A, int packed);
+int mi_sstream_pack_probe(int n, int ncols, const int* ptrow, const int* indcol, int shift, int* eligible, long long* groups, int* max_dist);
 int mi_sstream_plan_probe(int n, int ncols, const int* ptrow, const int* indcol, int* eligible, int* rounds, long long* steps, double* padding);
 int mi_sstream_plan_probe_ex(int n, int ncols, const int* ptrow, const int* indcol, int shift, int ghost_lo, int ghost_hi, int* eligible, int* rounds,
                              long long* steps, double* padding, int* ghost_workgroups, int* rounds_min_max);
diff --git a/navierstokes_amd/csrc/capi_csr.hip b/navierstokes_amd/csrc/capi_csr.hip
--- a/navierstokes_amd/csrc/capi_csr.hip
+++ b/navierstokes_amd/csrc/capi_csr.hip
@@ -32,7 +32,36 @@
     return kSsMaxPadding;
 }
 
-static int build_sstream(mi_csr_t A, const int* ptrow, const int* indcol, int ghost_lo = 0, int ghost_hi = 0)
+static int ss_pack_env()
+{
+    const char* e = getenv("MI355_SSTREAM_PACKED");
+    return !e ? -1 : (atoi(e) != 0 ? 1 : 0);
+}
+
+static int build_sstream_columns(mi_csr_t A, SstreamCopy& T, const int* ptrow, const int* indcol, bool want_pack, const SsPlanHost* have = nullptr)
+{
+    if (!T.dev.val || T.mw || (want_pack ? T.dev.pack != nullptr : T.dev.slot != nullptr)) return MI_OK;
+    SsPlanHost mine;
+    if (!have) {
+        build_sstream_plan(A->n, A->ncols, ptrow, indcol, 1e300, mine, !want_pack, T.shift, A->ghost_lo, A->ghost_hi);
+        if (!mine.eligible || mine.steps != T.steps || mine.nwg != T.nwg) return fail(MI_ERR_STATE, "sliced copy: its plan cannot be rebuilt from the handle's pattern");
+        have = &mine;
+    }
+    if (!want_pack) {
+        HIP_TRY(T.dev.slot.upload(have->slot));
+        return MI_OK;
+    }
+    SsPackHost K;
+    build_sstream_pack(*have, A->n, ptrow, indcol, A->ghost_lo < A->ghost_hi, K);
+    A->ss.pack_eligible = K.eligible ? 1 : 0;
+    A->ss.pack_why = K.why;
+    if (!K.eligible) return MI_OK;
+    HIP_TRY(T.dev.pack.upload(K.code));
+    T.groups = K.groups;
+    return MI_OK;
+}
+
+static int build_sstream(mi_csr_t A, const int* ptrow, const int* indcol, int ghost_lo = 0, int ghost_hi = 0, bool for_race = false)
 {
     if (A->ss.dev.val) return MI_OK;
     SsPlanHost P;
@@ -41,7 +70,14 @@
     build_sstream_plan(A->n, A->ncols, ptrow, indcol, ss_max_padding(), P, true, shift, ghost_lo, ghost_hi);
     SstreamCopy T;
     hipError_t e;
+    const int pack_env = ss_pack_env();
+    auto not_packed = [&](const char* why) {
+        A->ss.pack_eligible = 0;
+        A->ss.pack_why = why;
+        return pack_env == 1 ? fail(MI_ERR_UNSUPPORTED, std::string("MI355_SSTREAM_PACKED=1: ") + why) : MI_OK;
+    };
     if (!P.eligible) {
+        if (int rc = not_packed(kSsPackWhyPlan)) return rc;
         if (ghost_lo < ghost_hi || env_is("MI355_SSTREAM_MW", "0")) return MI_OK;
         build_sstream_mw_plan(A->n, A->ncols, ptrow, indcol, ss_max_padding(), M, shift);
         if (!M.eligible) return MI_OK;
@@ -76,15 +112,49 @@
         T.nt = (f & 1) == 0;
         T.deep = f >= 2;
     }
+    if (P.eligible && ghost_lo < ghost_hi) {
+        if (int rc = not_packed(kSsPackWhyGhosts)) return rc;
+    } else if (P.eligible && (pack_env == 1 || (pack_env < 0 && for_race && !getenv("MI355_SSTREAM_FORM")))) {
+        if (int rc = build_sstream_columns(A, T, ptrow, indcol, true, &P)) return rc;
+        if (!T.dev.pack) {
+            if (int rc = not_packed(A->ss.pack_why)) return rc;
+        } else if (pack_env == 1) {
+            T.packed = true;
+            T.dev.slot = {};
+        }
+    }
     A->ss.copy() = std::move(T);
     return MI_OK;
+}
+
+static int sstream_columns_on_demand(mi_csr_t A, bool want_pack)
+{
+    if (!A->ss.dev.val || A->ss.mw || (want_pack ? A->ss.dev.pack != nullptr : A->ss.dev.slot != nullptr)) return MI_OK;
+    if (!A->d_indcol) return fail(MI_ERR_STATE, "sliced copy: the handle holds no column indices to rebuild a column stream from");
+    std::vector<int> back((size_t)A->nnz);
+    HIP_TRY(hipMemcpy(back.data(), A->d_indcol, sizeof(int) * (size_t)A->nnz, hipMemcpyDeviceToHost));
+    return build_sstream_columns(A, A->ss, A->h_ptrow.data(), back.data(), want_pack);
 }
 
 int launch_sstream(mi_csr_t A, const double* d_x, double* d_y, const int* rowmap, hipStream_t s, const RingComm* comm)
 {
     SstreamTable& T = A->ss;
     SsView S{T.dev.val, T.dev.slot, T.dev.wg, T.dev.win, T.nwg, A->n + T.shift, A->ncols, rowmap, T.shift};
+    S.pack = T.dev.pack;
+    S.slice_len = T.dev.slice_len;
     double* yy = rowmap ? d_y : d_y - T.shift;
+    if (T.packed ? (!T.dev.pack || T.mw || comm) : !T.dev.slot) return fail(MI_ERR_STATE, "sliced copy: the column stream in use is not on the device");
+    if (T.packed) {
+        if (T.deep) {
+            if (T.nt) hipLaunchKernelGGL((spmv_sstream<12, true, 0, 12>), dim3((unsigned)T.nwg), dim3(256), 0, s, S, d_x, yy);
+            else hipLaunchKernelGGL((spmv_sstream<12, false, 0, 12>), dim3((unsigned)T.nwg), dim3(256), 0, s, S, d_x, yy);
+        } else {
+            if (T.nt) hipLaunchKernelGGL((spmv_sstream<8, true, 0, 12>), dim3((unsigned)T.nwg), dim3(256), 0, s, S, d_x, yy);
+            else hipLaunchKernelGGL((spmv_sstream<8, false, 0, 12>), dim3((unsigned)T.nwg), dim3(256), 0, s, S, d_x, yy);
+        }
+        HIP_TRY(hipGetLastError());
+        return MI_OK;
+    }
     if (T.mw) {
         if (comm) return fail(MI_ERR_STATE, "the cut-ring sliced stream has no fused multi-GPU form");
         SsMwView V{S, T.dev.winK};
@@ -422,7 +492,8 @@
         if (!asked && A->mring.ok_fraction < 0.90) A->mring = {};
     }
     if (plan_wanted("MI355_SSTREAM", "sstream", measured, &asked)) {
-        if ((rc = build_sstream(A, in.ptrow, in.indcol, in.ghost_lo, in.ghost_hi))) return rc;
+        const bool for_race = !getenv("MI355_SPMV_KERNEL") && !env_is("MI355_SPMV_AUTOTUNE", "0") && in.nnz >= kMeasureNnz;
+        if ((rc = build_sstream(A, in.ptrow, in.indcol, in.ghost_lo, in.ghost_hi, for_race))) return rc;
         A->ss.asked = asked;
     }
     return MI_OK;
@@ -566,7 +637,27 @@
         if (bf >= 0) {
             A->ss.nt = (bf & 1) == 0;
             A->ss.deep = bf >= 2;
-            if (better(us[bf], holder)) A->auto_kernel = MI_KERNEL_SSTREAM;
+            double ss_us = us[bf];
+            if (A->ss.dev.pack && A->ss.dev.slot) {
+                bool pfailed = false, ufailed = false;
+                for (int round = 0; round < 2; round++) {
+                    A->ss.packed = true;
+                    if (!pfailed) measure(3, timed, A->ss.us_packed, pfailed);
+                    A->ss.packed = false;
+                    if (!ufailed) measure(3, timed, A->ss.us_unpacked, ufailed);
+                }
+                if (pfailed) A->ss.us_packed = 0.0;
+                if (ufailed) A->ss.us_unpacked = 0.0;
+                A->ss.packed = !ufailed && better(A->ss.us_packed, A->ss.us_unpacked);
+                if (A->ss.packed) {
+                    A->ss.dev.slot = {};
+                    ss_us = A->ss.us_packed;
+                } else {
+                    A->ss.dev.pack = {};
+                    A->ss.groups = 0;
+                }
+            }
+            if (better(ss_us, holder)) A->auto_kernel = MI_KERNEL_SSTREAM;
         }
         if (A->auto_kernel != MI_KERNEL_SSTREAM && !A->ss.asked && !(A->ghost_lo < A->ghost_hi)) A->ss.copy() = {};
     }
@@ -652,6 +743,10 @@
     const bool forced_kernel = apply_forced_kernel(A);
     if (!forced_kernel && in.nnz < kMeasureNnz && A->auto_kernel == MI_KERNEL_RING && !in.ghosts()) A->auto_kernel = MI_KERNEL_STREAM;
     if (!forced_kernel && !env_is("MI355_SPMV_AUTOTUNE", "0") && in.nnz >= kMeasureNnz && (rc = measure_at_create(A, in, defer_placement))) return rc;
+    if (!A->ss.packed && A->ss.dev.pack) {
+        A->ss.dev.pack = {};
+        A->ss.groups = 0;
+    }
     HIP_TRY(hipStreamSynchronize(nullptr));
     *out = owner.release();
     return MI_OK;
@@ -1125,6 +1220,65 @@
     return MI_OK;
 }
 
+extern "C" int mi_csr_sstream_pack_info(mi_csr_t A, int* built, int* slots_built, int* in_use, int* eligible, const char** reason, long long* groups,
+                                        double* us_packed, double* us_unpacked, double* stream_bytes_per_nnz)
+{
+    CHECK_ARG(A, "null handle");
+    if (A->inner) A = A->inner;
+    const SstreamTable& T = A->ss;
+    if (built) *built = T.dev.pack != nullptr;
+    if (slots_built) *slots_built = T.dev.slot != nullptr;
+    if (in_use) *in_use = T.dev.val && T.packed;
+    if (eligible) *eligible = T.pack_eligible;
+    if (reason) *reason = T.pack_why;
+    if (groups) *groups = T.groups;
+    if (us_packed) *us_packed = T.us_packed;
+    if (us_unpacked) *us_unpacked = T.us_unpacked;
+    if (stream_bytes_per_nnz)
+        *stream_bytes_per_nnz = T.dev.val && A->nnz > 0 ? ((double)T.steps * 1024.0 + (T.packed ? (double)T.groups * 768.0 : (double)T.steps * 256.0)) / (double)A->nnz : 0.0;
+    return MI_OK;
+}
+
+extern "C" int mi_csr_sstream_set_packed(mi_csr_t A, int packed)
+{
+    CHECK_ARG(A, "null handle");
+    if (A->inner) A = A->inner;
+    if (!A->ss.dev.val) return fail(MI_ERR_UNSUPPORTED, "the handle holds no sliced copy (mi_csr_set_kernel(MI_KERNEL_SSTREAM) builds one)");
+    int rc = need_device();
+    if (rc || (rc = sstream_columns_on_demand(A, packed != 0))) return rc;
+    if (packed && !A->ss.dev.pack) return fail(MI_ERR_UNSUPPORTED, std::string("the sliced copy cannot be packed: ") + (A->ss.mw ? kSsPackWhyPlan : A->ss.pack_why));
+    HIP_TRY(hipDeviceSynchronize());
+    A->ss.packed = packed != 0;
+    if (A->ss.packed) A->ss.dev.slot = {};
+    else {
+        A->ss.dev.pack = {};
+        A->ss.groups = 0;
+    }
+    return MI_OK;
+}
+
+extern "C" int mi_sstream_pack_probe(int n, int ncols, const int* ptrow, const int* indcol, int shift, int* eligible, long long* groups, int* max_dist)
+{
+    CHECK_ARG(n >= 0 && ncols >= 0 && ptrow && ptrow[0] == 0 && eligible, "bad argument");
+    CHECK_ARG(shift == 0 || shift == 1, "shift must be 0 or 1");
+    CHECK_ARG(ptrow[n] == 0 || indcol, "indcol is null");
+    for (int i = 0; i < n; i++) CHECK_ARG(ptrow[i] <= ptrow[i + 1], "ptrow must be non-decreasing");
+    for (int k = 0; k < ptrow[n]; k++) CHECK_ARG(indcol[k] >= 0 && indcol[k] < ncols, "column index outside [0, ncols)");
+    SsPlanHost P;
+    SsPackHost K;
+    build_sstream_plan(n, ncols, ptrow, indcol, ss_max_padding(), P, true, shift);
+    build_sstream_pack(P, n, ptrow, indcol, false, K);
+    *eligible = K.eligible ? 1 : 0;
+    if (groups) *groups = K.groups;
+    if (max_dist) *max_dist = K.max_dist;
+    if (!K.eligible) {
+        g_err = std::string("not eligible: ") + K.why;
+        return MI_OK;
+    }
+    if (const char* bad = check_sstream_pack(P, K, n, ptrow)) return fail(MI_ERR_STATE, std::string("packed column stream: ") + bad);
+    return MI_OK;
+}
+
 extern "C" int mi_sstream_plan_probe(int n, int ncols, const int* ptrow, const int* indcol, int* eligible, int* rounds, long long* steps, double* padding)
 {
     return mi_sstream_plan_probe_ex(n, ncols, ptrow, indcol, 0, 0, 0, eligible, rounds, steps, padding, nullptr, nullptr);
@@ -1475,7 +1629,7 @@
     case MI_KERNEL_SSTREAM: {
         static thread_local char nm[64];
         if (A->ss.mw) snprintf(nm, sizeof nm, "spmv_sstream_mw<%d, %s>", A->ss.deep ? 12 : 8, A->ss.nt ? "true" : "false");
-        else snprintf(nm, sizeof nm, "spmv_sstream<%d, %s, 0>", A->ss.deep ? 12 : 8, A->ss.nt ? "true" : "false");
+        else snprintf(nm, sizeof nm, A->ss.packed ? "spmv_sstream<%d, %s, 0, 12>" : "spmv_sstream<%d, %s, 0>", A->ss.deep ? 12 : 8, A->ss.nt ? "true" : "false");
         return nm;
     }
     case MI_KERNEL_TILE: {
diff --git a/navierstokes_amd/csrc/capi_internal.hpp b/navierstokes_amd/csrc/capi_internal.hpp
--- a/navierstokes_amd/csrc/capi_internal.hpp
+++ b/navierstokes_amd/csrc/capi_internal.hpp
@@ -178,12 +178,17 @@
     bool nt = true;
     bool deep = true;
     bool fusable = false;
+    bool packed = false;
+    long long groups = 0;
     bool asked = false;
     std::vector<int> h_wg_halo;
     std::vector<SsWg> h_wg;
 };
 struct SstreamTable : SstreamCopy {
     double tune_us[4] = {0, 0, 0, 0};
+    double us_packed = 0, us_unpacked = 0;
+    int pack_eligible = -1;
+    const char* pack_why = "";
     SstreamCopy& copy() { return *this; }
 };
 
diff --git a/navierstokes_amd/csrc/spmv_sstream.hpp b/navierstokes_amd/csrc/spmv_sstream.hpp
--- a/navierstokes_amd/csrc/spmv_sstream.hpp
+++ b/navierstokes_amd/csrc/spmv_sstream.hpp
@@ -24,6 +24,9 @@
 constexpr unsigned kSsFirst = 0x4000u;
 constexpr int kSsPadSteps = 64;
 constexpr int kSsMaxWgs = 256;
+constexpr int kSsPackBias = 2047;
+constexpr unsigned kSsPackPad = 0xFFFu;
+constexpr int kSsPackTail = kSsPadSteps / 4 + 1;
 constexpr int kSsFill = 24;
 constexpr int kSsGhostSlack = 3;
 
@@ -34,7 +37,8 @@
     int t[5];
     int halo;
     int link;
-    int pad[3];
+    int gbase;
+    int pad[2];
 };
 static_assert(sizeof(SsWg) == 64, "one record = one 64-byte scalar load");
 
@@ -47,6 +51,8 @@
     const int* rowmap;
     int shift;
     unsigned long long* trace = nullptr;
+    const unsigned* pack = nullptr;
+    const int* slice_len = nullptr;
 };
 
 struct SsPlanHost {
@@ -54,6 +60,7 @@
     const char* why = "";
     int nwg = 0, rounds = 0, shift = 0;
     long long steps = 0, pad_places = 0;
+    long long groups = 0;
     int max_slice_nnz = 0;
     std::vector<int> wptr, rptr, slice_step, slice_len;
     std::vector<int2> win;
@@ -207,6 +214,8 @@
         for (int k = 0; k < 5; k++) W.t[k] = P.wptr[(size_t)g * 4 + k];
         W.halo = P.wg_halo[g];
         W.link = -1;
+        W.gbase = (int)P.groups;
+        for (int k = 0; k < 4; k++) P.groups += (W.t[k + 1] - W.t[k] + 3) / 4;
     }
     P.eligible = true;
     if (!want_slots) return;
@@ -303,6 +312,120 @@
     return nullptr;
 }
 
+struct SsPackHost {
+    bool eligible = false;
+    const char* why = "";
+    long long groups = 0;
+    int max_dist = 0;
+    std::vector<unsigned> code;
+};
+constexpr const char* kSsPackWhyPlan = "the plain sliced plan is not eligible";
+constexpr const char* kSsPackWhyGhosts = "a combined piece with ghost columns is not packed";
+constexpr const char* kSsPackWhyFar = "a nonzero lies more than 2047 columns from its row";
+
+inline unsigned ss_pack_get(const unsigned* q, int k)
+{
+    const int o = 12 * k, w = o >> 5, b = o & 31;
+    unsigned v = q[w] >> b;
+    if (b + 12 > 32) v |= q[w + 1] << (32 - b);
+    return v & 0xFFFu;
+}
+inline void ss_pack_put(unsigned* q, int k, unsigned code)
+{
+    const int o = 12 * k, w = o >> 5, b = o & 31;
+    q[w] = (q[w] & ~(0xFFFu << b)) | (code << b);
+    if (b + 12 > 32) q[w + 1] = (q[w + 1] & ~(0xFFFu >> (32 - b))) | (code >> (32 - b));
+}
+
+inline void build_sstream_pack(const SsPlanHost& P, int n, const int* ptrow, const int* indcol, bool ghosts, SsPackHost& K, bool want_codes = true)
+{
+    K = SsPackHost();
+    for (int i = 0; i < n; i++)
+        for (int k = ptrow[i]; k < ptrow[i + 1]; k++) K.max_dist = std::max(K.max_dist, indcol[k] > i ? indcol[k] - i : i - indcol[k]);
+    if (!P.eligible) { K.why = kSsPackWhyPlan; return; }
+    if (ghosts) { K.why = kSsPackWhyGhosts; return; }
+    if (K.max_dist > kSsPackBias) { K.why = kSsPackWhyFar; return; }
+    K.eligible = true;
+    K.groups = P.groups + kSsPackTail;
+    if (!want_codes) return;
+    const int shift = P.shift, nv = n + shift;
+    auto PT = [&](int v) { const int i = v - shift; return ptrow[i < 0 ? 0 : (i > n ? n : i)]; };
+    K.code.assign((size_t)K.groups * 64 * 3, 0xFFFFFFFFu);
+    auto fill = [&](int g0, int g1) {
+        for (int g = g0; g < g1; g++) {
+            long long gb = P.wg[g].gbase;
+            for (int wv = 0; wv < 4; wv++) {
+                const int t0 = P.wptr[(size_t)g * 4 + wv];
+                for (int r = P.rptr[g]; r < P.rptr[g + 1]; r++) {
+                    const int row0 = r * kSsRound + wv * kSsSliceRows;
+                    const int s0 = P.slice_step[(size_t)r * 4 + wv] - t0;
+                    for (int l = 0; l < 64; l++)
+                        for (int h = 0; h < 2; h++) {
+                            const int v = row0 + 2 * l + h;
+                            if (v >= nv || v < shift) continue;
+                            const int i = v - shift, len = PT(v + 1) - PT(v);
+                            for (int j = 0; j < len; j++) {
+                                const int o = s0 + j;
+                                ss_pack_put(&K.code[((size_t)(gb + (o >> 2)) * 64 + l) * 3], 2 * (o & 3) + h, (unsigned)(indcol[PT(v) + j] - i + kSsPackBias));
+                            }
+                        }
+                }
+                gb += (P.wptr[(size_t)g * 4 + wv + 1] - t0 + 3) / 4;
+            }
+        }
+    };
+    unsigned nt = std::thread::hardware_concurrency();
+    nt = nt > 16 ? 16 : (nt < 1 ? 1 : nt);
+    if (P.rounds < 64 || nt == 1) fill(0, P.nwg);
+    else {
+        std::vector<std::thread> th;
+        for (unsigned k = 0; k < nt; k++) th.emplace_back(fill, (int)((long long)P.nwg * k / nt), (int)((long long)P.nwg * (k + 1) / nt));
+        for (std::thread& x : th) x.join();
+    }
+}
+
+inline const char* check_sstream_pack(const SsPlanHost& P, const SsPackHost& K, int n, const int* ptrow)
+{
+    if (!K.eligible) return nullptr;
+    if (!P.eligible || P.slot.size() != (size_t)(P.steps + kSsPadSteps) * 64) return "packed stream without its 16-bit plan";
+    if (K.groups != P.groups + kSsPackTail || K.code.size() != (size_t)K.groups * 64 * 3) return "group count disagrees with the streams";
+    const int shift = P.shift, nv = n + shift;
+    auto PT = [&](int v) { const int i = v - shift; return ptrow[i < 0 ? 0 : (i > n ? n : i)]; };
+    long long gb = 0, real = 0;
+    for (int g = 0; g < P.nwg; g++) {
+        if (P.wg[g].gbase != gb) return "a workgroup record's group base is not the running sum";
+        for (int wv = 0; wv < 4; wv++) {
+            const int t0 = P.wptr[(size_t)g * 4 + wv], t1 = P.wptr[(size_t)g * 4 + wv + 1];
+            const long long ng = (t1 - t0 + 3) / 4;
+            int r = P.rptr[g];
+            for (long long o = 0; o < 4 * ng; o++) {
+                while (o < t1 - t0 && r + 1 < P.rptr[g + 1] && t0 + o >= P.slice_step[(size_t)(r + 1) * 4 + wv]) r++;
+                for (int l = 0; l < 64; l++)
+                    for (int h = 0; h < 2; h++) {
+                        const unsigned code = ss_pack_get(&K.code[((size_t)(gb + (o >> 2)) * 64 + l) * 3], 2 * (int)(o & 3) + h);
+                        bool is_real = false;
+                        if (o < t1 - t0) {
+                            const int v = r * kSsRound + wv * kSsSliceRows + 2 * l + h, j = (int)(t0 + o) - P.slice_step[(size_t)r * 4 + wv];
+                            is_real = v >= shift && v < nv && j < PT(v + 1) - PT(v);
+                            if (is_real) {
+                                const unsigned sh = (P.slot[(size_t)(t0 + o) * 64 + l] >> (16 * h)) & 0xffffu;
+                                if (code == kSsPackPad) return "a nonzero is coded as padding";
+                                if ((unsigned)((v - shift + (int)code - kSsPackBias) & (kSsRing - 1)) != (sh & (kSsRing - 1)) || (sh & kSsPad)) return "a code does not decode to the plan's slot";
+                                real++;
+                            }
+                        }
+                        if (!is_real && code != kSsPackPad) return "a padding place is not 0xFFF";
+                    }
+            }
+            gb += ng;
+        }
+    }
+    if (gb != P.groups || real != (long long)ptrow[n]) return "the packed stream does not hold every nonzero once";
+    for (size_t q = (size_t)P.groups * 64 * 3; q < K.code.size(); q++)
+        if (K.code[q] != 0xFFFFFFFFu) return "the tail is not 0xFF bytes";
+    return nullptr;
+}
+
 template <int CAP>
 __global__ __launch_bounds__(256) void sstream_fill_kernel(int nslices, int n, int shift, const int* __restrict__ ptrow, const double* __restrict__ src,
                                                            double* __restrict__ csr_out, const int* __restrict__ slice_step, const int* __restrict__ slice_len,
@@ -358,6 +481,7 @@
     DevArray<int2> winK;
     DevArray<ss_v2d> val;
     DevArray<unsigned> slot;
+    DevArray<unsigned> pack;
     DevArray<SsWg> wg;
     DevArray<int2> win;
     DevArray<int> slice_step, slice_len;
@@ -378,11 +502,24 @@
     return e;
 }
 
-template <int D, bool NT, int ABL, int MODE>
+struct __attribute__((packed, aligned(4))) ss_pk3 {
+    unsigned w[3];
+};
+__device__ __forceinline__ unsigned ss_code(const ss_pk3& q, int k)
+{
+    const int o = 12 * k, w = o >> 5, b = o & 31;
+    unsigned v = q.w[w] >> b;
+    if (b + 12 > 32) v |= q.w[w + 1] << (32 - b);
+    return v & kSsPackPad;
+}
+
+template <int D, bool NT, int ABL, int MODE, int PACK = 0>
 __device__ __forceinline__ void ss_body(const SsView& S, const SsWg& W, int g, const double* __restrict__ x_in, double* __restrict__ y, const RingComm& C,
                                         double* ring , ss_v2d* s_park )
 {
     constexpr bool GHOSTS = MODE == 2;
+    static_assert(PACK == 0 || (PACK == 12 && MODE == 0 && D % 4 == 0), "the packed column stream: plain products, whole groups in flight");
+    constexpr int NG = PACK ? D / 4 : 1;
     const int tid = threadIdx.x, lane = tid & 63;
     const int wv = __builtin_amdgcn_readfirstlane(tid >> 6);
     const double* __restrict__ x = MODE != 0 ? x_in - C.n_left : x_in;
@@ -401,13 +538,30 @@
     const unsigned* sb = S.slot + lane;
     ss_v2d a[D];
     unsigned sl[D];
+    ss_pk3 pk[NG];
+    int gb = 0;
+    if constexpr (PACK != 0) {
+        const int g1 = W.gbase + ((W.t[1] - W.t[0] + 3) >> 2), g2 = g1 + ((W.t[2] - W.t[1] + 3) >> 2), g3 = g2 + ((W.t[3] - W.t[2] + 3) >> 2);
+        gb = wv == 0 ? W.gbase : (wv == 1 ? g1 : (wv == 2 ? g2 : g3));
+    }
+    const ss_pk3* pb = reinterpret_cast<const ss_pk3*>(S.pack) + lane;
     auto first_steps = [&]() {
 #pragma unroll
         for (int d = 0; d < D; d++) {
             a[d] = NT ? __builtin_nontemporal_load(vb + (size_t)(t0 + d) * 64) : vb[(size_t)(t0 + d) * 64];
-            sl[d] = sb[(size_t)(t0 + d) * 64];
+            if constexpr (PACK == 0) sl[d] = sb[(size_t)(t0 + d) * 64];
+        }
+        if constexpr (PACK != 0) {
+#pragma unroll
+            for (int q = 0; q < NG; q++) pk[q] = pb[(size_t)(gb + q) * 64];
         }
     };
+    int next_begin = 0, len_ahead = 0, base = 0;
+    if constexpr (PACK != 0) {
+        next_begin = t0 + S.slice_len[4 * r_begin + wv];
+        len_ahead = S.slice_len[4 * min(r_begin + 1, r_end - 1) + wv];
+        base = r_begin * kSsRound + wv * kSsSliceRows + 2 * lane - S.shift - kSsPackBias;
+    }
     if (GHOSTS) {
         first_steps();
         push_wait_flags(C.flags, C.nb, C.n_nb, C.step, 0u, C.timeouts, C.spin_max, tid, 256);
@@ -463,13 +617,13 @@
         park[parked * 64] = ss_v2d{acc0, acc1};
         if (++parked == kSsPark || r == r_end - 1 - kSsTail) flush();
     };
-    for (int t = t0; t < t_end; t += D) {
+    for (int t = t0, gi = gb; t < t_end; t += D, gi += NG) {
 #pragma unroll
         for (int d = 0; d < D; d++) {
             const int i = t + d;
             if (i < t_end) {
-                const unsigned s = sl[d];
-                if ((__builtin_amdgcn_readfirstlane(s) & kSsFirst) && i != t0) {
+                const unsigned s = PACK == 0 ? sl[d] : 0u;
+                if (PACK == 0 ? (__builtin_amdgcn_readfirstlane(s) & kSsFirst) && i != t0 : i == next_begin) {
                     emit();
                     acc0 = acc1 = 0.0;
                     r++;
@@ -487,14 +641,28 @@
 #pragma unroll
                         for (int u = 0; u < kSsNewMax / 256; u++) nx[u] = x[min(max(wn.x + tid + 256 * u, cfirst), cowned)];
                     }
+                    if constexpr (PACK != 0) {
+                        base += kSsRound;
+                        next_begin += len_ahead;
+                        len_ahead = S.slice_len[4 * min(r + 1, r_end - 1) + wv];
+                    }
                 }
-                const double x0 = (ABL & 1) ? 1.0 + lane : ring[s & (kSsRing - 1)], x1 = (ABL & 1) ? 0.5 : ring[(s >> 16) & (kSsRing - 1)];
-                const double n0 = fma(a[d].x, x0, acc0), n1 = fma(a[d].y, x1, acc1);
-                acc0 = (s & kSsPad) ? acc0 : n0;
-                acc1 = (s & (kSsPad << 16)) ? acc1 : n1;
+                if constexpr (PACK == 0) {
+                    const double x0 = (ABL & 1) ? 1.0 + lane : ring[s & (kSsRing - 1)], x1 = (ABL & 1) ? 0.5 : ring[(s >> 16) & (kSsRing - 1)];
+                    const double n0 = fma(a[d].x, x0, acc0), n1 = fma(a[d].y, x1, acc1);
+                    acc0 = (s & kSsPad) ? acc0 : n0;
+                    acc1 = (s & (kSsPad << 16)) ? acc1 : n1;
+                } else {
+                    const unsigned c0 = ss_code(pk[d / 4], 2 * (d % 4)), c1 = ss_code(pk[d / 4], 2 * (d % 4) + 1);
+                    const double x0 = (ABL & 1) ? 1.0 + lane : ring[(base + (int)c0) & (kSsRing - 1)], x1 = (ABL & 1) ? 0.5 : ring[(base + 1 + (int)c1) & (kSsRing - 1)];
+                    const double n0 = fma(a[d].x, x0, acc0), n1 = fma(a[d].y, x1, acc1);
+                    acc0 = c0 == kSsPackPad ? acc0 : n0;
+                    acc1 = c1 == kSsPackPad ? acc1 : n1;
+                }
             }
             a[d] = NT ? __builtin_nontemporal_load(vb + (size_t)(i + D) * 64) : vb[(size_t)(i + D) * 64];
-            sl[d] = sb[(size_t)(i + D) * 64];
+            if constexpr (PACK == 0) sl[d] = sb[(size_t)(i + D) * 64];
+            else if (d % 4 == 3) pk[d / 4] = pb[(size_t)(gi + NG + d / 4) * 64];
         }
     }
     if ((ABL & 8) && tid == 0) S.trace[4 * g + 2] = __builtin_amdgcn_s_memrealtime();
@@ -524,6 +692,17 @@
     ss_body<D, NT, ABL, 0>(S, W, g, x, y, RingComm{}, ring, s_park);
 }
 
+template <int D, bool NT, int ABL, int PACK>
+__global__ __launch_bounds__(256) void spmv_sstream(SsView S, const double* __restrict__ x, double* __restrict__ y)
+{
+    const int g = ss_logical_wg(S, (int)blockIdx.x);
+    const SsWg W = S.wg[g];
+    if (W.r_begin >= W.r_end) return;
+    __shared__ double ring[kSsRing];
+    __shared__ ss_v2d s_park[4 * kSsPark * 64];
+    ss_body<D, NT, ABL, 0, PACK>(S, W, g, x, y, RingComm{}, ring, s_park);
+}
+
 template <int D, bool NT, int ABL = 0>
 __global__ __launch_bounds__(256) void spmv_sstream_fused(SsView S, const double* __restrict__ x, double* __restrict__ y, RingComm C)
 {
diff --git a/navierstokes_amd/mpk.py b/navierstokes_amd/mpk.py
--- a/navierstokes_amd/mpk.py
+++ b/navierstokes_amd/mpk.py
@@ -106,6 +106,9 @@
         "mi_csr_mring_info": [_vp, P(i), P(i), P(i), P(d), P(d), P(i)],
         "mi_csr_sstream_info": [_vp, P(i), P(i), P(ll), P(d), P(d), P(i)],
         "mi_sstream_plan_probe": [i, i, _vp, _vp, P(i), P(i), P(ll), P(d)],
+        "mi_csr_sstream_pack_info": [_vp, P(i), P(i), P(i), P(i), P(_c.c_char_p), P(ll), P(d), P(d), P(d)],
+        "mi_csr_sstream_set_packed": [_vp, i],
+        "mi_sstream_pack_probe": [i, i, _vp, _vp, i, P(i), P(ll), P(i)],
         "mi_sstream_plan_probe_ex": [i, i, _vp, _vp, i, i, i, P(i), P(i), P(ll), P(d), P(i), P(i)],
         "mi_sstream_mw_plan_probe": [i, i, _vp, _vp, i, P(i), P(i), P(ll), P(d)],
         "mi_csr_placement_info": [_vp, P(i), P(i), P(d), i],
@@ -386,8 +389,24 @@
         pad = _c.c_double()
         us = (_c.c_double * 4)()
         check(lib().mi_csr_sstream_info(self.handle, _c.byref(b), _c.byref(r), _c.byref(st), _c.byref(pad), us, _c.byref(fm)))
+        pk = self.sstream_pack_info()
         return dict(built=bool(b.value), rounds=r.value, steps=st.value, padding=pad.value, us_d8_nt=us[0], us_d8_temporal=us[1], us_d12_nt=us[2],
-                    us_d12_temporal=us[3], form=fm.value)
+                    us_d12_temporal=us[3], form=fm.value, packed=pk["in_use"], us_packed=pk["us_packed"],
+                    us_unpacked_same_form=pk["us_unpacked"], stream_bytes_per_nnz=pk["stream_bytes_per_nnz"])
+
+    def sstream_pack_info(self):
+        b, sb, iu, el = _c.c_int(), _c.c_int(), _c.c_int(), _c.c_int()
+        why = _c.c_char_p()
+        g = _c.c_longlong()
+        up, uu, bpn = _c.c_double(), _c.c_double(), _c.c_double()
+        check(lib().mi_csr_sstream_pack_info(self.handle, _c.byref(b), _c.byref(sb), _c.byref(iu), _c.byref(el), _c.byref(why), _c.byref(g),
+                                             _c.byref(up), _c.byref(uu), _c.byref(bpn)))
+        return dict(built=bool(b.value), slots_built=bool(sb.value), in_use=bool(iu.value), eligible=None if el.value < 0 else bool(el.value),
+                    reason=(why.value or b"").decode(), groups=g.value, us_packed=up.value, us_unpacked=uu.value, stream_bytes_per_nnz=bpn.value)
+
+    def sstream_set_packed(self, packed):
+        check(lib().mi_csr_sstream_set_packed(self.handle, 1 if packed else 0))
+        return self
 
     def tile_info(self):
         b, nb, nt = _c.c_int(), _c.c_int(), _c.c_int()
```
